# GuyTevet/motion-diffusion-model

Hardware: NVIDIA H100
Metric: motions/sec (higher is better)
Workload: dtype fp16 operands / fp32 accumulate (in/out projections hi-lo split)

## Files before the change

### motion-diffusion-model_b200/csrc/attention_tc.cuh

```cuda
#pragma once
#include <cuda_fp16.h>

#include "epilogues.cuh"
#include "ptx.cuh"

namespace b200 {

constexpr int ATC_THREADS = 128;
constexpr int ATC_QROWS = 64;
constexpr int ATC_TILES_PER_CTA = 4;
constexpr int ATC_DH = 128;
constexpr int ATC_MAX_KEYS = 256;

__host__ __device__ constexpr int atc_keys(int S) { return S <= 64 ? 64 : S <= 208 ? 208 : 256; }

struct AttnTcSmem {
  static __host__ __device__ int total(int keys) { return 1024 + 4 * keys * 128; }
};

template <int KEYS, bool WIDE>
__global__ void __launch_bounds__(ATC_THREADS, 2)
attention_tc_kernel(const __grid_constant__ CUtensorMap map_kv, const __half* __restrict__ qkv, __half* __restrict__ out,
                    const int* __restrict__ kvlen, int S, int d, float scale_log2) {
  constexpr int ATOM = KEYS * 128;
  constexpr int NS = KEYS / 2;
  constexpr int NB = KEYS / 16;
  extern __shared__ uint8_t smem_raw[];
  __shared__ uint64_t bar_k, bar_v;
  uint8_t* sK = reinterpret_cast<uint8_t*>((reinterpret_cast<uintptr_t>(smem_raw) + 1023) & ~uintptr_t(1023));
  uint8_t* sV = sK + 2 * ATOM;
  const int warp = threadIdx.x >> 5, lane = threadIdx.x & 31;
  const int h = blockIdx.x, smp = blockIdx.y;
  const int ld = 3 * d;
  const __half* base = qkv + static_cast<size_t>(smp) * S * ld;

  pdl_launch_dependents();
  if (threadIdx.x == 0) {
    tma_prefetch_desc(&map_kv);
    mbar_init(&bar_k, 1);
    mbar_init(&bar_v, 1);
    fence_barrier_init();
  }
  __syncthreads();
  pdl_wait();
  if (threadIdx.x == 0) {
    mbar_expect_tx(&bar_k, 2 * ATOM);
    for (int a = 0; a < 2; ++a) tma_load_3d(sK + a * ATOM, &map_kv, &bar_k, d + h * ATC_DH + 64 * a, 0, smp);
    mbar_expect_tx(&bar_v, 2 * ATOM);
    for (int a = 0; a < 2; ++a) tma_load_3d(sV + a * ATOM, &map_kv, &bar_v, 2 * d + h * ATC_DH + 64 * a, 0, smp);
  }

  const int kvl = min(kvlen[smp], S);
  const int nblk = max(1, (kvl + 15) >> 4);
  const int g = lane >> 2, t = lane & 3;
  const uint64_t desc_k = wgmma_desc_k_sw128(smem_u32(sK));
  const uint64_t desc_v = wgmma_desc_mn_sw128(smem_u32(sV), ATOM);
  const int ntiles = (S + ATC_QROWS - 1) / ATC_QROWS;
  const int ldo = (WIDE ? 2 : 1) * d;

  uint32_t qa[8][4];
  auto load_q = [&](int tile) {
    const int ra = tile * ATC_QROWS + warp * 16 + g, rb = ra + 8;
    const bool va = ra < S, vb = rb < S;
    const uint32_t* pa = reinterpret_cast<const uint32_t*>(base + static_cast<size_t>(va ? ra : 0) * ld + h * ATC_DH);
    const uint32_t* pb = reinterpret_cast<const uint32_t*>(base + static_cast<size_t>(vb ? rb : 0) * ld + h * ATC_DH);
#pragma unroll
    for (int ks = 0; ks < 8; ++ks) {
      qa[ks][0] = va ? pa[8 * ks + t] : 0u;
      qa[ks][1] = vb ? pb[8 * ks + t] : 0u;
      qa[ks][2] = va ? pa[8 * ks + 4 + t] : 0u;
      qa[ks][3] = vb ? pb[8 * ks + 4 + t] : 0u;
    }
  };
  if (static_cast<int>(blockIdx.z) < ntiles) load_q(blockIdx.z);
#pragma unroll 1
  for (int tile = blockIdx.z; tile < ntiles; tile += gridDim.z) {
    const int ra = tile * ATC_QROWS + warp * 16 + g, rb = ra + 8;
    const bool va = ra < S, vb = rb < S;
    float s[NS];
    mbar_wait(&bar_k, 0);
    wgmma_fence();
#pragma unroll
    for (int ks = 0; ks < 8; ++ks)
      WgmmaRA<KEYS, 0>::mma(s, qa[ks], desc_k + (((ks >> 2) * ATOM + (ks & 3) * 32) >> 4), ks != 0);
    wgmma_commit();
    wgmma_wait<0>();
    wgmma_fence_acc(s);
    float mxa = -INFINITY, mxb = -INFINITY;
#pragma unroll
    for (int j = 0; j < NS / 4; ++j)
#pragma unroll
      for (int i = 0; i < 2; ++i) {
        if (8 * j + 2 * t + i < kvl) {
          mxa = fmaxf(mxa, s[4 * j + i]);
          mxb = fmaxf(mxb, s[4 * j + 2 + i]);
        }
      }
#pragma unroll
    for (int o = 1; o < 4; o <<= 1) {
      mxa = fmaxf(mxa, __shfl_xor_sync(0xffffffffu, mxa, o));
      mxb = fmaxf(mxb, __shfl_xor_sync(0xffffffffu, mxb, o));
    }
    const float offa = (mxa == -INFINITY) ? 0.f : mxa * scale_log2;
    const float offb = (mxb == -INFINITY) ? 0.f : mxb * scale_log2;
    auto ex2 = [](float x) {
      float y;
      asm("ex2.approx.ftz.f32 %0, %1;" : "=f"(y) : "f"(x));
      return y;
    };
    uint32_t p[NB][4];
    float suma = 0.f, sumb = 0.f;
#pragma unroll
    for (int j = 0; j < NS / 4; ++j) {
      const int key = 8 * j + 2 * t;
      const float p0 = key < kvl ? ex2(fmaf(s[4 * j], scale_log2, -offa)) : 0.f;
      const float p1 = key + 1 < kvl ? ex2(fmaf(s[4 * j + 1], scale_log2, -offa)) : 0.f;
      const float p2 = key < kvl ? ex2(fmaf(s[4 * j + 2], scale_log2, -offb)) : 0.f;
      const float p3 = key + 1 < kvl ? ex2(fmaf(s[4 * j + 3], scale_log2, -offb)) : 0.f;
      suma += p0 + p1;
      sumb += p2 + p3;
      p[j >> 1][2 * (j & 1)] = pack_half2(p0, p1);
      p[j >> 1][2 * (j & 1) + 1] = pack_half2(p2, p3);
    }
#pragma unroll
    for (int off = 1; off < 4; off <<= 1) {
      suma += __shfl_xor_sync(0xffffffffu, suma, off);
      sumb += __shfl_xor_sync(0xffffffffu, sumb, off);
    }
    const float inva = suma > 0.f ? 1.f / suma : 0.f;
    const float invb = sumb > 0.f ? 1.f / sumb : 0.f;
    float o[64];
    mbar_wait(&bar_v, 0);
    wgmma_fence();
#pragma unroll
    for (int kk = 0; kk < NB; ++kk)
      if (kk < nblk) WgmmaRA<128, 1>::mma(o, p[kk], desc_v + ((kk * 16 * 128) >> 4), kk != 0);
    wgmma_commit();
    if (tile + static_cast<int>(gridDim.z) < ntiles) load_q(tile + gridDim.z);
    wgmma_wait<0>();
    wgmma_fence_acc(o);
    __half* oa = out + (static_cast<size_t>(smp) * S + (va ? ra : 0)) * ldo + h * ATC_DH + 2 * t;
    __half* ob = out + (static_cast<size_t>(smp) * S + (vb ? rb : 0)) * ldo + h * ATC_DH + 2 * t;
#pragma unroll
    for (int j = 0; j < 16; ++j) {
      const float x0 = o[4 * j] * inva, x1 = o[4 * j + 1] * inva, x2 = o[4 * j + 2] * invb, x3 = o[4 * j + 3] * invb;
      const __half2 ha = __floats2half2_rn(x0, x1), hb = __floats2half2_rn(x2, x3);
      if (va) *reinterpret_cast<__half2*>(oa + 8 * j) = ha;
      if (vb) *reinterpret_cast<__half2*>(ob + 8 * j) = hb;
      if (WIDE) {
        const float2 fa = __half22float2(ha), fb = __half22float2(hb);
        if (va) *reinterpret_cast<__half2*>(oa + d + 8 * j) = __floats2half2_rn(x0 - fa.x, x1 - fa.y);
        if (vb) *reinterpret_cast<__half2*>(ob + d + 8 * j) = __floats2half2_rn(x2 - fb.x, x3 - fb.y);
      }
    }
  }
}

}
```

### motion-diffusion-model_b200/csrc/engine.cu

```cuda
#include <cuda.h>
#include <cuda_fp16.h>
#include <cuda_runtime.h>

#include <cmath>
#include <cstdarg>
#include <cstdio>
#include <cstring>
#include <map>
#include <string>
#include <vector>

#include "../../include/b200mdm.h"
#include "attention_tc.cuh"
#include "epilogues.cuh"
#include "gemm.cuh"
#include "gemm_ln.cuh"
#include "gemm_pingpong.cuh"
#include "postprocess.cuh"
#include "kernels.cuh"

using namespace b200;

static thread_local char g_err[512] = "";
static int fail(int code, const char* fmt, ...) {
  va_list ap;
  va_start(ap, fmt);
  vsnprintf(g_err, sizeof(g_err), fmt, ap);
  va_end(ap);
  return code;
}
#define CUDA_TRY(expr)                                                                               \
  do {                                                                                               \
    cudaError_t _e = (expr);                                                                         \
    if (_e != cudaSuccess)                                                                           \
      return fail(B200MDM_ECUDA, "%s failed: %s (%s:%d)", #expr, cudaGetErrorString(_e), __FILE__, __LINE__); \
  } while (0)
#define TRY(expr)            \
  do {                       \
    int _r = (expr);         \
    if (_r != B200MDM_OK) return _r; \
  } while (0)

typedef CUresult (*EncodeTiledFn)(CUtensorMap*, CUtensorMapDataType, cuuint32_t, void*, const cuuint64_t*,
                                  const cuuint64_t*, const cuuint32_t*, const cuuint32_t*, CUtensorMapInterleave,
                                  CUtensorMapSwizzle, CUtensorMapL2promotion, CUtensorMapFloatOOBfill);
static EncodeTiledFn g_encode = nullptr;
static int resolve_driver() {
  if (g_encode) return B200MDM_OK;
  void* fn = nullptr;
  cudaDriverEntryPointQueryResult qres;
  CUDA_TRY(cudaGetDriverEntryPoint("cuTensorMapEncodeTiled", &fn, cudaEnableDefault, &qres));
  if (!fn || qres != cudaDriverEntryPointSuccess) return fail(B200MDM_ECUDA, "cuTensorMapEncodeTiled not available");
  g_encode = reinterpret_cast<EncodeTiledFn>(fn);
  return B200MDM_OK;
}
static int make_map_t(CUtensorMap* m, const void* ptr, int elem_bytes, uint64_t rows, uint64_t cols, uint64_t ld,
                      uint32_t box_rows) {
  TRY(resolve_driver());
  if ((reinterpret_cast<uintptr_t>(ptr) & 15) || (ld * elem_bytes) % 16) return fail(B200MDM_EINVAL, "TMA operand misaligned");
  cuuint64_t gdim[2] = {cols, rows};
  cuuint64_t gstr[1] = {ld * elem_bytes};
  cuuint32_t box[2] = {static_cast<cuuint32_t>(128 / elem_bytes), box_rows};
  cuuint32_t estr[2] = {1, 1};
  CUresult r = g_encode(m, elem_bytes == 2 ? CU_TENSOR_MAP_DATA_TYPE_FLOAT16 : CU_TENSOR_MAP_DATA_TYPE_FLOAT32, 2,
                        const_cast<void*>(ptr), gdim, gstr, box, estr, CU_TENSOR_MAP_INTERLEAVE_NONE,
                        CU_TENSOR_MAP_SWIZZLE_128B, CU_TENSOR_MAP_L2_PROMOTION_L2_256B, CU_TENSOR_MAP_FLOAT_OOB_FILL_NONE);
  if (r != CUDA_SUCCESS) return fail(B200MDM_ECUDA, "cuTensorMapEncodeTiled failed (%d)", static_cast<int>(r));
  return B200MDM_OK;
}
static int make_map(CUtensorMap* m, const void* ptr, uint64_t rows, uint64_t cols, uint64_t ld, uint32_t box_rows) {
  return make_map_t(m, ptr, 2, rows, cols, ld, box_rows);
}
static int make_map_3d(CUtensorMap* m, const void* ptr, uint64_t n, uint64_t rows, uint64_t cols, uint64_t ld,
                       uint32_t box_rows) {
  TRY(resolve_driver());
  if ((reinterpret_cast<uintptr_t>(ptr) & 15) || (ld * 2) % 16) return fail(B200MDM_EINVAL, "TMA operand misaligned");
  cuuint64_t gdim[3] = {cols, rows, n};
  cuuint64_t gstr[2] = {ld * 2, rows * ld * 2};
  cuuint32_t box[3] = {64, box_rows, 1};
  cuuint32_t estr[3] = {1, 1, 1};
  CUresult r = g_encode(m, CU_TENSOR_MAP_DATA_TYPE_FLOAT16, 3, const_cast<void*>(ptr), gdim, gstr, box, estr,
                        CU_TENSOR_MAP_INTERLEAVE_NONE, CU_TENSOR_MAP_SWIZZLE_128B, CU_TENSOR_MAP_L2_PROMOTION_L2_256B,
                        CU_TENSOR_MAP_FLOAT_OOB_FILL_NONE);
  if (r != CUDA_SUCCESS) return fail(B200MDM_ECUDA, "cuTensorMapEncodeTiled(3d) failed (%d)", static_cast<int>(r));
  return B200MDM_OK;
}

static int make_hres_map(CUtensorMap* m, const void* hres, uint64_t rows) {
  return make_map(m, hres, rows, 2 * GLN_D, 2 * GLN_D, GLN_RES_BOX_ROWS);
}

static int make_map_res(CUtensorMap* m, const void* ptr, uint64_t rows, uint64_t d) {
  TRY(resolve_driver());
  if (reinterpret_cast<uintptr_t>(ptr) & 15) return fail(B200MDM_EINVAL, "TMA operand misaligned");
  cuuint64_t gdim[2] = {2 * d, rows};
  cuuint64_t gstr[1] = {d * 4};
  cuuint32_t box[2] = {32, 32};
  cuuint32_t estr[2] = {1, 1};
  CUresult r = g_encode(m, CU_TENSOR_MAP_DATA_TYPE_FLOAT16, 2, const_cast<void*>(ptr), gdim, gstr, box, estr,
                        CU_TENSOR_MAP_INTERLEAVE_NONE, CU_TENSOR_MAP_SWIZZLE_64B, CU_TENSOR_MAP_L2_PROMOTION_L2_256B,
                        CU_TENSOR_MAP_FLOAT_OOB_FILL_NONE);
  if (r != CUDA_SUCCESS) return fail(B200MDM_ECUDA, "cuTensorMapEncodeTiled(residual) failed (%d)", static_cast<int>(r));
  return B200MDM_OK;
}

struct Tensor32 {
  float* dev = nullptr;
  std::vector<int64_t> shape;
  size_t numel = 0;
};

struct LayerW {
  __half *wqkv = nullptr, *wo = nullptr, *w1 = nullptr, *w2 = nullptr;
  const float *bqkv, *bo, *b1, *b2, *g1, *be1, *g2, *be2;
  CUtensorMap m_wqkv, m_w1;
  CUtensorMap m_wo_256, m_w2_256;
  __half *wq_c = nullptr, *wo_c = nullptr;
  const float *bq_c = nullptr, *bo_c = nullptr, *g3 = nullptr, *be3 = nullptr;
  CUtensorMap m_wq_c, m_wo_c_256;
  const float *wv_c32 = nullptr, *bv_c32 = nullptr, *wo_c32 = nullptr;
};

struct GraphKey {
  int mode = -1, B = 0, T = 0, flags = 0;
  int order = 0;
  const void *pred = nullptr, *imask = nullptr, *imotion = nullptr;
  const void* target_g = nullptr;
  bool operator==(const GraphKey& o) const {
    return mode == o.mode && B == o.B && T == o.T && flags == o.flags && order == o.order && pred == o.pred &&
           imask == o.imask && imotion == o.imotion && target_g == o.target_g;
  }
};

struct Workspace {
  int B = 0, T = 0, S = 0, halves = 1, Bp = 0, M = 0, MB = 0;
  __half *xin16 = nullptr, *hres = nullptr, *qkv16 = nullptr, *att16 = nullptr, *ffn16 = nullptr, *g16 = nullptr;
  float *tok0 = nullptr, *condproj = nullptr, *proj = nullptr, *scale = nullptr, *x_work = nullptr, *eps_buf = nullptr;
  int *kvlen = nullptr, *tvec = nullptr, *action = nullptr;
  CUtensorMap m_xin, m_h16, m_att, m_ffn, m_g16;
  CUtensorMap m_qkv_st, m_ffn_st;
  CUtensorMap m_qkv_kv;
  CUtensorMap m_res_c, m_res_u;
  CUtensorMap m_hres;
  float* pe_bias = nullptr;
  bool cond_set = false;
  int Mt = 0;
  float *encperm = nullptr, *memtok = nullptr, *memproj = nullptr;
  __half *mem16 = nullptr, *qc16 = nullptr, *kvc16 = nullptr;
  unsigned char* memmask = nullptr;
  CUtensorMap m_mem, m_qc_st, m_kvc_st;
  bool prefix_set = false;
  float *cross_mb = nullptr, *cross_u = nullptr, *cross_b = nullptr, *cross_c = nullptr;
  float *tgt_valid = nullptr, *tgt_g = nullptr;
  bool target_set = false;
  float *plms_ring = nullptr, *plms_mid = nullptr, *plms_pred = nullptr;
  int plms_done = -1, plms_order = 0;
  cudaGraphExec_t graph_exec = nullptr;
  GraphKey graph_key;
  int graph_kernels = 0;
  unsigned long long last_use = 0;
};

struct b200mdm_engine : Workspace {
  b200mdm_config cfg;
  int d, ff, L, H, JF, Kp_in, N_out_pad;
  int num_sms = 132;
  std::map<std::string, Tensor32> store;
  bool finalized = false;
  __half *w_in3 = nullptr, *w_out3 = nullptr;
  CUtensorMap m_win, m_wout;
  std::vector<LayerW> layers;
  const float *b_in = nullptr, *b_out = nullptr, *pe = nullptr, *w_txt = nullptr, *b_txt = nullptr, *act_emb = nullptr;
  float *temb_hidden = nullptr, *temb_table = nullptr;
  __half* wkv_all = nullptr;
  float* bkv_all = nullptr;
  CUtensorMap m_wkv_all;
  float *tw0 = nullptr, *tb0 = nullptr, *twk = nullptr, *tbk = nullptr, *twsum = nullptr;
  int tG = 0, tdj = 0, tin = 0, tlayers = 0;
  std::vector<float> h_valid;
  float* sched = nullptr;
  int* tmap = nullptr;
  int n_steps = 0, sched_cap = 0;
  float* sched_next = nullptr;
  bool sched_next_fresh = false;
  std::vector<Workspace> pool;
  unsigned long long use_clock = 0;
  std::vector<int> h_kv, h_action;
  std::vector<unsigned char> h_mask;
  bool dec = false;
  bool dec_clip = false;
  float* cross_t = nullptr;
  int ctx = 0, s_off = 1;
  int kw = 1;
  const unsigned char* inpaint_mask = nullptr;
  const float* inpaint_motion = nullptr;
  unsigned long long noise_seed = 0;
  long long noise_sample_base = 0;
  StepState* state = nullptr;
  cudaStream_t work = nullptr;
  cudaEvent_t ev_in = nullptr, ev_out = nullptr;
  long long launches = 0;
};

template <class T>
static int dalloc(T** p, size_t n, bool zero = false) {
  const cudaError_t err = cudaMalloc(reinterpret_cast<void**>(p), n * sizeof(T));
  if (err != cudaSuccess) {
    cudaGetLastError();
    return fail(B200MDM_ECUDA, "cudaMalloc of %zu bytes failed: %s", n * sizeof(T), cudaGetErrorString(err));
  }
  if (zero) CUDA_TRY(cudaMemset(*p, 0, n * sizeof(T)));
  return B200MDM_OK;
}
template <class T>
static void dfree(T*& p) {
  if (p) cudaFree(p);
  p = nullptr;
}

template <int BN, class Epi, bool RES = false>
static int set_gemm_attr() {
  CUDA_TRY(cudaFuncSetAttribute(gemm_f16_wgmma<BN, Epi, RES>, cudaFuncAttributeMaxDynamicSharedMemorySize,
                                GemmSmem<BN, Epi, RES>::TOTAL));
  return B200MDM_OK;
}
template <class Epi>
static int set_pingpong_attr() {
  CUDA_TRY(cudaFuncSetAttribute(gemm_f16_pingpong<Epi>, cudaFuncAttributeMaxDynamicSharedMemorySize, PP_SMEM_BYTES));
  return B200MDM_OK;
}
template <int KEYS>
static int set_attention_attr() {
  CUDA_TRY(cudaFuncSetAttribute(attention_tc_kernel<KEYS, false>, cudaFuncAttributeMaxDynamicSharedMemorySize,
                                AttnTcSmem::total(KEYS)));
  CUDA_TRY(cudaFuncSetAttribute(attention_tc_kernel<KEYS, true>, cudaFuncAttributeMaxDynamicSharedMemorySize,
                                AttnTcSmem::total(KEYS)));
  return B200MDM_OK;
}
static int init_kernel_attrs() {
  static unsigned long long done_mask = 0;
  int dev = 0;
  CUDA_TRY(cudaGetDevice(&dev));
  if (dev < 64 && ((done_mask >> dev) & 1ull)) return B200MDM_OK;
  TRY((set_pingpong_attr<EpiBiasF16<false>>()));
  TRY((set_pingpong_attr<EpiBiasF16<true>>()));
  TRY((set_pingpong_attr<EpiBiasF16Wide<true>>()));
  TRY((set_pingpong_attr<EpiBiasF16Global>()));
  TRY((set_gemm_attr<256, EpiBiasF16<false>>()));
  TRY((set_gemm_attr<256, EpiBiasF16<true>>()));
  TRY((set_gemm_attr<64, EpiBiasF16<false>, true>()));
  TRY((set_gemm_attr<64, EpiBiasF16<true>, true>()));
  CUDA_TRY(cudaFuncSetAttribute(gemm_resid_ln_cluster, cudaFuncAttributeMaxDynamicSharedMemorySize, GemmLnSmem::TOTAL));
  TRY((set_gemm_attr<128, EpiEmbed>()));
  TRY((set_gemm_attr<96, EpiOut<OutStep>>()));
  TRY((set_gemm_attr<96, EpiOut<OutPlms>>()));
  TRY((set_gemm_attr<96, EpiOut<OutReverse>>()));
  TRY((set_attention_attr<64>()));
  TRY((set_attention_attr<208>()));
  TRY((set_attention_attr<256>()));
  CUDA_TRY(cudaFuncSetAttribute(cross_attention_long_kernel, cudaFuncAttributeMaxDynamicSharedMemorySize, XAL_SMEM));
  if (dev < 64) done_mask |= 1ull << dev;
  return B200MDM_OK;
}

static bool g_pdl_now = false;
static bool pdl_enabled() {
  static int v = -1;
  if (v < 0) {
    const char* e = getenv("B200MDM_PDL");
    v = (e && e[0] == '0') ? 0 : 1;
  }
  return v == 1;
}
struct PdlScope {
  PdlScope() { g_pdl_now = pdl_enabled(); }
  ~PdlScope() { g_pdl_now = false; }
};
template <class... KArgs, class... Args>
static cudaError_t launch_k(void (*kern)(KArgs...), dim3 grid, dim3 block, size_t smem, cudaStream_t s, Args&&... args) {
  cudaLaunchConfig_t cfg;
  memset(&cfg, 0, sizeof(cfg));
  cfg.gridDim = grid;
  cfg.blockDim = block;
  cfg.dynamicSmemBytes = smem;
  cfg.stream = s;
  cudaLaunchAttribute at[1];
  at[0].id = cudaLaunchAttributeProgrammaticStreamSerialization;
  at[0].val.programmaticStreamSerializationAllowed = 1;
  cfg.attrs = at;
  cfg.numAttrs = g_pdl_now ? 1 : 0;
  return cudaLaunchKernelEx(&cfg, kern, static_cast<KArgs>(std::forward<Args>(args))...);
}

template <int BN, class Epi, class = void> struct epi_unstaged : std::false_type {};
template <int BN, class Epi> struct epi_unstaged<BN, Epi, std::enable_if_t<Epi::UNSTAGED>> : std::true_type {};

template <int BN, class Epi>
static int launch_gemm(const CUtensorMap& a, const CUtensorMap& b, const CUtensorMap& c, int M, int N, int K,
                       const typename Epi::Params& p, cudaStream_t s, int num_sms) {
  if (!epi_unstaged<BN, Epi>::value && N * 4 > GEMM_BIAS_BYTES)
    return fail(B200MDM_ENOTIMPL, "GEMM epilogue vectors are staged for N <= %d", GEMM_BIAS_BYTES / 4);
  const int tiles = ((M + GEMM_BLOCK_M - 1) / GEMM_BLOCK_M) * ((N + BN - 1) / BN);
  const int grid = tiles < num_sms ? tiles : num_sms;
  CUDA_TRY(launch_k(gemm_f16_wgmma<BN, Epi>, dim3(grid), dim3(GEMM_THREADS), GemmSmem<BN, Epi>::TOTAL, s, a, b, c, M, N, K, p));
  return B200MDM_OK;
}
template <int BN, class Epi>
static int launch_gemm_resident(const CUtensorMap& a, const CUtensorMap& b, const CUtensorMap& c, int M, int N, int K,
                                const typename Epi::Params& p, cudaStream_t s, int num_sms) {
  const int tiles_n = (N + BN - 1) / BN;
  const int tiles = ((M + GEMM_BLOCK_M - 1) / GEMM_BLOCK_M) * tiles_n;
  const int grid = tiles < num_sms ? tiles : num_sms;
  if (K > GEMM_RES_KB_MAX * GEMM_BLOCK_K || tiles_n > grid || N * 4 > GEMM_BIAS_BYTES)
    return fail(B200MDM_ENOTIMPL, "W-resident GEMM needs K <= %d and N <= %d", GEMM_RES_KB_MAX * GEMM_BLOCK_K, grid * BN);
  CUDA_TRY(launch_k(gemm_f16_wgmma<BN, Epi, true>, dim3(grid), dim3(GEMM_THREADS), GemmSmem<BN, Epi, true>::TOTAL, s, a, b, c, M, N, K, p));
  return B200MDM_OK;
}
template <class Epi>
static int launch_gemm_pp(const CUtensorMap& a, const CUtensorMap& b, const CUtensorMap& c, int M, int N, int K,
                          const typename Epi::Params& p, cudaStream_t s, int num_sms) {
  if (!epi_unstaged<PP_BLOCK_N, Epi>::value && N * 4 > GEMM_BIAS_BYTES)
    return fail(B200MDM_ENOTIMPL, "GEMM epilogue vectors are staged for N <= %d", GEMM_BIAS_BYTES / 4);
  const int tiles = ((M + GEMM_BLOCK_M - 1) / GEMM_BLOCK_M) * ((N + PP_BLOCK_N - 1) / PP_BLOCK_N);
  const int grid = tiles < num_sms ? tiles : num_sms;
  CUDA_TRY(launch_k(gemm_f16_pingpong<Epi>, dim3(grid), dim3(GEMM_THREADS), PP_SMEM_BYTES, s, a, b, c, M, N, K, p));
  return B200MDM_OK;
}
template <bool GELU>
static int launch_gemm_bias(const CUtensorMap& a, const CUtensorMap& b, const CUtensorMap& c, int M, int N, int K,
                            const float* bias, cudaStream_t s, int num_sms) {
  typename EpiBiasF16<GELU>::Params p{bias};
  return launch_gemm_pp<EpiBiasF16<GELU>>(a, b, c, M, N, K, p, s, num_sms);
}

static int launch_gemm_resid_ln(const CUtensorMap& a, const CUtensorMap& w256, const CUtensorMap& hres, int M, int K,
                                const float* bias, const float* gamma, const float* beta, cudaStream_t s, int num_sms) {
  const int tiles = (M + GEMM_BLOCK_M - 1) / GEMM_BLOCK_M;
  const int max_clusters = num_sms / 2;
  const int clusters = tiles < max_clusters ? tiles : max_clusters;
  GemmLnParams lp{bias, gamma, beta, 1e-5f};
  CUDA_TRY(launch_k(gemm_resid_ln_cluster, dim3(2 * clusters), dim3(GLN_THREADS), GemmLnSmem::TOTAL, s, a, w256, hres, M, K, lp));
  return B200MDM_OK;
}

static int make_attention_kv_map(CUtensorMap* m, const void* qkv, int n_samples, int S, int ld) {
  return make_map_3d(m, qkv, n_samples, S, ld, ld, atc_keys(S));
}
template <int KEYS>
static cudaError_t launch_attention_keys(const CUtensorMap& map_kv, const __half* qkv, __half* out, const int* kvlen,
                                         dim3 grid, int S, int d, float scale_log2, cudaStream_t s, bool wide) {
  return launch_k(wide ? attention_tc_kernel<KEYS, true> : attention_tc_kernel<KEYS, false>, grid, dim3(ATC_THREADS),
                  AttnTcSmem::total(KEYS), s, map_kv, qkv, out, kvlen, S, d, scale_log2);
}
static int launch_attention_tc(const CUtensorMap& map_kv, const __half* qkv, __half* out, const int* kvlen, int n_samples,
                               int S, int d, int H, cudaStream_t s, bool wide = false) {
  if (d != H * ATC_DH) return fail(B200MDM_ENOTIMPL, "attention: head_dim must be 128");
  if (S > ATC_MAX_KEYS) return fail(B200MDM_ENOTIMPL, "attention: at most %d tokens per sample", ATC_MAX_KEYS);
  const float scale_log2 = 1.4426950408889634f / sqrtf(static_cast<float>(ATC_DH));
  const int tiles = (S + ATC_QROWS - 1) / ATC_QROWS;
  const dim3 grid(H, n_samples, (tiles + ATC_TILES_PER_CTA - 1) / ATC_TILES_PER_CTA);
  const int keys = atc_keys(S);
  if (keys == 64) CUDA_TRY(launch_attention_keys<64>(map_kv, qkv, out, kvlen, grid, S, d, scale_log2, s, wide));
  else if (keys == 208) CUDA_TRY(launch_attention_keys<208>(map_kv, qkv, out, kvlen, grid, S, d, scale_log2, s, wide));
  else CUDA_TRY(launch_attention_keys<256>(map_kv, qkv, out, kvlen, grid, S, d, scale_log2, s, wide));
  return B200MDM_OK;
}
#ifdef B200_TRACE
static int debug_skip_mask() {
  static int v = -1;
  if (v < 0) {
    const char* e = getenv("B200MDM_DEBUG_SKIP");
    v = e ? atoi(e) : 0;
  }
  return v;
}
#define B200_SKIP(bit) (debug_skip_mask() & (bit))
#else
#define B200_SKIP(bit) (0)
#endif
extern "C" const char* b200mdm_last_error(void) { return g_err; }
extern "C" int b200mdm_version(void) { return 1; }

extern "C" int b200mdm_create(const b200mdm_config* cfg, b200mdm_engine** out) {
  if (!cfg || !out) return fail(B200MDM_EINVAL, "null argument");
  if (cfg->arch != B200MDM_ARCH_TRANS_ENC && cfg->arch != B200MDM_ARCH_TRANS_DEC)
    return fail(B200MDM_ENOTIMPL, "arch %d: trans_enc and trans_dec are implemented", cfg->arch);
  if (cfg->arch == B200MDM_ARCH_TRANS_DEC && (cfg->cond_mode != B200MDM_COND_TEXT || cfg->context_len < 0))
    return fail(B200MDM_ENOTIMPL, "trans_dec needs text-token conditioning (BERT) and context_len >= 0");
  if (cfg->emb_trans_dec < 0 || cfg->emb_trans_dec > 1 || cfg->dec_memory < B200MDM_DEC_MEMORY_TOKENS ||
      cfg->dec_memory > B200MDM_DEC_MEMORY_CLIP)
    return fail(B200MDM_EINVAL, "emb_trans_dec must be 0 or 1 and dec_memory 0 (tokens) or 1 (CLIP) (got %d / %d)",
                cfg->emb_trans_dec, cfg->dec_memory);
  if (cfg->arch == B200MDM_ARCH_TRANS_ENC && (cfg->emb_trans_dec || cfg->dec_memory))
    return fail(B200MDM_EINVAL, "emb_trans_dec and dec_memory are trans_dec fields");
  if (cfg->arch == B200MDM_ARCH_TRANS_DEC && (cfg->dec_memory == B200MDM_DEC_MEMORY_CLIP) != (cfg->emb_trans_dec == 1))
    return fail(B200MDM_ENOTIMPL, "trans_dec implements the BERT token memory without the timestep token (DiP) and the CLIP "
                "memory with it (emb_trans_dec); got dec_memory %d, emb_trans_dec %d", cfg->dec_memory, cfg->emb_trans_dec);
  if (cfg->dec_memory == B200MDM_DEC_MEMORY_CLIP && cfg->context_len != 0)
    return fail(B200MDM_ENOTIMPL, "trans_dec with a CLIP memory has no prefix completion (context_len %d)", cfg->context_len);
  if (cfg->latent_dim != 512 || cfg->num_heads != 4 || cfg->ff_size % 64 || cfg->ff_size <= 0)
    return fail(B200MDM_ENOTIMPL, "kernels are specialised for latent_dim 512 / 4 heads (got %d / %d)", cfg->latent_dim,
                cfg->num_heads);
  if (cfg->num_layers <= 0 || cfg->njoints <= 0 || cfg->nfeats <= 0 || cfg->pos_embed_max_len <= 0 || cfg->temb_rows <= 0)
    return fail(B200MDM_EINVAL, "bad config");
  if (cfg->target_encoder < B200MDM_TARGET_NONE || cfg->target_encoder > B200MDM_TARGET_SPLIT)
    return fail(B200MDM_EINVAL, "target_encoder %d: 0 none, 1 single, 2 multi, 3 split", cfg->target_encoder);
  if (cfg->target_encoder != B200MDM_TARGET_NONE) {
    if (cfg->target_joints <= 0 || cfg->target_joints > 64 || cfg->target_enc_layers < 0 || cfg->target_enc_layers > 16)
      return fail(B200MDM_EINVAL, "target encoder: 1..64 joints and 0..16 layers (got %d / %d)", cfg->target_joints,
                  cfg->target_enc_layers);
    if (cfg->target_encoder == B200MDM_TARGET_SPLIT && cfg->latent_dim % cfg->target_joints)
      return fail(B200MDM_EINVAL, "split target encoder: latent_dim %% target_joints != 0 (model/mdm.py:427)");
  }
  int dev = 0;
  CUDA_TRY(cudaGetDevice(&dev));
  cudaDeviceProp prop;
  CUDA_TRY(cudaGetDeviceProperties(&prop, dev));
  if (prop.major != 9 || prop.minor != 0) return fail(B200MDM_ECUDA, "sm_90a device required (found sm_%d%d)", prop.major, prop.minor);
  TRY(init_kernel_attrs());
  TRY(resolve_driver());
  b200mdm_engine* e = new b200mdm_engine();
  e->cfg = *cfg;
  e->d = cfg->latent_dim;
  e->ff = cfg->ff_size;
  e->L = cfg->num_layers;
  e->H = cfg->num_heads;
  e->JF = cfg->njoints * cfg->nfeats;
  e->Kp_in = (e->JF + 7) & ~7;
  e->N_out_pad = ((e->JF + 95) / 96) * 96;
  e->num_sms = prop.multiProcessorCount;
  e->layers.resize(e->L);
  e->dec = cfg->arch == B200MDM_ARCH_TRANS_DEC;
  e->dec_clip = e->dec && cfg->dec_memory == B200MDM_DEC_MEMORY_CLIP;
  e->ctx = e->dec ? cfg->context_len : 0;
  e->s_off = (e->dec && !e->dec_clip) ? e->ctx : 1;
  e->kw = (e->dec && !e->dec_clip) ? 2 : 1;
  CUDA_TRY(cudaStreamCreateWithFlags(&e->work, cudaStreamNonBlocking));
  CUDA_TRY(cudaEventCreateWithFlags(&e->ev_in, cudaEventDisableTiming));
  CUDA_TRY(cudaEventCreateWithFlags(&e->ev_out, cudaEventDisableTiming));
  TRY(dalloc(&e->state, 1, true));
  *out = e;
  return B200MDM_OK;
}

static void drop_graph(Workspace* w) {
  if (w->graph_exec) cudaGraphExecDestroy(w->graph_exec);
  w->graph_exec = nullptr;
  w->graph_key = GraphKey();
}
static void free_workspace(Workspace* w) {
  drop_graph(w);
  dfree(w->xin16); dfree(w->hres); dfree(w->qkv16); dfree(w->att16); dfree(w->ffn16); dfree(w->g16);
  dfree(w->tok0); dfree(w->condproj); dfree(w->proj); dfree(w->scale); dfree(w->x_work); dfree(w->pe_bias); dfree(w->eps_buf);
  dfree(w->kvlen); dfree(w->tvec); dfree(w->action);
  dfree(w->encperm); dfree(w->memtok); dfree(w->memproj); dfree(w->mem16); dfree(w->qc16); dfree(w->kvc16); dfree(w->memmask);
  dfree(w->cross_mb); dfree(w->cross_u); dfree(w->cross_b); dfree(w->cross_c);
  dfree(w->tgt_valid); dfree(w->tgt_g);
  dfree(w->plms_ring); dfree(w->plms_mid); dfree(w->plms_pred);
  *w = Workspace();
}
static void free_all_workspaces(b200mdm_engine* e) {
  free_workspace(static_cast<Workspace*>(e));
  for (auto& w : e->pool) free_workspace(&w);
  e->pool.clear();
}
static void drop_all_graphs(b200mdm_engine* e) {
  drop_graph(static_cast<Workspace*>(e));
  for (auto& w : e->pool) drop_graph(&w);
}

extern "C" int b200mdm_destroy(b200mdm_engine* e) {
  if (!e) return B200MDM_OK;
  cudaDeviceSynchronize();
  free_all_workspaces(e);
  for (auto& kv : e->store) cudaFree(kv.second.dev);
  for (auto& l : e->layers) { dfree(l.wqkv); dfree(l.wo); dfree(l.w1); dfree(l.w2); dfree(l.wq_c); dfree(l.wo_c); }
  dfree(e->w_in3); dfree(e->w_out3); dfree(e->temb_hidden); dfree(e->temb_table); dfree(e->sched); dfree(e->tmap);
  dfree(e->sched_next);
  dfree(e->wkv_all); dfree(e->bkv_all); dfree(e->cross_t);
  dfree(e->tw0); dfree(e->tb0); dfree(e->twk); dfree(e->tbk); dfree(e->twsum);
  dfree(e->state);
  if (e->work) cudaStreamDestroy(e->work);
  if (e->ev_in) cudaEventDestroy(e->ev_in);
  if (e->ev_out) cudaEventDestroy(e->ev_out);
  delete e;
  return B200MDM_OK;
}

static bool known_weight_name(const b200mdm_engine* e, const std::string& n) {
  static const char* fixed[] = {"input_process.poseEmbedding.weight", "input_process.poseEmbedding.bias",
                                "embed_timestep.time_embed.0.weight", "embed_timestep.time_embed.0.bias",
                                "embed_timestep.time_embed.2.weight", "embed_timestep.time_embed.2.bias",
                                "embed_text.weight", "embed_text.bias", "embed_action.action_embedding",
                                "output_process.poseFinal.weight", "output_process.poseFinal.bias",
                                "sequence_pos_encoder.pe", "embed_timestep.sequence_pos_encoder.pe"};
  for (const char* f : fixed)
    if (n == f) return true;
  static const char* per_layer[] = {"self_attn.in_proj_weight", "self_attn.in_proj_bias", "self_attn.out_proj.weight",
                                    "self_attn.out_proj.bias", "linear1.weight", "linear1.bias", "linear2.weight",
                                    "linear2.bias", "norm1.weight", "norm1.bias", "norm2.weight", "norm2.bias",
                                    "multihead_attn.in_proj_weight", "multihead_attn.in_proj_bias",
                                    "multihead_attn.out_proj.weight", "multihead_attn.out_proj.bias", "norm3.weight", "norm3.bias"};
  const std::string pre = e->dec ? "seqTransDecoder.layers." : "seqTransEncoder.layers.";
  if (n.compare(0, pre.size(), pre) == 0) {
    size_t dot = n.find('.', pre.size());
    if (dot == std::string::npos) return false;
    int l = atoi(n.substr(pre.size(), dot - pre.size()).c_str());
    if (l < 0 || l >= e->L) return false;
    std::string rest = n.substr(dot + 1);
    for (const char* f : per_layer)
      if (rest == f) return true;
  }
  if (e->cfg.target_encoder != B200MDM_TARGET_NONE) {
    const int tl = e->cfg.target_enc_layers, nj = e->cfg.target_joints;
    auto lin = [](const std::string& r, int max_layer) {
      for (int k = 0; k <= max_layer; ++k)
        if (r == std::to_string(2 * k) + ".weight" || r == std::to_string(2 * k) + ".bias") return true;
      return false;
    };
    auto joint = [nj](const std::string& r, std::string* tail) {
      size_t dot = r.find('.');
      if (dot == std::string::npos || dot == 0 || r.find_first_not_of("0123456789") != dot) return false;
      if (atoi(r.substr(0, dot).c_str()) >= nj) return false;
      *tail = r.substr(dot + 1);
      return true;
    };
    const std::string pre = "embed_target_cond.";
    if (n.compare(0, pre.size(), pre) != 0) return false;
    const std::string r = n.substr(pre.size());
    std::string tail;
    switch (e->cfg.target_encoder) {
      case B200MDM_TARGET_SINGLE:
        return r.compare(0, 4, "mlp.") == 0 && lin(r.substr(4), tl);
      case B200MDM_TARGET_SPLIT:
        return r.compare(0, 10, "mini_mlps.") == 0 && joint(r.substr(10), &tail) && lin(tail, tl);
      case B200MDM_TARGET_MULTI:
        if (r == "target_all_loc_emb.weights") return true;
        return r.compare(0, 15, "target_loc_emb.") == 0 && joint(r.substr(15), &tail) && lin(tail, 1);
    }
  }
  return false;
}

extern "C" int b200mdm_load_weight(b200mdm_engine* e, const char* name, const float* data, const int64_t* shape,
                                   int32_t ndim) {
  if (!e || !name || !data || !shape || ndim < 1 || ndim > 4) return fail(B200MDM_EINVAL, "bad argument");
  std::string n(name);
  if (!known_weight_name(e, n)) return fail(B200MDM_EINVAL, "unexpected state_dict key '%s'", name);
  size_t numel = 1;
  std::vector<int64_t> shp(shape, shape + ndim);
  for (int64_t s : shp) {
    if (s <= 0) return fail(B200MDM_EINVAL, "bad shape for '%s'", name);
    numel *= static_cast<size_t>(s);
  }
  Tensor32& t = e->store[n];
  if (t.dev && t.numel != numel) { cudaFree(t.dev); t.dev = nullptr; }
  if (!t.dev) TRY(dalloc(&t.dev, numel));
  t.shape = shp;
  t.numel = numel;
  CUDA_TRY(cudaMemcpy(t.dev, data, numel * sizeof(float), cudaMemcpyDefault));
  e->finalized = false;
  return B200MDM_OK;
}

static int need(b200mdm_engine* e, const std::string& name, std::initializer_list<int64_t> shape, const float** out) {
  auto it = e->store.find(name);
  if (it == e->store.end()) return fail(B200MDM_ESTATE, "missing weight '%s'", name.c_str());
  std::vector<int64_t> want(shape);
  size_t numel = 1;
  for (int64_t s : want) numel *= static_cast<size_t>(s);
  if (it->second.numel != numel) return fail(B200MDM_EINVAL, "weight '%s' has %zu elements, expected %zu", name.c_str(), it->second.numel, numel);
  *out = it->second.dev;
  return B200MDM_OK;
}

static int to_f16(const float* src, __half** dst, size_t n, cudaStream_t s) {
  TRY(dalloc(dst, n));
  f32_to_f16_kernel<<<512, 256, 0, s>>>(src, *dst, n);
  CUDA_TRY(cudaGetLastError());
  return B200MDM_OK;
}
static int to_f16_k(const float* src, __half** dst, int N, int K, int kw, cudaStream_t s) {
  if (kw == 1) return to_f16(src, dst, static_cast<size_t>(N) * K, s);
  TRY(dalloc(dst, static_cast<size_t>(N) * K * 2));
  f32_to_f16_dup_kernel<<<512, 256, 0, s>>>(src, *dst, N, K);
  CUDA_TRY(cudaGetLastError());
  return B200MDM_OK;
}

static int pack_target_weights(b200mdm_engine* e, cudaStream_t s) {
  dfree(e->tw0); dfree(e->tb0); dfree(e->twk); dfree(e->tbk); dfree(e->twsum);
  const int enc = e->cfg.target_encoder, n = e->cfg.target_joints, d = e->d;
  if (enc == B200MDM_TARGET_NONE) return B200MDM_OK;
  const bool multi = enc == B200MDM_TARGET_MULTI;
  e->tG = enc == B200MDM_TARGET_SINGLE ? 1 : n;
  e->tdj = enc == B200MDM_TARGET_SPLIT ? d / n : d;
  e->tin = enc == B200MDM_TARGET_SINGLE ? 4 * n : multi ? 3 : 4;
  e->tlayers = multi ? 1 : e->cfg.target_enc_layers;
  const int G = e->tG, dj = e->tdj, in = e->tin, L = e->tlayers;
  TRY(dalloc(&e->tw0, static_cast<size_t>(G) * dj * in));
  TRY(dalloc(&e->tb0, static_cast<size_t>(G) * dj));
  TRY(dalloc(&e->twk, static_cast<size_t>(L > 0 ? L : 1) * G * dj * dj));
  TRY(dalloc(&e->tbk, static_cast<size_t>(L > 0 ? L : 1) * G * dj));
  for (int i = 0; i < G; ++i) {
    const std::string p = enc == B200MDM_TARGET_SINGLE ? std::string("embed_target_cond.mlp.")
                          : multi ? "embed_target_cond.target_loc_emb." + std::to_string(i) + "."
                                  : "embed_target_cond.mini_mlps." + std::to_string(i) + ".";
    const float *w, *b;
    TRY(need(e, p + "0.weight", {dj, in}, &w));
    TRY(need(e, p + "0.bias", {dj}, &b));
    CUDA_TRY(cudaMemcpyAsync(e->tw0 + static_cast<size_t>(i) * dj * in, w, sizeof(float) * dj * in, cudaMemcpyDeviceToDevice, s));
    CUDA_TRY(cudaMemcpyAsync(e->tb0 + static_cast<size_t>(i) * dj, b, sizeof(float) * dj, cudaMemcpyDeviceToDevice, s));
    for (int l = 0; l < L; ++l) {
      const std::string k = std::to_string(2 * (l + 1));
      TRY(need(e, p + k + ".weight", {dj, dj}, &w));
      TRY(need(e, p + k + ".bias", {dj}, &b));
      CUDA_TRY(cudaMemcpyAsync(e->twk + (static_cast<size_t>(l) * G + i) * dj * dj, w, sizeof(float) * dj * dj,
                               cudaMemcpyDeviceToDevice, s));
      CUDA_TRY(cudaMemcpyAsync(e->tbk + (static_cast<size_t>(l) * G + i) * dj, b, sizeof(float) * dj, cudaMemcpyDeviceToDevice, s));
    }
  }
  if (multi) {
    const float* ws;
    TRY(need(e, "embed_target_cond.target_all_loc_emb.weights", {n}, &ws));
    TRY(dalloc(&e->twsum, n));
    CUDA_TRY(cudaMemcpyAsync(e->twsum, ws, sizeof(float) * n, cudaMemcpyDeviceToDevice, s));
  }
  return B200MDM_OK;
}

static int encode_target(b200mdm_engine* e, const float* target_dev, const uint8_t* valid_host, int B, float* valid_dev,
                         float* g_dev, std::vector<float>& staging, cudaStream_t s) {
  const int n = e->cfg.target_joints, d = e->d;
  staging.assign(static_cast<size_t>(B) * n, 0.f);
  for (size_t i = 0; i < staging.size(); ++i) staging[i] = valid_host[i] ? 1.f : 0.f;
  CUDA_TRY(cudaMemcpyAsync(valid_dev, staging.data(), staging.size() * sizeof(float), cudaMemcpyHostToDevice, s));
  const size_t smem = sizeof(float) * (4 * n + 2 * d);
  target_embed_kernel<<<B, d, smem, s>>>(target_dev, valid_dev, e->tw0, e->tb0, e->twk, e->tbk, e->twsum, g_dev, n, e->tG,
                                         e->tdj, e->tin, e->tlayers, e->cfg.target_encoder == B200MDM_TARGET_MULTI ? 1 : 0);
  CUDA_TRY(cudaGetLastError());
  return B200MDM_OK;
}

extern "C" int b200mdm_finalize_weights(b200mdm_engine* e, void* stream) {
  if (!e) return fail(B200MDM_EINVAL, "null engine");
  cudaStream_t s = static_cast<cudaStream_t>(stream);
  const int d = e->d, ff = e->ff, JF = e->JF;
  const float *w_in, *w_out, *t0w, *t0b, *t2w, *t2b;
  TRY(need(e, "input_process.poseEmbedding.weight", {d, JF}, &w_in));
  TRY(need(e, "input_process.poseEmbedding.bias", {d}, &e->b_in));
  TRY(need(e, "output_process.poseFinal.weight", {JF, d}, &w_out));
  TRY(need(e, "output_process.poseFinal.bias", {JF}, &e->b_out));
  TRY(need(e, "embed_timestep.time_embed.0.weight", {d, d}, &t0w));
  TRY(need(e, "embed_timestep.time_embed.0.bias", {d}, &t0b));
  TRY(need(e, "embed_timestep.time_embed.2.weight", {d, d}, &t2w));
  TRY(need(e, "embed_timestep.time_embed.2.bias", {d}, &t2b));
  TRY(need(e, "sequence_pos_encoder.pe", {e->cfg.pos_embed_max_len, d}, &e->pe));
  if (e->cfg.cond_mode == B200MDM_COND_TEXT) {
    TRY(need(e, "embed_text.weight", {d, e->cfg.cond_dim}, &e->w_txt));
    TRY(need(e, "embed_text.bias", {d}, &e->b_txt));
  } else if (e->cfg.cond_mode == B200MDM_COND_ACTION) {
    TRY(need(e, "embed_action.action_embedding", {e->cfg.num_actions, d}, &e->act_emb));
  }
  if (e->cfg.temb_rows > e->cfg.pos_embed_max_len) return fail(B200MDM_EINVAL, "temb_rows exceeds the positional table");

  CUDA_TRY(cudaDeviceSynchronize());
  free_all_workspaces(e);
  for (auto& l : e->layers) { dfree(l.wqkv); dfree(l.wo); dfree(l.w1); dfree(l.w2); dfree(l.wq_c); dfree(l.wo_c); }
  dfree(e->w_in3); dfree(e->w_out3); dfree(e->temb_hidden); dfree(e->temb_table); dfree(e->wkv_all); dfree(e->bkv_all);
  dfree(e->cross_t);

  const int Kp = e->Kp_in;
  TRY(dalloc(&e->w_in3, static_cast<size_t>(d) * 3 * Kp, true));
  split_weight_kernel<<<d, 128, 0, s>>>(w_in, e->w_in3, d, JF, Kp);
  CUDA_TRY(cudaGetLastError());
  TRY(dalloc(&e->w_out3, static_cast<size_t>(e->N_out_pad) * 3 * d, true));
  split_weight_kernel<<<JF, 128, 0, s>>>(w_out, e->w_out3, JF, d, d);
  CUDA_TRY(cudaGetLastError());
  TRY(make_map(&e->m_win, e->w_in3, d, 3 * Kp, 3 * Kp, 128));
  TRY(make_map(&e->m_wout, e->w_out3, e->N_out_pad, 3 * d, 3 * d, 96));

  for (int l = 0; l < e->L; ++l) {
    LayerW& w = e->layers[l];
    const std::string p = std::string(e->dec ? "seqTransDecoder.layers." : "seqTransEncoder.layers.") + std::to_string(l) + ".";
    const float *wqkv, *wo, *w1, *w2;
    TRY(need(e, p + "self_attn.in_proj_weight", {3 * d, d}, &wqkv));
    TRY(need(e, p + "self_attn.in_proj_bias", {3 * d}, &w.bqkv));
    TRY(need(e, p + "self_attn.out_proj.weight", {d, d}, &wo));
    TRY(need(e, p + "self_attn.out_proj.bias", {d}, &w.bo));
    TRY(need(e, p + "linear1.weight", {ff, d}, &w1));
    TRY(need(e, p + "linear1.bias", {ff}, &w.b1));
    TRY(need(e, p + "linear2.weight", {d, ff}, &w2));
    TRY(need(e, p + "linear2.bias", {d}, &w.b2));
    TRY(need(e, p + "norm1.weight", {d}, &w.g1));
    TRY(need(e, p + "norm1.bias", {d}, &w.be1));
    TRY(need(e, p + "norm2.weight", {d}, &w.g2));
    TRY(need(e, p + "norm2.bias", {d}, &w.be2));
    const int kw = e->kw;
    TRY(to_f16_k(wqkv, &w.wqkv, 3 * d, d, kw, s));
    TRY(to_f16_k(wo, &w.wo, d, d, kw, s));
    TRY(to_f16_k(w1, &w.w1, ff, d, kw, s));
    TRY(to_f16_k(w2, &w.w2, d, ff, kw, s));
    TRY(make_map(&w.m_wqkv, w.wqkv, 3 * d, kw * d, kw * d, 128));
    TRY(make_map(&w.m_w1, w.w1, ff, kw * d, kw * d, 128));
    TRY(make_map(&w.m_wo_256, w.wo, d, kw * d, kw * d, 256));
    TRY(make_map(&w.m_w2_256, w.w2, d, kw * ff, kw * ff, 256));
    if (e->dec) {
      const float *wc, *bc, *woc;
      TRY(need(e, p + "multihead_attn.in_proj_weight", {3 * d, d}, &wc));
      TRY(need(e, p + "multihead_attn.in_proj_bias", {3 * d}, &bc));
      TRY(need(e, p + "multihead_attn.out_proj.weight", {d, d}, &woc));
      TRY(need(e, p + "multihead_attn.out_proj.bias", {d}, &w.bo_c));
      TRY(need(e, p + "norm3.weight", {d}, &w.g3));
      TRY(need(e, p + "norm3.bias", {d}, &w.be3));
      if (e->dec_clip) {
        w.wv_c32 = wc + static_cast<size_t>(2) * d * d;
        w.bv_c32 = bc + 2 * d;
        w.wo_c32 = woc;
        continue;
      }
      w.bq_c = bc;
      TRY(to_f16_k(wc, &w.wq_c, d, d, kw, s));
      if (l == 0) {
        TRY(dalloc(&e->wkv_all, static_cast<size_t>(e->L) * 2 * d * d));
        TRY(dalloc(&e->bkv_all, static_cast<size_t>(e->L) * 2 * d));
        TRY(make_map(&e->m_wkv_all, e->wkv_all, static_cast<uint64_t>(e->L) * 2 * d, d, d, 128));
      }
      f32_to_f16_kernel<<<512, 256, 0, s>>>(wc + static_cast<size_t>(d) * d, e->wkv_all + static_cast<size_t>(l) * 2 * d * d,
                                            static_cast<size_t>(2) * d * d);
      CUDA_TRY(cudaGetLastError());
      CUDA_TRY(cudaMemcpyAsync(e->bkv_all + static_cast<size_t>(l) * 2 * d, bc + d, sizeof(float) * 2 * d, cudaMemcpyDeviceToDevice, s));
      TRY(to_f16_k(woc, &w.wo_c, d, d, kw, s));
      TRY(make_map(&w.m_wq_c, w.wq_c, d, kw * d, kw * d, 128));
      TRY(make_map(&w.m_wo_c_256, w.wo_c, d, kw * d, kw * d, 256));
    }
  }
  TRY(pack_target_weights(e, s));
  const int R = e->cfg.temb_rows;
  TRY(dalloc(&e->temb_hidden, static_cast<size_t>(R) * d));
  TRY(dalloc(&e->temb_table, static_cast<size_t>(R) * d));
  const size_t warps = static_cast<size_t>(R) * d;
  const int blocks = static_cast<int>((warps * 32 + 255) / 256);
  small_linear_kernel<1><<<blocks, 256, 0, s>>>(e->pe, t0w, t0b, e->temb_hidden, R, d, d, d);
  CUDA_TRY(cudaGetLastError());
  small_linear_kernel<0><<<blocks, 256, 0, s>>>(e->temb_hidden, t2w, t2b, e->temb_table, R, d, d, d);
  CUDA_TRY(cudaGetLastError());
  if (e->dec_clip) {
    TRY(dalloc(&e->cross_t, static_cast<size_t>(e->L) * R * d));
    for (int l = 0; l < e->L; ++l) {
      const LayerW& w = e->layers[l];
      small_linear_kernel<0><<<blocks, 256, 0, s>>>(e->temb_table, w.wv_c32, nullptr, e->temb_hidden, R, d, d, d);
      CUDA_TRY(cudaGetLastError());
      small_linear_kernel<0><<<blocks, 256, 0, s>>>(e->temb_hidden, w.wo_c32, nullptr, e->cross_t + static_cast<size_t>(l) * R * d,
                                                    R, d, d, d);
      CUDA_TRY(cudaGetLastError());
    }
  }
  CUDA_TRY(cudaStreamSynchronize(s));
  e->finalized = true;
  return B200MDM_OK;
}

extern "C" int b200mdm_set_schedule(b200mdm_engine* e, int32_t n_steps, const float* rows_host,
                                    const int32_t* timestep_map_host) {
  if (!e || n_steps <= 0 || !rows_host || !timestep_map_host) return fail(B200MDM_EINVAL, "bad argument");
  for (int i = 0; i < n_steps; ++i)
    if (timestep_map_host[i] < 0 || timestep_map_host[i] >= e->cfg.temb_rows)
      return fail(B200MDM_EINVAL, "timestep_map[%d] = %d outside the pre-embedded range [0, %d)", i, timestep_map_host[i],
                  e->cfg.temb_rows);
  CUDA_TRY(cudaDeviceSynchronize());
  if (n_steps > e->sched_cap) {
    drop_all_graphs(e);
    dfree(e->sched);
    dfree(e->tmap);
    dfree(e->sched_next);
    e->sched_cap = 0;
    const int cap = n_steps > 1000 ? n_steps : 1000;
    TRY(dalloc(&e->sched, static_cast<size_t>(cap) * SCHED_STRIDE));
    TRY(dalloc(&e->tmap, cap));
    TRY(dalloc(&e->sched_next, static_cast<size_t>(cap) * SCHED_NEXT_STRIDE));
    e->sched_cap = cap;
  }
  e->n_steps = n_steps;
  e->sched_next_fresh = false;
  CUDA_TRY(cudaMemcpy(e->sched, rows_host, static_cast<size_t>(n_steps) * SCHED_STRIDE * sizeof(float), cudaMemcpyHostToDevice));
  CUDA_TRY(cudaMemcpy(e->tmap, timestep_map_host, static_cast<size_t>(n_steps) * sizeof(int), cudaMemcpyHostToDevice));
  return B200MDM_OK;
}

static_assert(SCHED_NEXT_STRIDE == B200MDM_SCHED_NEXT_STRIDE, "the reverse table's row layout is part of the ABI");
static_assert(MODE_X0 == B200MDM_MODE_X0 && MODE_DDPM == B200MDM_MODE_DDPM && MODE_DDIM == B200MDM_MODE_DDIM &&
                  MODE_DDIM_REVERSE == B200MDM_MODE_DDIM_REVERSE,
              "the output epilogue's modes are the public ones");
extern "C" int b200mdm_set_schedule_next(b200mdm_engine* e, int32_t n_steps, const float* rows_host) {
  if (!e || !rows_host) return fail(B200MDM_EINVAL, "bad argument");
  if (e->n_steps <= 0) return fail(B200MDM_ESTATE, "b200mdm_set_schedule has not been called");
  if (n_steps != e->n_steps)
    return fail(B200MDM_EINVAL, "n_steps %d differs from the schedule's %d", n_steps, e->n_steps);
  CUDA_TRY(cudaDeviceSynchronize());
  CUDA_TRY(cudaMemcpy(e->sched_next, rows_host, static_cast<size_t>(n_steps) * SCHED_NEXT_STRIDE * sizeof(float),
                      cudaMemcpyHostToDevice));
  e->sched_next_fresh = true;
  return B200MDM_OK;
}

static void attach_l2_window(b200mdm_engine* e, cudaStream_t stream = nullptr);

static int build_workspace(b200mdm_engine* e, int B, int T, int halves, cudaStream_t s) {
  const int d = e->d, S = T + e->s_off, Bp = halves * B;
  const size_t M = static_cast<size_t>(Bp) * S, MB = static_cast<size_t>(B) * S;
  TRY(dalloc(&e->xin16, MB * 3 * e->Kp_in, true));
  const int kw = e->kw;
  TRY(dalloc(&e->hres, M * d * 2, true));
  TRY(dalloc(&e->qkv16, M * 3 * d));
  TRY(dalloc(&e->att16, M * d * kw));
  TRY(dalloc(&e->ffn16, M * e->ff * kw));
  TRY(dalloc(&e->g16, static_cast<size_t>(B) * T * 3 * d));
  TRY(dalloc(&e->tok0, static_cast<size_t>(Bp) * d));
  TRY(dalloc(&e->condproj, static_cast<size_t>(Bp) * d, true));
  TRY(dalloc(&e->proj, static_cast<size_t>(B) * d, true));
  TRY(dalloc(&e->scale, B, true));
  TRY(dalloc(&e->x_work, static_cast<size_t>(B) * e->JF * T));
  TRY(dalloc(&e->kvlen, Bp));
  TRY(dalloc(&e->tvec, B, true));
  TRY(dalloc(&e->action, B, true));
  if (e->dec_clip) {
    const size_t rows = static_cast<size_t>(Bp) * d, all = static_cast<size_t>(e->L) * Bp * d;
    TRY(dalloc(&e->cross_mb, rows));
    TRY(dalloc(&e->cross_u, rows));
    TRY(dalloc(&e->cross_b, all));
    TRY(dalloc(&e->cross_c, all));
  } else if (e->dec) {
    TRY(dalloc(&e->qc16, M * d));
    TRY(make_map_t(&e->m_qc_st, e->qc16, 2, M, d, d, 32));
    e->Mt = 0;
    e->prefix_set = false;
  }
  e->B = B; e->T = T; e->S = S; e->halves = halves; e->Bp = Bp;
  e->M = static_cast<int>(M); e->MB = static_cast<int>(MB);
  attach_l2_window(e);
  TRY(make_map(&e->m_xin, e->xin16, MB, 3 * e->Kp_in, 3 * e->Kp_in, GEMM_BLOCK_M));
  TRY(make_map(&e->m_h16, e->hres, M, kw * d, 2 * d, GEMM_BLOCK_M));
  TRY(make_map(&e->m_att, e->att16, M, kw * d, kw * d, GEMM_BLOCK_M));
  TRY(make_map(&e->m_ffn, e->ffn16, M, kw * e->ff, kw * e->ff, GEMM_BLOCK_M));
  TRY(make_map(&e->m_g16, e->g16, static_cast<size_t>(B) * T, 3 * d, 3 * d, GEMM_BLOCK_M));
  TRY(make_map_t(&e->m_qkv_st, e->qkv16, 2, M, 3 * d, 3 * d, 32));
  TRY(make_attention_kv_map(&e->m_qkv_kv, e->qkv16, Bp, S, 3 * d));
  TRY(make_map_t(&e->m_ffn_st, e->ffn16, 2, M, kw * e->ff, kw * e->ff, 32));
  TRY(make_map_res(&e->m_res_c, e->hres, MB, d));
  TRY(make_map_res(&e->m_res_u, e->hres + (halves == 2 ? MB * d * 2 : 0), MB, d));
  TRY(make_hres_map(&e->m_hres, e->hres, M));
  TRY(dalloc(&e->pe_bias, static_cast<size_t>(S) * d));
  pe_bias_kernel<<<S, 128, 0, s>>>(e->pe_bias, e->pe, e->b_in, S, d);
  CUDA_TRY(cudaGetLastError());
  TRY(dalloc(&e->eps_buf, static_cast<size_t>(B) * e->JF * T));
  if (e->cfg.target_encoder != B200MDM_TARGET_NONE) {
    TRY(dalloc(&e->tgt_valid, static_cast<size_t>(B) * e->cfg.target_joints));
    TRY(dalloc(&e->tgt_g, static_cast<size_t>(B) * d));
  }
  return B200MDM_OK;
}

static void attach_l2_window(b200mdm_engine* e, cudaStream_t stream) {
  cudaDeviceProp prop;
  int dev = 0;
  if (cudaGetDevice(&dev) == cudaSuccess && cudaGetDeviceProperties(&prop, dev) == cudaSuccess && prop.persistingL2CacheMaxSize > 0) {
    const size_t want = static_cast<size_t>(e->M) * e->d * 2 * sizeof(__half);
    cudaStreamAttrValue attr;
    memset(&attr, 0, sizeof(attr));
    if (2 * want <= static_cast<size_t>(prop.l2CacheSize)) {
      const size_t carve = want < static_cast<size_t>(prop.persistingL2CacheMaxSize) ? want : static_cast<size_t>(prop.persistingL2CacheMaxSize);
      cudaDeviceSetLimit(cudaLimitPersistingL2CacheSize, carve);
      attr.accessPolicyWindow.base_ptr = e->hres;
      attr.accessPolicyWindow.num_bytes = want < static_cast<size_t>(prop.accessPolicyMaxWindowSize) ? want : static_cast<size_t>(prop.accessPolicyMaxWindowSize);
      attr.accessPolicyWindow.hitRatio = want <= carve ? 1.0f : static_cast<float>(carve) / static_cast<float>(want);
      attr.accessPolicyWindow.hitProp = cudaAccessPropertyPersisting;
      attr.accessPolicyWindow.missProp = cudaAccessPropertyStreaming;
    }
    cudaStreamSetAttribute(stream ? stream : e->work, cudaStreamAttributeAccessPolicyWindow, &attr);
    cudaGetLastError();
  }
}

static int select_workspace(b200mdm_engine* e, int B, int T, int halves, cudaStream_t s) {
  constexpr size_t MAX_PARKED = 3;
  Workspace* cur = static_cast<Workspace*>(e);
  e->last_use = ++e->use_clock;
  if (cur->B == B && cur->T == T && cur->halves == halves) return B200MDM_OK;
  if (cur->B > 0) {
    e->pool.push_back(*cur);
    *cur = Workspace();
  }
  for (size_t i = 0; i < e->pool.size(); ++i) {
    if (e->pool[i].B == B && e->pool[i].T == T && e->pool[i].halves == halves) {
      *cur = e->pool[i];
      e->pool.erase(e->pool.begin() + i);
      cur->last_use = e->use_clock;
      cur->cond_set = false;
      cur->prefix_set = false;
      cur->target_set = false;
      attach_l2_window(e);
      return B200MDM_OK;
    }
  }
  while (e->pool.size() > MAX_PARKED) {
    size_t lru = 0;
    for (size_t i = 1; i < e->pool.size(); ++i)
      if (e->pool[i].last_use < e->pool[lru].last_use) lru = i;
    CUDA_TRY(cudaDeviceSynchronize());
    free_workspace(&e->pool[lru]);
    e->pool.erase(e->pool.begin() + lru);
  }
  int r = build_workspace(e, B, T, halves, s);
  if (r != B200MDM_OK) free_workspace(cur);
  cur->last_use = e->use_clock;
  return r;
}


extern "C" int b200mdm_set_cond(b200mdm_engine* e, int32_t batch, int32_t nframes, const float* cond_embed_dev,
                                const int64_t* lengths_host, const float* scale_dev, int32_t force_uncond,
                                const int64_t* action_host, void* stream) {
  if (!e) return fail(B200MDM_EINVAL, "null engine");
  if (e->dec) return fail(B200MDM_EINVAL, "trans_dec engines take their conditioning through b200mdm_set_cond_dec");
  if (!e->finalized) return fail(B200MDM_ESTATE, "weights not finalised");
  if (batch <= 0 || nframes <= 0) return fail(B200MDM_EINVAL, "bad batch / nframes");
  if (nframes + 1 > e->cfg.pos_embed_max_len) return fail(B200MDM_EINVAL, "sequence longer than the positional table");
  if (nframes + 1 > ATC_MAX_KEYS)
    return fail(B200MDM_ENOTIMPL, "sequences of more than %d tokens (the attention kernels keep all keys of a sample on chip; "
                "every dataset of the reference stops at 196 frames)", ATC_MAX_KEYS);
  cudaStream_t s = static_cast<cudaStream_t>(stream);
  const int halves = scale_dev ? 2 : 1;
  if (e->cfg.cond_mode == B200MDM_COND_TEXT && !cond_embed_dev && !(halves == 1 && force_uncond))
    return fail(B200MDM_EINVAL, "text-conditioned model needs y['text_embed']");
  if (e->cfg.cond_mode == B200MDM_COND_ACTION && !action_host && !(halves == 1 && force_uncond))
    return fail(B200MDM_EINVAL, "action-conditioned model needs y['action']");
  if (halves == 2 && e->cfg.cond_mode == B200MDM_COND_NONE)
    return fail(B200MDM_EINVAL, "classifier-free guidance needs a conditioned model (sampler_util.py:29)");
  TRY(select_workspace(e, batch, nframes, halves, s));
  const int d = e->d, B = batch, S = nframes + 1;
  std::vector<int>& kv = e->h_kv;
  kv.assign(e->Bp, S);
  if (e->cfg.mask_frames && lengths_host && nframes > 1) {
    for (int b = 0; b < e->Bp; ++b) {
      long long len = lengths_host[b % B];
      if (len < 0) len = 0;
      if (len > nframes) len = nframes;
      kv[b] = static_cast<int>(len) + 1;
    }
  }
  CUDA_TRY(cudaMemcpyAsync(e->kvlen, kv.data(), kv.size() * sizeof(int), cudaMemcpyHostToDevice, s));
  if (scale_dev) CUDA_TRY(cudaMemcpyAsync(e->scale, scale_dev, B * sizeof(float), cudaMemcpyDeviceToDevice, s));
  if (e->cfg.cond_mode == B200MDM_COND_ACTION && action_host) {
    std::vector<int>& a = e->h_action;
    a.assign(B, 0);
    for (int b = 0; b < B; ++b) {
      if (action_host[b] < 0 || action_host[b] >= e->cfg.num_actions) return fail(B200MDM_EINVAL, "action index out of range");
      a[b] = static_cast<int>(action_host[b]);
    }
    CUDA_TRY(cudaMemcpyAsync(e->action, a.data(), B * sizeof(int), cudaMemcpyHostToDevice, s));
  }
  if (e->cfg.cond_mode == B200MDM_COND_TEXT && cond_embed_dev) {
    const size_t warps = static_cast<size_t>(B) * d;
    small_linear_kernel<0><<<static_cast<int>((warps * 32 + 255) / 256), 256, 0, s>>>(cond_embed_dev, e->w_txt, e->b_txt, e->proj, B,
                                                                                       d, e->cfg.cond_dim, e->cfg.cond_dim);
    CUDA_TRY(cudaGetLastError());
    e->launches++;
  }
  condproj_fill_kernel<<<e->Bp, 128, 0, s>>>(e->condproj, e->proj, e->b_txt, e->act_emb, e->action, B, d, e->Bp,
                                             (halves == 1 && force_uncond) ? 1 : 0, e->cfg.cond_mode);
  CUDA_TRY(cudaGetLastError());
  e->launches++;
  e->cond_set = true;
  e->target_set = false;
  return B200MDM_OK;
}

static int cross_rows_per_sample(b200mdm_engine* e, const float* g, cudaStream_t s) {
  const int d = e->d, Bp = e->Bp;
  cross_mem_kernel<<<Bp, 128, 0, s>>>(e->cross_mb, e->condproj, g, e->B, d);
  CUDA_TRY(cudaGetLastError());
  const int blocks = static_cast<int>((static_cast<size_t>(Bp) * d * 32 + 255) / 256);
  for (int l = 0; l < e->L; ++l) {
    const LayerW& w = e->layers[l];
    small_linear_kernel<0><<<blocks, 256, 0, s>>>(e->cross_mb, w.wv_c32, w.bv_c32, e->cross_u, Bp, d, d, d);
    CUDA_TRY(cudaGetLastError());
    small_linear_kernel<0><<<blocks, 256, 0, s>>>(e->cross_u, w.wo_c32, w.bo_c, e->cross_b + static_cast<size_t>(l) * Bp * d,
                                                  Bp, d, d, d);
    CUDA_TRY(cudaGetLastError());
  }
  e->launches += 1 + 2 * e->L;
  return B200MDM_OK;
}

static int set_cond_dec_clip(b200mdm_engine* e, int32_t batch, int32_t nframes, const float* clip_dev,
                             const uint8_t* text_mask_host, int32_t n_tokens, const int64_t* lengths_host,
                             const float* scale_dev, int32_t force_uncond, cudaStream_t s) {
  if (n_tokens != 1) return fail(B200MDM_EINVAL, "a CLIP-memory decoder takes one memory token per sample (n_tokens %d)", n_tokens);
  if (batch <= 0 || nframes <= 0) return fail(B200MDM_EINVAL, "bad batch / nframes");
  if (!clip_dev || !text_mask_host) return fail(B200MDM_EINVAL, "the CLIP decoder needs y['text_embed'] and an all-zero mask");
  for (int b = 0; b < batch; ++b)
    if (text_mask_host[b]) return fail(B200MDM_EINVAL, "the CLIP memory has no padding mask (model/mdm.py:262-263)");
  if (nframes + 1 > e->cfg.pos_embed_max_len) return fail(B200MDM_EINVAL, "sequence longer than the positional table");
  if (nframes + 1 > ATC_MAX_KEYS) return fail(B200MDM_ENOTIMPL, "sequences of more than %d tokens", ATC_MAX_KEYS);
  const int halves = scale_dev ? 2 : 1;
  TRY(select_workspace(e, batch, nframes, halves, s));
  const int d = e->d, B = batch, S = e->S;
  std::vector<int>& kv = e->h_kv;
  kv.assign(e->Bp, S);
  if (e->cfg.mask_frames && lengths_host && nframes > 1) {
    for (int b = 0; b < e->Bp; ++b) {
      long long len = lengths_host[b % B];
      if (len < 0) len = 0;
      if (len > nframes) len = nframes;
      kv[b] = static_cast<int>(len) + 1;
    }
  }
  CUDA_TRY(cudaMemcpyAsync(e->kvlen, kv.data(), kv.size() * sizeof(int), cudaMemcpyHostToDevice, s));
  if (scale_dev) CUDA_TRY(cudaMemcpyAsync(e->scale, scale_dev, B * sizeof(float), cudaMemcpyDeviceToDevice, s));
  const size_t warps = static_cast<size_t>(B) * d;
  small_linear_kernel<0><<<static_cast<int>((warps * 32 + 255) / 256), 256, 0, s>>>(clip_dev, e->w_txt, e->b_txt, e->proj, B, d,
                                                                                     e->cfg.cond_dim, e->cfg.cond_dim);
  CUDA_TRY(cudaGetLastError());
  condproj_fill_kernel<<<e->Bp, 128, 0, s>>>(e->condproj, e->proj, e->b_txt, nullptr, nullptr, B, d, e->Bp,
                                             (halves == 1 && force_uncond) ? 1 : 0, B200MDM_COND_TEXT);
  CUDA_TRY(cudaGetLastError());
  e->launches += 2;
  TRY(cross_rows_per_sample(e, nullptr, s));
  e->cond_set = true;
  e->target_set = false;
  return B200MDM_OK;
}

extern "C" int b200mdm_set_cond_dec(b200mdm_engine* e, int32_t batch, int32_t nframes, const float* enc_text_dev,
                                    const uint8_t* text_mask_host, int32_t n_tokens, const int64_t* lengths_host,
                                    const float* scale_dev, int32_t force_uncond, void* stream) {
  if (!e) return fail(B200MDM_EINVAL, "null engine");
  if (!e->dec) return fail(B200MDM_EINVAL, "b200mdm_set_cond_dec is for trans_dec engines");
  if (!e->finalized) return fail(B200MDM_ESTATE, "weights not finalised");
  if (e->dec_clip)
    return set_cond_dec_clip(e, batch, nframes, enc_text_dev, text_mask_host, n_tokens, lengths_host, scale_dev, force_uncond,
                             static_cast<cudaStream_t>(stream));
  if (batch <= 0 || nframes <= 0) return fail(B200MDM_EINVAL, "bad batch / nframes");
  if (n_tokens <= 0 || n_tokens > XAL_MAX_MT)
    return fail(B200MDM_EINVAL, "n_tokens %d: a text memory holds 1..%d tokens (DistilBERT's position limit)", n_tokens, XAL_MAX_MT);
  if (nframes + e->ctx > e->cfg.pos_embed_max_len) return fail(B200MDM_EINVAL, "sequence longer than the positional table");
  if (nframes + e->ctx > ATC_MAX_KEYS) return fail(B200MDM_ENOTIMPL, "sequences of more than %d tokens", ATC_MAX_KEYS);
  if (!enc_text_dev || !text_mask_host) return fail(B200MDM_EINVAL, "DiP needs y['text_embed'] = (tokens, mask)");
  cudaStream_t s = static_cast<cudaStream_t>(stream);
  const int halves = scale_dev ? 2 : 1;
  TRY(select_workspace(e, batch, nframes, halves, s));
  const int d = e->d, B = batch, S = e->S, Bp = e->Bp, Mt = n_tokens, C = e->cfg.cond_dim;
  if (Mt != e->Mt) {
    CUDA_TRY(cudaDeviceSynchronize());
    drop_graph(e);
    dfree(e->encperm); dfree(e->memtok); dfree(e->memproj); dfree(e->mem16); dfree(e->kvc16); dfree(e->memmask);
    e->Mt = 0;
    TRY(dalloc(&e->encperm, static_cast<size_t>(B) * Mt * C));
    TRY(dalloc(&e->memtok, static_cast<size_t>(B) * Mt * d));
    TRY(dalloc(&e->memproj, static_cast<size_t>(Bp) * Mt * d));
    TRY(dalloc(&e->mem16, static_cast<size_t>(Bp) * Mt * 2 * d));
    TRY(dalloc(&e->kvc16, static_cast<size_t>(Bp) * Mt * 2 * d * e->L));
    TRY(dalloc(&e->memmask, static_cast<size_t>(Bp) * Mt));
    TRY(make_map(&e->m_mem, e->mem16, static_cast<uint64_t>(Bp) * Mt, 2 * d, 2 * d, GEMM_BLOCK_M));
    TRY(make_map_t(&e->m_kvc_st, e->kvc16, 2, static_cast<uint64_t>(Bp) * Mt, 2 * d * e->L, 2 * d * e->L, 32));
    e->Mt = Mt;
  }
  std::vector<int>& kv = e->h_kv;
  kv.assign(Bp, S);
  if (e->cfg.mask_frames && lengths_host && S > 1) {
    for (int b = 0; b < Bp; ++b) {
      long long len = lengths_host[b % B];
      if (len < 0) len = 0;
      if (len > nframes) len = nframes;
      kv[b] = static_cast<int>(len) + e->ctx;
    }
  }
  std::vector<unsigned char>& mk = e->h_mask;
  mk.assign(static_cast<size_t>(Bp) * Mt, 0);
  for (int b = 0; b < Bp; ++b)
    for (int m = 0; m < Mt; ++m) mk[static_cast<size_t>(b) * Mt + m] = text_mask_host[static_cast<size_t>(b % B) * Mt + m] ? 1 : 0;
  CUDA_TRY(cudaMemcpyAsync(e->kvlen, kv.data(), kv.size() * sizeof(int), cudaMemcpyHostToDevice, s));
  CUDA_TRY(cudaMemcpyAsync(e->memmask, mk.data(), mk.size(), cudaMemcpyHostToDevice, s));
  if (scale_dev) CUDA_TRY(cudaMemcpyAsync(e->scale, scale_dev, B * sizeof(float), cudaMemcpyDeviceToDevice, s));
  permute_mbc_kernel<<<dim3(Mt, B), 128, 0, s>>>(enc_text_dev, e->encperm, Mt, B, C);
  CUDA_TRY(cudaGetLastError());
  const size_t warps = static_cast<size_t>(B) * Mt * d;
  small_linear_kernel<0><<<static_cast<int>((warps * 32 + 255) / 256), 256, 0, s>>>(e->encperm, e->w_txt, e->b_txt, e->memtok, B * Mt, d, C, C);
  CUDA_TRY(cudaGetLastError());
  memproj_fill_kernel<<<dim3(Mt, Bp), 128, 0, s>>>(e->memproj, e->memtok, e->b_txt, B, Mt, d, Bp, (halves == 1 && force_uncond) ? 1 : 0);
  CUDA_TRY(cudaGetLastError());
  e->launches += 3;
  e->cond_set = true;
  e->target_set = false;
  return B200MDM_OK;
}

extern "C" int b200mdm_set_target(b200mdm_engine* e, const float* target_dev, const uint8_t* valid_host, void* stream) {
  if (!e || !target_dev || !valid_host) return fail(B200MDM_EINVAL, "null argument");
  if (e->cfg.target_encoder == B200MDM_TARGET_NONE) return fail(B200MDM_EINVAL, "this engine has no target encoder");
  if (!e->cond_set) return fail(B200MDM_ESTATE, "call b200mdm_set_cond / b200mdm_set_cond_dec first (they size the workspace)");
  TRY(encode_target(e, target_dev, valid_host, e->B, e->tgt_valid, e->tgt_g, e->h_valid, static_cast<cudaStream_t>(stream)));
  e->launches++;
  if (e->dec_clip) TRY(cross_rows_per_sample(e, e->tgt_g, static_cast<cudaStream_t>(stream)));
  e->target_set = true;
  return B200MDM_OK;
}

extern "C" int b200mdm_set_prefix(b200mdm_engine* e, const float* prefix_dev, void* stream) {
  if (!e || !prefix_dev) return fail(B200MDM_EINVAL, "null argument");
  if (!e->dec || e->ctx <= 0) return fail(B200MDM_EINVAL, "this engine has no prefix (context_len == 0)");
  if (!e->cond_set) return fail(B200MDM_ESTATE, "call b200mdm_set_cond_dec first (it sizes the workspace)");
  dim3 grid((e->ctx + 31) / 32, (e->JF + 31) / 32, e->B), block(32, 8);
  pack_input_kernel<<<grid, block, 0, static_cast<cudaStream_t>(stream)>>>(prefix_dev, e->xin16, e->B, e->JF, e->ctx, e->S, e->Kp_in,
                                                                          3 * e->Kp_in, 0);
  CUDA_TRY(cudaGetLastError());
  e->launches++;
  e->prefix_set = true;
  return B200MDM_OK;
}

extern "C" int b200mdm_set_inpaint(b200mdm_engine* e, const uint8_t* mask_dev, const float* motion_dev) {
  if (!e) return fail(B200MDM_EINVAL, "null engine");
  if ((mask_dev == nullptr) != (motion_dev == nullptr)) return fail(B200MDM_EINVAL, "inpainting needs both mask and motion");
  e->inpaint_mask = mask_dev;
  e->inpaint_motion = motion_dev;
  return B200MDM_OK;
}

struct StepArgs {
  int mode = B200MDM_MODE_X0;
  const float* x_in = nullptr;
  const float* noise = nullptr;
  int const_noise = 0;
  int clip = 0;
  float* x_out = nullptr;
  float* pred = nullptr;
  bool explicit_t = false;
  bool philox = false;
  int back = 0;
  const float* x_step = nullptr;
  int order = 0;
};

static int launch_out_gemm(const CUtensorMap& m_g16, const CUtensorMap& m_wout, int B, int T, int JF, int d,
                           const StepArgs& a, EpiOutParams p, cudaStream_t s, int sms) {
  p.x_t = a.x_in;
  p.noise = a.noise;
  p.x_out = a.x_out;
  p.pred_xstart = a.pred;
  p.x_step = a.x_step;
  p.noise_batch_stride = a.const_noise ? 0 : static_cast<long long>(JF) * T;
  p.B = B; p.T = T; p.J = JF; p.mode = a.mode;
  p.clip_denoised = a.clip;
  p.order = a.order;
  p.back = a.back;
  const int M = B * T, N = ((JF + 95) / 96) * 96, K = 3 * d;
  if (a.mode <= MODE_DDIM) return launch_gemm<96, EpiOut<OutStep>>(m_g16, m_wout, m_g16, M, N, K, p, s, sms);
  if (a.mode == MODE_DDIM_REVERSE) return launch_gemm<96, EpiOut<OutReverse>>(m_g16, m_wout, m_g16, M, N, K, p, s, sms);
  return launch_gemm<96, EpiOut<OutPlms>>(m_g16, m_wout, m_g16, M, N, K, p, s, sms);
}

static int enqueue_forward(b200mdm_engine* e, const StepArgs& a, cudaStream_t s, int* n_kernels) {
  const int d = e->d, ff = e->ff, B = e->B, T = e->T, S = e->S, JF = e->JF, Kp = e->Kp_in;
  int nk = 0;
  PdlScope pdl_scope;
  if (a.philox) {
    const long long quads = (static_cast<long long>(JF) * T + 3) / 4 * B;
    const int blocks = static_cast<int>(quads / 256 + 1 < 1184 ? quads / 256 + 1 : 1184);
    CUDA_TRY(launch_k(philox_normal_kernel, dim3(blocks), dim3(256), 0, s, e->eps_buf, B, static_cast<long long>(JF) * T,
                      0ull, 0ll, 0u, e->state));
    ++nk;
  }
  {
    dim3 grid((T + 31) / 32, (JF + 31) / 32, B), block(32, 8);
    CUDA_TRY(launch_k(pack_input_kernel, grid, block, 0, s, a.x_in, e->xin16, B, JF, T, S, Kp, 3 * Kp, e->s_off));
    ++nk;
  }
  {
    EpiEmbed::Params p;
    p.res_c = e->m_res_c; p.res_u = e->m_res_u;
    p.pe_bias = e->pe_bias;
    p.S = S; p.d = d; p.halves = e->halves;
    TRY((launch_gemm<128, EpiEmbed>(e->m_xin, e->m_win, e->m_xin, e->MB, d, 3 * Kp, p, s, e->num_sms)));
    ++nk;
  }
  const float* target_g = e->target_set ? e->tgt_g : nullptr;
  if (!e->dec || e->dec_clip) {
    CUDA_TRY(launch_k(tok0_rows_kernel, dim3(e->Bp), dim3(128), 0, s, e->hres, e->dec_clip ? nullptr : e->condproj,
                      e->temb_table, e->pe, a.explicit_t ? e->tvec : nullptr, e->tmap, e->state, target_g, B, S, d,
                      e->cfg.temb_rows, a.back));
    if (e->dec_clip) {
      CUDA_TRY(launch_k(cross_rows_kernel, dim3(e->Bp, e->L), dim3(128), 0, s, e->cross_c, e->cross_b, e->cross_t,
                        a.explicit_t ? e->tvec : nullptr, e->tmap, e->state, B, e->Bp, d, e->cfg.temb_rows, a.back));
      ++nk;
    }
  } else {
    CUDA_TRY(launch_k(mem_build_kernel, dim3(e->Mt, e->Bp), dim3(128), 0, s, e->mem16, e->memproj, e->temb_table,
                      a.explicit_t ? e->tvec : nullptr, e->tmap, e->state, target_g, B, e->Mt, d, e->cfg.temb_rows, a.back));
    EpiBiasF16Global::Params p{e->bkv_all};
    TRY((launch_gemm_pp<EpiBiasF16Global>(e->m_mem, e->m_wkv_all, e->m_kvc_st, e->Bp * e->Mt, e->L * 2 * d, d, p, s, e->num_sms)));
    ++nk;
  }
  ++nk;
  const int kw = e->kw;
  const bool wide = kw == 2;
  for (int l = 0; l < e->L; ++l) {
    const LayerW& w = e->layers[l];
    if (B200_SKIP(1)) {
      ++nk;
    } else {
      {
        TRY((launch_gemm_bias<false>(e->m_h16, w.m_wqkv, e->m_qkv_st, e->M, 3 * d, d, w.bqkv, s, e->num_sms)));
      }
      TRY(launch_attention_tc(e->m_qkv_kv, e->qkv16, e->att16, e->kvlen, e->Bp, S, d, e->H, s, wide));
    }
    if (!B200_SKIP(2)) TRY(launch_gemm_resid_ln(e->m_att, w.m_wo_256, e->m_hres, e->M, kw * d, w.bo, w.g1, w.be1, s, e->num_sms));
    if (e->dec_clip) {
      CUDA_TRY(launch_k(row_bias_ln_kernel, dim3((e->M + RBLN_ROWS_PER_CTA - 1) / RBLN_ROWS_PER_CTA), dim3(32 * RBLN_ROWS_PER_CTA),
                        0, s, e->hres, e->cross_c + static_cast<size_t>(l) * e->Bp * d, w.g2, w.be2, e->M, S, 1e-5f));
      ++nk;
    } else if (e->dec) {
      TRY((launch_gemm_bias<false>(e->m_h16, w.m_wq_c, e->m_qc_st, e->M, d, d, w.bq_c, s, e->num_sms)));
      {
        const float sl2 = 1.4426950408889634f / sqrtf(128.0f);
        const dim3 cg(e->H, e->Bp), cb(128);
        const __half* kvl = e->kvc16 + static_cast<size_t>(l) * 2 * d;
        const int ldkv = e->L * 2 * d;
        if (e->Mt <= 16)
          CUDA_TRY(launch_k(cross_attention_kernel<2>, cg, cb, 0, s, e->qc16, kvl, e->memmask, e->att16, S, e->Mt, d, ldkv, sl2));
        else if (e->Mt <= 32)
          CUDA_TRY(launch_k(cross_attention_kernel<4>, cg, cb, 0, s, e->qc16, kvl, e->memmask, e->att16, S, e->Mt, d, ldkv, sl2));
        else if (e->Mt <= 64)
          CUDA_TRY(launch_k(cross_attention_kernel<8>, cg, cb, 0, s, e->qc16, kvl, e->memmask, e->att16, S, e->Mt, d, ldkv, sl2));
        else
          CUDA_TRY(launch_k(cross_attention_long_kernel, dim3(e->H, e->Bp, (S + XAL_ROWS - 1) / XAL_ROWS), cb, XAL_SMEM, s,
                            e->qc16, kvl, e->memmask, e->att16, S, e->Mt, d, ldkv, sl2));
      }
      TRY(launch_gemm_resid_ln(e->m_att, w.m_wo_c_256, e->m_hres, e->M, d, w.bo_c, w.g2, w.be2, s, e->num_sms));
      nk += 3;
    }
    if (wide) {
      EpiBiasF16Wide<true>::Params p{w.b1, ff};
      TRY((launch_gemm_pp<EpiBiasF16Wide<true>>(e->m_h16, w.m_w1, e->m_ffn_st, e->M, ff, kw * d, p, s, e->num_sms)));
    } else if (!B200_SKIP(4)) {
      TRY((launch_gemm_bias<true>(e->m_h16, w.m_w1, e->m_ffn_st, e->M, ff, d, w.b1, s, e->num_sms)));
    }
    if (!B200_SKIP(8)) TRY(launch_gemm_resid_ln(e->m_ffn, w.m_w2_256, e->m_hres, e->M, kw * ff, w.b2, e->dec ? w.g3 : w.g2,
                             e->dec ? w.be3 : w.be2, s, e->num_sms));
    nk += 5;
  }
  CUDA_TRY(launch_k(blend_split_kernel, dim3((B * T + 7) / 8), dim3(256), 0, s, e->hres, e->g16, e->scale, B, S, T, e->s_off, d,
                    e->halves));
  ++nk;
  {
    EpiOutParams p{};
    p.bias = e->b_out;
    p.inpaint_mask = e->inpaint_mask;
    p.inpaint_motion = e->inpaint_motion;
    p.sched = e->sched;
    p.sched_next = e->sched_next;
    p.eps_ring = e->plms_ring;
    p.state = e->state;
    TRY(launch_out_gemm(e->m_g16, e->m_wout, B, T, JF, d, a, p, s, e->num_sms));
    ++nk;
  }
  *n_kernels = nk;
  return B200MDM_OK;
}

static int check_ready(b200mdm_engine* e, bool need_sched) {
  if (!e) return fail(B200MDM_EINVAL, "null engine");
  if (!e->finalized) return fail(B200MDM_ESTATE, "weights not finalised");
  if (!e->cond_set) return fail(B200MDM_ESTATE, "b200mdm_set_cond has not been called");
  if (e->dec && e->ctx > 0 && !e->prefix_set) return fail(B200MDM_ESTATE, "b200mdm_set_prefix has not been called (y['prefix'])");
  if (need_sched && e->n_steps <= 0) return fail(B200MDM_ESTATE, "b200mdm_set_schedule has not been called");
  return B200MDM_OK;
}

extern "C" int b200mdm_denoise(b200mdm_engine* e, const float* x_dev, const int32_t* timesteps_host, float* out_dev,
                               void* stream) {
  TRY(check_ready(e, false));
  if (!x_dev || !timesteps_host || !out_dev) return fail(B200MDM_EINVAL, "null tensor");
  for (int b = 0; b < e->B; ++b)
    if (timesteps_host[b] < 0 || timesteps_host[b] >= e->cfg.temb_rows)
      return fail(B200MDM_EINVAL, "timestep %d outside the pre-embedded range [0, %d)", timesteps_host[b], e->cfg.temb_rows);
  cudaStream_t s = static_cast<cudaStream_t>(stream);
  CUDA_TRY(cudaMemcpyAsync(e->tvec, timesteps_host, e->B * sizeof(int), cudaMemcpyHostToDevice, s));
  CUDA_TRY(cudaStreamSynchronize(s));
  StepArgs a;
  a.mode = B200MDM_MODE_X0;
  a.x_in = x_dev;
  a.x_out = out_dev;
  a.explicit_t = true;
  int nk = 0;
  TRY(enqueue_forward(e, a, s, &nk));
  e->launches += nk;
  return B200MDM_OK;
}

extern "C" int b200mdm_sample_step(b200mdm_engine* e, int32_t mode, int32_t index, const float* x_t_dev,
                                   const float* noise_dev, int32_t flags, float* x_out_dev,
                                   float* pred_xstart_dev, void* stream) {
  TRY(check_ready(e, true));
  const bool reverse = mode == B200MDM_MODE_DDIM_REVERSE;
  if (mode != B200MDM_MODE_DDPM && mode != B200MDM_MODE_DDIM && !reverse) return fail(B200MDM_EINVAL, "bad mode");
  if (index < 0 || index >= e->n_steps) return fail(B200MDM_EINVAL, "schedule index out of range");
  if (!x_t_dev || (!noise_dev && !reverse) || !x_out_dev) return fail(B200MDM_EINVAL, "null tensor");
  if (reverse && (flags & ~B200MDM_FLAG_CLIP_DENOISED))
    return fail(B200MDM_EINVAL, "DDIM inversion takes no flag but B200MDM_FLAG_CLIP_DENOISED");
  if (reverse && !e->sched_next_fresh)
    return fail(B200MDM_ESTATE, "b200mdm_set_schedule_next has not been called for the current schedule");
  cudaStream_t s = static_cast<cudaStream_t>(stream);
  step_set_kernel<<<1, 1, 0, s>>>(e->state, 0, index, nullptr, 0, e->noise_seed, e->noise_sample_base, e->n_steps);
  CUDA_TRY(cudaGetLastError());
  StepArgs a;
  a.mode = mode;
  a.x_in = x_t_dev;
  a.noise = noise_dev;
  a.const_noise = flags & B200MDM_FLAG_CONST_NOISE;
  a.clip = (flags & B200MDM_FLAG_CLIP_DENOISED) ? 1 : 0;
  a.x_out = x_out_dev;
  a.pred = pred_xstart_dev;
  int nk = 0;
  TRY(enqueue_forward(e, a, s, &nk));
  e->launches += nk + 1;
  return B200MDM_OK;
}

static cudaError_t launch_advance(b200mdm_engine* e, const StepArgs& a, cudaStream_t s) {
  PdlScope pdl_scope;
  return launch_k(step_advance_kernel, dim3(1), dim3(1), 0, s, e->state, a.mode == MODE_DDIM_REVERSE ? 1 : -1);
}

static int ensure_step_graph(b200mdm_engine* e, const GraphKey& key, const StepArgs& a) {
  if (e->graph_exec && key == e->graph_key) return B200MDM_OK;
  drop_graph(e);
  cudaGraph_t graph = nullptr;
  CUDA_TRY(cudaStreamBeginCapture(e->work, cudaStreamCaptureModeThreadLocal));
  int nk = 0;
  int r = enqueue_forward(e, a, e->work, &nk);
  if (r == B200MDM_OK && launch_advance(e, a, e->work) != cudaSuccess)
    r = fail(B200MDM_ECUDA, "step_advance launch failed during capture");
  cudaError_t ce = cudaStreamEndCapture(e->work, &graph);
  if (r != B200MDM_OK) {
    if (graph) cudaGraphDestroy(graph);
    return r;
  }
  if (ce != cudaSuccess) return fail(B200MDM_ECUDA, "graph capture failed: %s", cudaGetErrorString(ce));
  ce = cudaGraphInstantiate(&e->graph_exec, graph, 0);
  cudaGraphDestroy(graph);
  if (ce != cudaSuccess) {
    e->graph_exec = nullptr;
    return fail(B200MDM_ECUDA, "graph instantiate failed: %s", cudaGetErrorString(ce));
  }
  e->graph_key = key;
  e->graph_kernels = nk + 1;
  return B200MDM_OK;
}

static int enqueue_step(b200mdm_engine* e, const StepArgs& a, cudaStream_t s, bool use_graph) {
  if (use_graph) {
    CUDA_TRY(cudaGraphLaunch(e->graph_exec, s));
    e->launches += e->graph_kernels;
    return B200MDM_OK;
  }
  int nk = 0;
  TRY(enqueue_forward(e, a, s, &nk));
  CUDA_TRY(launch_advance(e, a, s));
  e->launches += nk + 1;
  return B200MDM_OK;
}

static int enqueue_plms_euler(b200mdm_engine* e, const StepArgs& base, const float* x_t, float* x_out, cudaStream_t s) {
  StepArgs a = base;
  a.mode = MODE_PLMS_EULER1;
  a.x_in = x_t;
  a.x_out = e->plms_mid;
  a.pred = e->plms_pred;
  int nk1 = 0, nk2 = 0;
  TRY(enqueue_forward(e, a, s, &nk1));
  a.mode = MODE_PLMS_EULER2;
  a.x_in = e->plms_mid;
  a.x_step = x_t;
  a.x_out = x_out;
  a.back = 1;
  TRY(enqueue_forward(e, a, s, &nk2));
  CUDA_TRY(launch_advance(e, a, s));
  e->launches += nk1 + nk2 + 1;
  return B200MDM_OK;
}

static int run_loop(b200mdm_engine* e, const StepArgs& a, int32_t flags, int32_t first_index, int32_t n_run,
                    const float* x_in_dev, float* x_out_dev, const float* noise_tape_dev, int64_t noise_step_stride,
                    int32_t use_graph, void* stream, int done = 0, bool plms_euler = false) {
  cudaStream_t user = static_cast<cudaStream_t>(stream);
  const size_t x_bytes = static_cast<size_t>(e->B) * e->JF * e->T * sizeof(float);
  cudaStream_t s = use_graph ? e->work : user;
  if (!use_graph) attach_l2_window(e, user);
  if (use_graph) {
    GraphKey key;
    key.mode = a.mode; key.B = e->B; key.T = e->T; key.flags = flags; key.order = a.order;
    key.imask = e->inpaint_mask; key.imotion = e->inpaint_motion;
    key.target_g = e->target_set ? e->tgt_g : nullptr;
    TRY(ensure_step_graph(e, key, a));
    CUDA_TRY(cudaEventRecord(e->ev_in, user));
    CUDA_TRY(cudaStreamWaitEvent(e->work, e->ev_in, 0));
  }
  e->plms_done = -1;
  if (x_in_dev) CUDA_TRY(cudaMemcpyAsync(e->x_work, x_in_dev, x_bytes, cudaMemcpyDeviceToDevice, s));
  step_set_kernel<<<1, 1, 0, s>>>(e->state, done, first_index, noise_tape_dev, noise_step_stride, e->noise_seed,
                                  e->noise_sample_base, e->n_steps);
  CUDA_TRY(cudaGetLastError());
  e->launches += 1;
  int k = 0;
  if (plms_euler) {
    TRY(enqueue_plms_euler(e, a, e->x_work, e->x_work, s));
    k = 1;
  }
  for (; k < n_run; ++k) TRY(enqueue_step(e, a, s, use_graph));
  if (a.mode == MODE_PLMS_AB) {
    e->plms_done = done + n_run;
    e->plms_order = a.order;
  }
  if (x_out_dev) CUDA_TRY(cudaMemcpyAsync(x_out_dev, e->x_work, x_bytes, cudaMemcpyDeviceToDevice, s));
  if (use_graph) {
    CUDA_TRY(cudaEventRecord(e->ev_out, e->work));
    CUDA_TRY(cudaStreamWaitEvent(user, e->ev_out, 0));
  }
  return B200MDM_OK;
}

extern "C" int b200mdm_sample_loop_range(b200mdm_engine* e, int32_t mode, int32_t first_index, int32_t n_run,
                                         const float* x_in_dev, float* x_out_dev, const float* noise_tape_dev,
                                         int64_t noise_step_stride, int32_t flags, int32_t use_graph, void* stream) {
  TRY(check_ready(e, true));
  if (mode != B200MDM_MODE_DDPM && mode != B200MDM_MODE_DDIM) return fail(B200MDM_EINVAL, "bad mode");
  if (n_run <= 0 || first_index >= e->n_steps || first_index - n_run + 1 < 0) return fail(B200MDM_EINVAL, "bad step range");
  const bool philox = (flags & B200MDM_FLAG_PHILOX_NOISE) != 0;
  if (!philox && !noise_tape_dev) return fail(B200MDM_EINVAL, "null noise tape (or pass B200MDM_FLAG_PHILOX_NOISE)");
  StepArgs a;
  a.mode = mode;
  a.x_in = e->x_work;
  a.x_out = e->x_work;
  a.noise = philox ? e->eps_buf : nullptr;
  a.philox = philox;
  a.const_noise = flags & B200MDM_FLAG_CONST_NOISE;
  a.clip = (flags & B200MDM_FLAG_CLIP_DENOISED) ? 1 : 0;
  return run_loop(e, a, flags, first_index, n_run, x_in_dev, x_out_dev, noise_tape_dev, noise_step_stride, use_graph, stream);
}

extern "C" int b200mdm_sample_loop(b200mdm_engine* e, int32_t mode, int32_t skip_timesteps, const float* x_T_dev,
                                   float* x_0_dev, const float* noise_tape_dev, int64_t noise_step_stride,
                                   int32_t flags, int32_t use_graph, void* stream) {
  TRY(check_ready(e, true));
  if (skip_timesteps < 0 || skip_timesteps >= e->n_steps) return fail(B200MDM_EINVAL, "bad skip_timesteps");
  if (!x_T_dev || !x_0_dev) return fail(B200MDM_EINVAL, "null tensor");
  return b200mdm_sample_loop_range(e, mode, e->n_steps - 1 - skip_timesteps, e->n_steps - skip_timesteps, x_T_dev, x_0_dev,
                                   noise_tape_dev, noise_step_stride, flags, use_graph, stream);
}

extern "C" int b200mdm_ddim_reverse_loop_range(b200mdm_engine* e, int32_t first_index, int32_t n_run, const float* x_in_dev,
                                               float* x_out_dev, int32_t flags, int32_t use_graph, void* stream) {
  if (flags & ~B200MDM_FLAG_CLIP_DENOISED)
    return fail(B200MDM_EINVAL, "DDIM inversion takes no flag but B200MDM_FLAG_CLIP_DENOISED");
  if (n_run <= 0 || first_index < 0) return fail(B200MDM_EINVAL, "bad step range");
  TRY(check_ready(e, true));
  if (n_run > e->n_steps - first_index) return fail(B200MDM_EINVAL, "bad step range");
  if (!e->sched_next_fresh)
    return fail(B200MDM_ESTATE, "b200mdm_set_schedule_next has not been called for the current schedule");
  StepArgs a;
  a.mode = B200MDM_MODE_DDIM_REVERSE;
  a.x_in = e->x_work;
  a.x_out = e->x_work;
  a.clip = (flags & B200MDM_FLAG_CLIP_DENOISED) ? 1 : 0;
  return run_loop(e, a, flags, first_index, n_run, x_in_dev, x_out_dev, nullptr, 0, use_graph, stream);
}

static int ensure_plms(b200mdm_engine* e) {
  if (e->plms_ring && e->plms_mid && e->plms_pred) return B200MDM_OK;
  const size_t n = static_cast<size_t>(e->B) * e->JF * e->T;
  int r = B200MDM_OK;
  if (!e->plms_ring) r = dalloc(&e->plms_ring, PLMS_RING * n);
  if (r == B200MDM_OK && !e->plms_mid) r = dalloc(&e->plms_mid, n);
  if (r == B200MDM_OK && !e->plms_pred) r = dalloc(&e->plms_pred, n);
  if (r != B200MDM_OK) {
    dfree(e->plms_ring); dfree(e->plms_mid); dfree(e->plms_pred);
  }
  return r;
}

extern "C" int b200mdm_plms_loop_range(b200mdm_engine* e, int32_t order, int32_t first_index, int32_t n_run,
                                       const float* x_in_dev, float* x_out_dev, int32_t flags, int32_t use_graph,
                                       void* stream) {
  if (order < 1 || order > 4) return fail(B200MDM_EINVAL, "PLMS order %d is not an integer from 1 to 4", order);
  if (flags & ~B200MDM_FLAG_CLIP_DENOISED) return fail(B200MDM_EINVAL, "PLMS takes no flag but B200MDM_FLAG_CLIP_DENOISED");
  if (x_in_dev && order == 1)
    return fail(B200MDM_EINVAL, "a PLMS loop of order 1 has no first step (the reference needs old_out there)");
  if (n_run <= 0) return fail(B200MDM_EINVAL, "bad step range");
  TRY(check_ready(e, true));
  if (first_index >= e->n_steps || first_index - n_run + 1 < 0) return fail(B200MDM_EINVAL, "bad step range");
  if (!x_in_dev && (e->plms_done < 0 || e->plms_order != order))
    return fail(B200MDM_ESTATE, "no PLMS loop of order %d to continue (pass x_in_dev)", order);
  TRY(ensure_plms(e));
  StepArgs a;
  a.mode = MODE_PLMS_AB;
  a.order = order;
  a.x_in = e->x_work;
  a.x_out = e->x_work;
  a.clip = (flags & B200MDM_FLAG_CLIP_DENOISED) ? 1 : 0;
  const int done = x_in_dev ? 0 : e->plms_done;
  return run_loop(e, a, flags, first_index, n_run, x_in_dev, x_out_dev, nullptr, 0, use_graph, stream, done, done == 0);
}

extern "C" int b200mdm_plms_step(b200mdm_engine* e, int32_t index, int32_t order, const float* x_t_dev,
                                 const float* const* old_eps_dev, int32_t n_old, int32_t flags, float* x_out_dev,
                                 float* pred_xstart_dev, float* eps_out_dev, void* stream) {
  if (order < 1 || order > 4) return fail(B200MDM_EINVAL, "PLMS order %d is not an integer from 1 to 4", order);
  if (flags & ~B200MDM_FLAG_CLIP_DENOISED) return fail(B200MDM_EINVAL, "PLMS takes no flag but B200MDM_FLAG_CLIP_DENOISED");
  const bool euler = old_eps_dev == nullptr;
  if (n_old < 0 || (euler && n_old != 0))
    return fail(B200MDM_EINVAL, "bad eps history (n_old %d with %s array)", n_old, euler ? "a null" : "an");
  if (euler && order == 1)
    return fail(B200MDM_EINVAL, "PLMS of order 1 needs an eps history (the reference needs old_out there)");
  if (!x_t_dev || !x_out_dev) return fail(B200MDM_EINVAL, "null tensor");
  const int h = n_old < PLMS_RING ? n_old : PLMS_RING;
  for (int j = 0; j < h; ++j)
    if (!old_eps_dev[n_old - h + j]) return fail(B200MDM_EINVAL, "null eps history entry %d", n_old - h + j);
  TRY(check_ready(e, true));
  if (index < 0 || index >= e->n_steps) return fail(B200MDM_EINVAL, "schedule index out of range");
  TRY(ensure_plms(e));
  cudaStream_t s = static_cast<cudaStream_t>(stream);
  const size_t n = static_cast<size_t>(e->B) * e->JF * e->T, x_bytes = n * sizeof(float);
  for (int j = 0; j < h; ++j)
    CUDA_TRY(cudaMemcpyAsync(e->plms_ring + j * n, old_eps_dev[n_old - h + j], x_bytes, cudaMemcpyDeviceToDevice, s));
  step_set_kernel<<<1, 1, 0, s>>>(e->state, h, index, nullptr, 0, e->noise_seed, e->noise_sample_base, e->n_steps);
  CUDA_TRY(cudaGetLastError());
  e->launches += 1;
  e->plms_done = -1;
  StepArgs a;
  a.order = order;
  a.clip = (flags & B200MDM_FLAG_CLIP_DENOISED) ? 1 : 0;
  if (euler) {
    TRY(enqueue_plms_euler(e, a, x_t_dev, x_out_dev, s));
    if (pred_xstart_dev) CUDA_TRY(cudaMemcpyAsync(pred_xstart_dev, e->plms_pred, x_bytes, cudaMemcpyDeviceToDevice, s));
  } else {
    a.mode = MODE_PLMS_AB;
    a.x_in = x_t_dev;
    a.x_out = x_out_dev;
    a.pred = pred_xstart_dev;
    int nk = 0;
    TRY(enqueue_forward(e, a, s, &nk));
    e->launches += nk;
  }
  if (eps_out_dev)
    CUDA_TRY(cudaMemcpyAsync(eps_out_dev, e->plms_ring + (h % PLMS_RING) * n, x_bytes, cudaMemcpyDeviceToDevice, s));
  return B200MDM_OK;
}

extern "C" int b200mdm_set_noise_stream(b200mdm_engine* e, uint64_t seed, int64_t sample_index_base) {
  if (!e) return fail(B200MDM_EINVAL, "null engine");
  e->noise_seed = seed;
  e->noise_sample_base = sample_index_base;
  return B200MDM_OK;
}
extern "C" int b200mdm_philox_normal(float* out_dev, int32_t batch, int64_t n_per_sample, uint64_t seed,
                                     int64_t sample_index_base, int32_t step_id, void* stream) {
  if (!out_dev || batch <= 0 || n_per_sample <= 0) return fail(B200MDM_EINVAL, "bad argument");
  const long long quads = (n_per_sample + 3) / 4 * batch;
  const int blocks = static_cast<int>(quads / 256 + 1 < 1184 ? quads / 256 + 1 : 1184);
  philox_normal_kernel<<<blocks, 256, 0, static_cast<cudaStream_t>(stream)>>>(out_dev, batch, n_per_sample, seed, sample_index_base,
                                                                             static_cast<uint32_t>(step_id), nullptr);
  CUDA_TRY(cudaGetLastError());
  return B200MDM_OK;
}

extern "C" int b200mdm_q_sample(b200mdm_engine* e, float sqrt_ac, float sqrt_1mac, const float* x_start_dev,
                                const float* noise_dev, float* out_dev, int64_t n, void* stream) {
  if (!e || !noise_dev || !out_dev || n <= 0) return fail(B200MDM_EINVAL, "bad argument");
  q_sample_kernel<<<592, 256, 0, static_cast<cudaStream_t>(stream)>>>(out_dev, x_start_dev, noise_dev, sqrt_ac, sqrt_1mac,
                                                                     static_cast<size_t>(n));
  CUDA_TRY(cudaGetLastError());
  e->launches++;
  return B200MDM_OK;
}

extern "C" int64_t b200mdm_launch_count(b200mdm_engine* e, int32_t reset) {
  if (!e) return 0;
  long long v = e->launches;
  if (reset) e->launches = 0;
  return v;
}

template <int BN, bool RES = false>
static int test_gemm_bn(const void* a16, const void* w16, const float* bias, void* out16, int M, int N, int K, int act,
                        cudaStream_t s, int sms) {
  CUtensorMap ma, mb, mc;
  TRY(make_map(&ma, a16, M, K, K, GEMM_BLOCK_M));
  TRY(make_map(&mb, w16, N, K, K, BN));
  TRY(make_map_t(&mc, out16, 2, M, N, N, 32));
  EpiBiasF16<true>::Params pg{bias};
  EpiBiasF16<false>::Params pn{bias};
  if constexpr (RES)
    return act ? launch_gemm_resident<BN, EpiBiasF16<true>>(ma, mb, mc, M, N, K, pg, s, sms)
               : launch_gemm_resident<BN, EpiBiasF16<false>>(ma, mb, mc, M, N, K, pn, s, sms);
  else if constexpr (BN == PP_BLOCK_N)
    return act ? launch_gemm_pp<EpiBiasF16<true>>(ma, mb, mc, M, N, K, pg, s, sms)
               : launch_gemm_pp<EpiBiasF16<false>>(ma, mb, mc, M, N, K, pn, s, sms);
  else
    return act ? launch_gemm<BN, EpiBiasF16<true>>(ma, mb, mc, M, N, K, pg, s, sms)
               : launch_gemm<BN, EpiBiasF16<false>>(ma, mb, mc, M, N, K, pn, s, sms);
}

extern "C" int b200mdm_test_gemm_f16(const void* a16_dev, const void* w16_dev, const float* bias_dev, void* out16_dev,
                                     int32_t M, int32_t N, int32_t K, int32_t act, int32_t block_n, void* stream) {
  if (!a16_dev || !w16_dev || !bias_dev || !out16_dev || M <= 0 || N <= 0 || K <= 0 || K % 8 || N % 8)
    return fail(B200MDM_EINVAL, "bad argument (K %% 8 == 0, N %% 8 == 0 required)");
  TRY(init_kernel_attrs());
  int dev = 0, sms = 132;
  CUDA_TRY(cudaGetDevice(&dev));
  CUDA_TRY(cudaDeviceGetAttribute(&sms, cudaDevAttrMultiProcessorCount, dev));
  cudaStream_t s = static_cast<cudaStream_t>(stream);
  if (block_n == 128) return test_gemm_bn<128>(a16_dev, w16_dev, bias_dev, out16_dev, M, N, K, act, s, sms);
  if (block_n == 512) return test_gemm_bn<256>(a16_dev, w16_dev, bias_dev, out16_dev, M, N, K, act, s, sms);
  if (block_n == 513) return test_gemm_bn<64, true>(a16_dev, w16_dev, bias_dev, out16_dev, M, N, K, act, s, sms);
  return fail(B200MDM_EINVAL, "block_n must be 128 (128 x 128 tiles), 512 (128 x 256 tiles) or 513 (W-resident, 128 x 64 tiles)");
}

struct StreamScratch {
  cudaStream_t s;
  std::vector<void*> ptrs;
  explicit StreamScratch(cudaStream_t st) : s(st) {}
  ~StreamScratch() {
    for (void* p : ptrs) cudaFreeAsync(p, s);
  }
  template <class T>
  int alloc(T** p, size_t n, bool zero = false) {
    CUDA_TRY(cudaMallocAsync(reinterpret_cast<void**>(p), n * sizeof(T), s));
    ptrs.push_back(*p);
    if (zero) CUDA_TRY(cudaMemsetAsync(*p, 0, n * sizeof(T), s));
    return B200MDM_OK;
  }
};

static int device_sms(int* sms) {
  int dev = 0;
  CUDA_TRY(cudaGetDevice(&dev));
  CUDA_TRY(cudaDeviceGetAttribute(sms, cudaDevAttrMultiProcessorCount, dev));
  return B200MDM_OK;
}

extern "C" int b200mdm_test_gemm_epi(const void* a16_dev, const void* w16_dev, const float* bias_dev, void* out16_dev,
                                     int32_t M, int32_t N, int32_t K, int32_t epi, void* stream) {
  if (!a16_dev || !w16_dev || !bias_dev || !out16_dev || M <= 0 || N <= 0 || K <= 0 || K % 8)
    return fail(B200MDM_EINVAL, "bad argument (K %% 8 == 0 required)");
  TRY(init_kernel_attrs());
  int sms = 132;
  TRY(device_sms(&sms));
  cudaStream_t s = static_cast<cudaStream_t>(stream);
  CUtensorMap ma, mb, mc;
  TRY(make_map(&ma, a16_dev, M, K, K, GEMM_BLOCK_M));
  TRY(make_map(&mb, w16_dev, N, K, K, 128));
  if (epi == 0) {
    if (N % 64) return fail(B200MDM_EINVAL, "EpiBiasF16Wide needs N %% 64 == 0");
    TRY(make_map_t(&mc, out16_dev, 2, M, 2 * static_cast<uint64_t>(N), 2 * static_cast<uint64_t>(N), 32));
    EpiBiasF16Wide<true>::Params p{bias_dev, N};
    return launch_gemm_pp<EpiBiasF16Wide<true>>(ma, mb, mc, M, N, K, p, s, sms);
  }
  if (epi == 1) {
    if (N % 32) return fail(B200MDM_EINVAL, "EpiBiasF16Global needs N %% 32 == 0");
    TRY(make_map_t(&mc, out16_dev, 2, M, N, N, 32));
    EpiBiasF16Global::Params p{bias_dev};
    return launch_gemm_pp<EpiBiasF16Global>(ma, mb, mc, M, N, K, p, s, sms);
  }
  return fail(B200MDM_EINVAL, "epi must be 0 (EpiBiasF16Wide<GELU>) or 1 (EpiBiasF16Global)");
}

extern "C" int b200mdm_test_embed(const float* x_dev, const float* w_in_dev, const float* b_in_dev, const float* pe_dev,
                                  void* hres16_dev, int32_t B, int32_t JF, int32_t T, int32_t d, int32_t s_off,
                                  int32_t halves, void* stream) {
  if (!x_dev || !w_in_dev || !b_in_dev || !pe_dev || !hres16_dev || B <= 0 || JF <= 0 || T <= 0 || s_off < 0 ||
      d <= 0 || d % 64 || d * 4 > GEMM_BIAS_BYTES || (halves != 1 && halves != 2))
    return fail(B200MDM_EINVAL, "bad argument (d %% 64 == 0, d <= %d, halves 1 or 2)", GEMM_BIAS_BYTES / 4);
  TRY(init_kernel_attrs());
  int sms = 132;
  TRY(device_sms(&sms));
  cudaStream_t s = static_cast<cudaStream_t>(stream);
  const int S = T + s_off, Kp = (JF + 7) & ~7, MB = B * S;
  StreamScratch scr(s);
  __half *xin16 = nullptr, *w_in3 = nullptr;
  float* pe_bias = nullptr;
  TRY(scr.alloc(&xin16, static_cast<size_t>(MB) * 3 * Kp, true));
  TRY(scr.alloc(&w_in3, static_cast<size_t>(d) * 3 * Kp, true));
  TRY(scr.alloc(&pe_bias, static_cast<size_t>(S) * d));
  {
    dim3 grid((T + 31) / 32, (JF + 31) / 32, B), block(32, 8);
    pack_input_kernel<<<grid, block, 0, s>>>(x_dev, xin16, B, JF, T, S, Kp, 3 * Kp, s_off);
    CUDA_TRY(cudaGetLastError());
  }
  split_weight_kernel<<<d, 128, 0, s>>>(w_in_dev, w_in3, d, JF, Kp);
  CUDA_TRY(cudaGetLastError());
  pe_bias_kernel<<<S, 128, 0, s>>>(pe_bias, pe_dev, b_in_dev, S, d);
  CUDA_TRY(cudaGetLastError());
  CUtensorMap m_xin, m_win;
  TRY(make_map(&m_xin, xin16, MB, 3 * Kp, 3 * Kp, GEMM_BLOCK_M));
  TRY(make_map(&m_win, w_in3, d, 3 * Kp, 3 * Kp, 128));
  EpiEmbed::Params p;
  TRY(make_map_res(&p.res_c, hres16_dev, MB, d));
  TRY(make_map_res(&p.res_u, static_cast<__half*>(hres16_dev) + (halves == 2 ? static_cast<size_t>(MB) * d * 2 : 0), MB, d));
  p.pe_bias = pe_bias;
  p.S = S; p.d = d; p.halves = halves;
  return launch_gemm<128, EpiEmbed>(m_xin, m_win, m_xin, MB, d, 3 * Kp, p, s, sms);
}

extern "C" int b200mdm_test_out_step(const void* hres16_dev, const float* scale_dev, const float* w_out_dev,
                                     const float* b_out_dev, const float* x_t_dev, const float* noise_dev,
                                     const float* sched_row_dev, int32_t mode, int32_t flags, const uint8_t* inpaint_mask_dev,
                                     const float* inpaint_motion_dev, float* x_out_dev, float* pred_xstart_dev, int32_t B,
                                     int32_t JF, int32_t T, int32_t d, int32_t s_off, int32_t halves, void* stream) {
  if (!hres16_dev || !w_out_dev || !b_out_dev || !x_t_dev || !x_out_dev || !pred_xstart_dev || B <= 0 || JF <= 0 ||
      T <= 0 || s_off < 0 || d <= 0 || d % 64 || (halves != 1 && halves != 2) || (halves == 2 && !scale_dev) ||
      mode < B200MDM_MODE_X0 || mode > B200MDM_MODE_DDIM || (mode != B200MDM_MODE_X0 && (!noise_dev || !sched_row_dev)) ||
      (inpaint_mask_dev == nullptr) != (inpaint_motion_dev == nullptr))
    return fail(B200MDM_EINVAL, "bad argument");
  TRY(init_kernel_attrs());
  int sms = 132;
  TRY(device_sms(&sms));
  cudaStream_t s = static_cast<cudaStream_t>(stream);
  const int S = T + s_off, N_out_pad = ((JF + 95) / 96) * 96;
  StreamScratch scr(s);
  __half *g16 = nullptr, *w_out3 = nullptr;
  StepState* st = nullptr;
  TRY(scr.alloc(&g16, static_cast<size_t>(B) * T * 3 * d));
  TRY(scr.alloc(&w_out3, static_cast<size_t>(N_out_pad) * 3 * d, true));
  TRY(scr.alloc(&st, 1, true));
  split_weight_kernel<<<JF, 128, 0, s>>>(w_out_dev, w_out3, JF, d, d);
  CUDA_TRY(cudaGetLastError());
  blend_split_kernel<<<(B * T + 7) / 8, 256, 0, s>>>(static_cast<const __half*>(hres16_dev), g16, scale_dev, B, S, T, s_off, d,
                                                     halves);
  CUDA_TRY(cudaGetLastError());
  CUtensorMap m_g16, m_wout;
  TRY(make_map(&m_g16, g16, static_cast<uint64_t>(B) * T, 3 * d, 3 * d, GEMM_BLOCK_M));
  TRY(make_map(&m_wout, w_out3, N_out_pad, 3 * d, 3 * d, 96));
  EpiOutParams p{};
  p.bias = b_out_dev;
  p.inpaint_mask = inpaint_mask_dev;
  p.inpaint_motion = inpaint_motion_dev;
  p.sched = sched_row_dev;
  p.state = st;
  StepArgs a;
  a.mode = mode;
  a.x_in = x_t_dev;
  a.noise = noise_dev;
  a.const_noise = flags & B200MDM_FLAG_CONST_NOISE;
  a.clip = (flags & B200MDM_FLAG_CLIP_DENOISED) ? 1 : 0;
  a.x_out = x_out_dev;
  a.pred = pred_xstart_dev;
  return launch_out_gemm(m_g16, m_wout, B, T, JF, d, a, p, s, sms);
}

extern "C" int b200mdm_test_attention(const void* qkv16_dev, void* out16_dev, const int32_t* kvlen_dev,
                                      int32_t n_samples, int32_t S, int32_t d, int32_t impl, void* stream) {
  if (!qkv16_dev || !out16_dev || !kvlen_dev || n_samples <= 0 || S <= 0) return fail(B200MDM_EINVAL, "bad argument");
  TRY(init_kernel_attrs());
  cudaStream_t s = static_cast<cudaStream_t>(stream);
  if (impl != 0 && impl != 1) return fail(B200MDM_EINVAL, "impl must be 0 (fp16 output) or 1 ([hi | lo] output)");
  if (S > ATC_MAX_KEYS) return fail(B200MDM_EINVAL, "attention handles at most %d tokens", ATC_MAX_KEYS);
  CUtensorMap mkv;
  TRY(make_attention_kv_map(&mkv, qkv16_dev, n_samples, S, 3 * d));
  return launch_attention_tc(mkv, static_cast<const __half*>(qkv16_dev), static_cast<__half*>(out16_dev), kvlen_dev, n_samples,
                             S, d, d / ATC_DH, s, impl == 1);
}

extern "C" int b200mdm_test_cross_attention(const void* q16_dev, const void* kv16_dev, const unsigned char* mask_dev,
                                            void* out16_dev, int32_t n_samples, int32_t S, int32_t n_tokens, int32_t ld_kv,
                                            void* stream) {
  const int d = 512;
  if (!q16_dev || !kv16_dev || !mask_dev || !out16_dev || n_samples <= 0 || S <= 0 || n_tokens <= 0 || n_tokens > XAL_MAX_MT ||
      ld_kv < 2 * d || ld_kv % 8)
    return fail(B200MDM_EINVAL, "bad argument");
  cudaStream_t s = static_cast<cudaStream_t>(stream);
  const float sl2 = 1.4426950408889634f / sqrtf(128.0f);
  const dim3 cg(d / 128, n_samples), cb(128);
  const __half* q = static_cast<const __half*>(q16_dev);
  const __half* kv = static_cast<const __half*>(kv16_dev);
  __half* o = static_cast<__half*>(out16_dev);
  if (n_tokens <= 16) CUDA_TRY(launch_k(cross_attention_kernel<2>, cg, cb, 0, s, q, kv, mask_dev, o, S, n_tokens, d, ld_kv, sl2));
  else if (n_tokens <= 32) CUDA_TRY(launch_k(cross_attention_kernel<4>, cg, cb, 0, s, q, kv, mask_dev, o, S, n_tokens, d, ld_kv, sl2));
  else if (n_tokens <= 64) CUDA_TRY(launch_k(cross_attention_kernel<8>, cg, cb, 0, s, q, kv, mask_dev, o, S, n_tokens, d, ld_kv, sl2));
  else {
    TRY(init_kernel_attrs());
    CUDA_TRY(launch_k(cross_attention_long_kernel, dim3(d / 128, n_samples, (S + XAL_ROWS - 1) / XAL_ROWS), cb, XAL_SMEM, s, q, kv,
                      mask_dev, o, S, n_tokens, d, ld_kv, sl2));
  }
  return B200MDM_OK;
}

extern "C" int b200mdm_test_qkv_attention(const void* h16_dev, int32_t ld, const void* wqkv16_dev, const float* bqkv_dev,
                                          void* out16_dev, const int32_t* kvlen_dev, int32_t n_samples, int32_t S,
                                          void* stream) {
  if (!h16_dev || !wqkv16_dev || !bqkv_dev || !out16_dev || !kvlen_dev || n_samples <= 0 || S <= 0 || S > ATC_MAX_KEYS ||
      ld < 512 || ld % 8)
    return fail(B200MDM_EINVAL, "bad argument");
  TRY(init_kernel_attrs());
  int dev = 0, sms = 132;
  CUDA_TRY(cudaGetDevice(&dev));
  CUDA_TRY(cudaDeviceGetAttribute(&sms, cudaDevAttrMultiProcessorCount, dev));
  cudaStream_t s = static_cast<cudaStream_t>(stream);
  const int M = n_samples * S;
  __half* qkv = nullptr;
  CUDA_TRY(cudaMallocAsync(reinterpret_cast<void**>(&qkv), static_cast<size_t>(M) * 1536 * sizeof(__half), s));
  CUtensorMap ma, mb, mc, mkv;
  int r = make_map(&ma, h16_dev, M, 512, ld, GEMM_BLOCK_M);
  if (r == B200MDM_OK) r = make_map(&mb, wqkv16_dev, 1536, 512, 512, 128);
  if (r == B200MDM_OK) r = make_map_t(&mc, qkv, 2, M, 1536, 1536, 32);
  if (r == B200MDM_OK) r = launch_gemm_bias<false>(ma, mb, mc, M, 1536, 512, bqkv_dev, s, sms);
  if (r == B200MDM_OK) r = make_attention_kv_map(&mkv, qkv, n_samples, S, 1536);
  if (r == B200MDM_OK)
    r = launch_attention_tc(mkv, qkv, static_cast<__half*>(out16_dev), kvlen_dev, n_samples, S, 512, 4, s);
  CUDA_TRY(cudaFreeAsync(qkv, s));
  return r;
}

extern "C" int b200mdm_test_gemm_resid_ln(const void* a16_dev, const void* w16_dev, const float* bias_dev,
                                          const float* gamma_dev, const float* beta_dev, void* hres16_dev, int32_t M,
                                          int32_t K, void* stream) {
  if (!a16_dev || !w16_dev || !bias_dev || !gamma_dev || !beta_dev || !hres16_dev || M <= 0 || K <= 0 || K % 8)
    return fail(B200MDM_EINVAL, "bad argument");
  TRY(init_kernel_attrs());
  int dev = 0, sms = 132;
  CUDA_TRY(cudaGetDevice(&dev));
  CUDA_TRY(cudaDeviceGetAttribute(&sms, cudaDevAttrMultiProcessorCount, dev));
  CUtensorMap ma, mb, mh;
  TRY(make_map(&ma, a16_dev, M, K, K, GEMM_BLOCK_M));
  TRY(make_map(&mb, w16_dev, GLN_D, K, K, 256));
  TRY(make_hres_map(&mh, hres16_dev, M));
  return launch_gemm_resid_ln(ma, mb, mh, M, K, bias_dev, gamma_dev, beta_dev, static_cast<cudaStream_t>(stream), sms);
}

extern "C" int b200mdm_test_cross_rows(b200mdm_engine* e, int32_t timestep, float* out_dev, void* stream) {
  if (!e || !out_dev) return fail(B200MDM_EINVAL, "bad argument");
  if (!e->dec_clip) return fail(B200MDM_EINVAL, "cross-attention rows belong to trans_dec engines with a CLIP memory");
  if (!e->finalized || !e->cond_set) return fail(B200MDM_ESTATE, "weights and b200mdm_set_cond_dec first");
  if (timestep < 0 || timestep >= e->cfg.temb_rows) return fail(B200MDM_EINVAL, "timestep outside [0, %d)", e->cfg.temb_rows);
  cudaStream_t s = static_cast<cudaStream_t>(stream);
  std::vector<int> t(e->B, timestep);
  CUDA_TRY(cudaMemcpyAsync(e->tvec, t.data(), e->B * sizeof(int), cudaMemcpyHostToDevice, s));
  cross_rows_kernel<<<dim3(e->Bp, e->L), 128, 0, s>>>(out_dev, e->cross_b, e->cross_t, e->tvec, e->tmap, e->state, e->B, e->Bp,
                                                      e->d, e->cfg.temb_rows, 0);
  CUDA_TRY(cudaGetLastError());
  CUDA_TRY(cudaStreamSynchronize(s));
  return B200MDM_OK;
}

extern "C" int b200mdm_test_row_bias_ln(void* hres16_dev, const float* c_dev, const float* gamma_dev, const float* beta_dev,
                                        int32_t M, int32_t S, void* stream) {
  if (!hres16_dev || !c_dev || !gamma_dev || !beta_dev || M <= 0 || S <= 0) return fail(B200MDM_EINVAL, "bad argument");
  if ((reinterpret_cast<uintptr_t>(hres16_dev) | reinterpret_cast<uintptr_t>(c_dev) | reinterpret_cast<uintptr_t>(gamma_dev) |
       reinterpret_cast<uintptr_t>(beta_dev)) & 15)
    return fail(B200MDM_EINVAL, "operands must be 16-byte aligned");
  row_bias_ln_kernel<<<(M + RBLN_ROWS_PER_CTA - 1) / RBLN_ROWS_PER_CTA, 32 * RBLN_ROWS_PER_CTA, 0, static_cast<cudaStream_t>(stream)>>>(
      static_cast<__half*>(hres16_dev), c_dev, gamma_dev, beta_dev, M, S, 1e-5f);
  CUDA_TRY(cudaGetLastError());
  return B200MDM_OK;
}

#ifdef B200_TRACE
extern "C" int b200mdm_debug_ln_trace(uint64_t* host_out, int32_t* dims) {
  if (!dims) return fail(B200MDM_EINVAL, "bad argument");
  dims[0] = GLN_TRACE_CTAS; dims[1] = GLN_TRACE_ITERS; dims[2] = GLN_TRACE_ROLES; dims[3] = GLN_TRACE_EVENTS;
  if (host_out) {
    CUDA_TRY(cudaDeviceSynchronize());
    CUDA_TRY(cudaMemcpyFromSymbol(host_out, g_gln_trace, sizeof(g_gln_trace)));
    void* dev = nullptr;
    CUDA_TRY(cudaGetSymbolAddress(&dev, g_gln_trace));
    CUDA_TRY(cudaMemset(dev, 0, sizeof(g_gln_trace)));
    CUDA_TRY(cudaDeviceSynchronize());
  }
  return B200MDM_OK;
}
#endif

extern "C" int b200mdm_recover_from_ric(const float* data_dev, int64_t stride_b, int64_t stride_f, int64_t stride_t,
                                        const float* mean_dev, const float* std_dev, float* out_dev, int64_t ostride_b,
                                        int64_t ostride_t, int64_t ostride_c, int32_t batch, int32_t nframes,
                                        int32_t njoints, void* stream) {
  if (!data_dev || !out_dev || batch <= 0 || nframes <= 0 || njoints < 2) return fail(B200MDM_EINVAL, "bad argument");
  if ((mean_dev == nullptr) != (std_dev == nullptr)) return fail(B200MDM_EINVAL, "mean and std come together");
  const size_t smem = static_cast<size_t>(nframes) * 7 * sizeof(float);
  if (smem > 48 * 1024) return fail(B200MDM_ENOTIMPL, "recover_from_ric: %d frames exceed the single-CTA scan", nframes);
  RicArgs a;
  a.x = data_dev; a.xb = stride_b; a.xf = stride_f; a.xt = stride_t;
  a.mean = mean_dev; a.std = std_dev;
  a.out = out_dev; a.ob = ostride_b; a.ot = ostride_t; a.oc = ostride_c;
  a.T = nframes; a.joints = njoints;
  recover_from_ric_kernel<<<batch, 256, smem, static_cast<cudaStream_t>(stream)>>>(a);
  CUDA_TRY(cudaGetLastError());
  return B200MDM_OK;
}

extern "C" int b200mdm_test_target(b200mdm_engine* e, const float* target_dev, const uint8_t* valid_host, int32_t batch,
                                   float* out_dev, void* stream) {
  if (!e || !target_dev || !valid_host || !out_dev || batch <= 0) return fail(B200MDM_EINVAL, "bad argument");
  if (e->cfg.target_encoder == B200MDM_TARGET_NONE) return fail(B200MDM_EINVAL, "this engine has no target encoder");
  if (!e->finalized) return fail(B200MDM_ESTATE, "weights not finalised");
  cudaStream_t s = static_cast<cudaStream_t>(stream);
  float* valid = nullptr;
  CUDA_TRY(cudaMallocAsync(reinterpret_cast<void**>(&valid), static_cast<size_t>(batch) * e->cfg.target_joints * sizeof(float), s));
  std::vector<float> staging;
  const int r = encode_target(e, target_dev, valid_host, batch, valid, out_dev, staging, s);
  cudaFreeAsync(valid, s);
  CUDA_TRY(cudaStreamSynchronize(s));
  return r;
}
```

### motion-diffusion-model_b200/csrc/wgmma_ops.inc

```
template <> struct Wgmma<64> {
  static constexpr int NREG = 32;
  static __device__ __forceinline__ void mma(float (&d)[32], uint64_t da, uint64_t db, uint32_t accumulate) {
    asm volatile(
        "{\n\t.reg .pred p;\n\tsetp.ne.b32 p, %34, 0;\n\t"
        "wgmma.mma_async.sync.aligned.m64n64k16.f32.f16.f16 {%0, %1, %2, %3, %4, %5, %6, %7, %8, %9, %10, %11, %12, %13, %14, %15, %16, %17, %18, %19, %20, %21, %22, %23, %24, %25, %26, %27, %28, %29, %30, %31}, %32, %33, p, 1, 1, 0, 0;\n\t}\n"
        : "+f"(d[0]), "+f"(d[1]), "+f"(d[2]), "+f"(d[3]), "+f"(d[4]), "+f"(d[5]), "+f"(d[6]), "+f"(d[7]), "+f"(d[8]), "+f"(d[9]), "+f"(d[10]), "+f"(d[11]), "+f"(d[12]), "+f"(d[13]), "+f"(d[14]), "+f"(d[15]), "+f"(d[16]), "+f"(d[17]), "+f"(d[18]), "+f"(d[19]), "+f"(d[20]), "+f"(d[21]), "+f"(d[22]), "+f"(d[23]), "+f"(d[24]), "+f"(d[25]), "+f"(d[26]), "+f"(d[27]), "+f"(d[28]), "+f"(d[29]), "+f"(d[30]), "+f"(d[31])
        : "l"(da), "l"(db), "r"(accumulate));
  }
};
template <> struct Wgmma<96> {
  static constexpr int NREG = 48;
  static __device__ __forceinline__ void mma(float (&d)[48], uint64_t da, uint64_t db, uint32_t accumulate) {
    asm volatile(
        "{\n\t.reg .pred p;\n\tsetp.ne.b32 p, %50, 0;\n\t"
        "wgmma.mma_async.sync.aligned.m64n96k16.f32.f16.f16 {%0, %1, %2, %3, %4, %5, %6, %7, %8, %9, %10, %11, %12, %13, %14, %15, %16, %17, %18, %19, %20, %21, %22, %23, %24, %25, %26, %27, %28, %29, %30, %31, %32, %33, %34, %35, %36, %37, %38, %39, %40, %41, %42, %43, %44, %45, %46, %47}, %48, %49, p, 1, 1, 0, 0;\n\t}\n"
        : "+f"(d[0]), "+f"(d[1]), "+f"(d[2]), "+f"(d[3]), "+f"(d[4]), "+f"(d[5]), "+f"(d[6]), "+f"(d[7]), "+f"(d[8]), "+f"(d[9]), "+f"(d[10]), "+f"(d[11]), "+f"(d[12]), "+f"(d[13]), "+f"(d[14]), "+f"(d[15]), "+f"(d[16]), "+f"(d[17]), "+f"(d[18]), "+f"(d[19]), "+f"(d[20]), "+f"(d[21]), "+f"(d[22]), "+f"(d[23]), "+f"(d[24]), "+f"(d[25]), "+f"(d[26]), "+f"(d[27]), "+f"(d[28]), "+f"(d[29]), "+f"(d[30]), "+f"(d[31]), "+f"(d[32]), "+f"(d[33]), "+f"(d[34]), "+f"(d[35]), "+f"(d[36]), "+f"(d[37]), "+f"(d[38]), "+f"(d[39]), "+f"(d[40]), "+f"(d[41]), "+f"(d[42]), "+f"(d[43]), "+f"(d[44]), "+f"(d[45]), "+f"(d[46]), "+f"(d[47])
        : "l"(da), "l"(db), "r"(accumulate));
  }
};
template <> struct Wgmma<128> {
  static constexpr int NREG = 64;
  static __device__ __forceinline__ void mma(float (&d)[64], uint64_t da, uint64_t db, uint32_t accumulate) {
    asm volatile(
        "{\n\t.reg .pred p;\n\tsetp.ne.b32 p, %66, 0;\n\t"
        "wgmma.mma_async.sync.aligned.m64n128k16.f32.f16.f16 {%0, %1, %2, %3, %4, %5, %6, %7, %8, %9, %10, %11, %12, %13, %14, %15, %16, %17, %18, %19, %20, %21, %22, %23, %24, %25, %26, %27, %28, %29, %30, %31, %32, %33, %34, %35, %36, %37, %38, %39, %40, %41, %42, %43, %44, %45, %46, %47, %48, %49, %50, %51, %52, %53, %54, %55, %56, %57, %58, %59, %60, %61, %62, %63}, %64, %65, p, 1, 1, 0, 0;\n\t}\n"
        : "+f"(d[0]), "+f"(d[1]), "+f"(d[2]), "+f"(d[3]), "+f"(d[4]), "+f"(d[5]), "+f"(d[6]), "+f"(d[7]), "+f"(d[8]), "+f"(d[9]), "+f"(d[10]), "+f"(d[11]), "+f"(d[12]), "+f"(d[13]), "+f"(d[14]), "+f"(d[15]), "+f"(d[16]), "+f"(d[17]), "+f"(d[18]), "+f"(d[19]), "+f"(d[20]), "+f"(d[21]), "+f"(d[22]), "+f"(d[23]), "+f"(d[24]), "+f"(d[25]), "+f"(d[26]), "+f"(d[27]), "+f"(d[28]), "+f"(d[29]), "+f"(d[30]), "+f"(d[31]), "+f"(d[32]), "+f"(d[33]), "+f"(d[34]), "+f"(d[35]), "+f"(d[36]), "+f"(d[37]), "+f"(d[38]), "+f"(d[39]), "+f"(d[40]), "+f"(d[41]), "+f"(d[42]), "+f"(d[43]), "+f"(d[44]), "+f"(d[45]), "+f"(d[46]), "+f"(d[47]), "+f"(d[48]), "+f"(d[49]), "+f"(d[50]), "+f"(d[51]), "+f"(d[52]), "+f"(d[53]), "+f"(d[54]), "+f"(d[55]), "+f"(d[56]), "+f"(d[57]), "+f"(d[58]), "+f"(d[59]), "+f"(d[60]), "+f"(d[61]), "+f"(d[62]), "+f"(d[63])
        : "l"(da), "l"(db), "r"(accumulate));
  }
};
template <> struct Wgmma<256> {
  static constexpr int NREG = 128;
  static __device__ __forceinline__ void mma(float (&d)[128], uint64_t da, uint64_t db, uint32_t accumulate) {
    asm volatile(
        "{\n\t.reg .pred p;\n\tsetp.ne.b32 p, %130, 0;\n\t"
        "wgmma.mma_async.sync.aligned.m64n256k16.f32.f16.f16 {%0, %1, %2, %3, %4, %5, %6, %7, %8, %9, %10, %11, %12, %13, %14, %15, %16, %17, %18, %19, %20, %21, %22, %23, %24, %25, %26, %27, %28, %29, %30, %31, %32, %33, %34, %35, %36, %37, %38, %39, %40, %41, %42, %43, %44, %45, %46, %47, %48, %49, %50, %51, %52, %53, %54, %55, %56, %57, %58, %59, %60, %61, %62, %63, %64, %65, %66, %67, %68, %69, %70, %71, %72, %73, %74, %75, %76, %77, %78, %79, %80, %81, %82, %83, %84, %85, %86, %87, %88, %89, %90, %91, %92, %93, %94, %95, %96, %97, %98, %99, %100, %101, %102, %103, %104, %105, %106, %107, %108, %109, %110, %111, %112, %113, %114, %115, %116, %117, %118, %119, %120, %121, %122, %123, %124, %125, %126, %127}, %128, %129, p, 1, 1, 0, 0;\n\t}\n"
        : "+f"(d[0]), "+f"(d[1]), "+f"(d[2]), "+f"(d[3]), "+f"(d[4]), "+f"(d[5]), "+f"(d[6]), "+f"(d[7]), "+f"(d[8]), "+f"(d[9]), "+f"(d[10]), "+f"(d[11]), "+f"(d[12]), "+f"(d[13]), "+f"(d[14]), "+f"(d[15]), "+f"(d[16]), "+f"(d[17]), "+f"(d[18]), "+f"(d[19]), "+f"(d[20]), "+f"(d[21]), "+f"(d[22]), "+f"(d[23]), "+f"(d[24]), "+f"(d[25]), "+f"(d[26]), "+f"(d[27]), "+f"(d[28]), "+f"(d[29]), "+f"(d[30]), "+f"(d[31]), "+f"(d[32]), "+f"(d[33]), "+f"(d[34]), "+f"(d[35]), "+f"(d[36]), "+f"(d[37]), "+f"(d[38]), "+f"(d[39]), "+f"(d[40]), "+f"(d[41]), "+f"(d[42]), "+f"(d[43]), "+f"(d[44]), "+f"(d[45]), "+f"(d[46]), "+f"(d[47]), "+f"(d[48]), "+f"(d[49]), "+f"(d[50]), "+f"(d[51]), "+f"(d[52]), "+f"(d[53]), "+f"(d[54]), "+f"(d[55]), "+f"(d[56]), "+f"(d[57]), "+f"(d[58]), "+f"(d[59]), "+f"(d[60]), "+f"(d[61]), "+f"(d[62]), "+f"(d[63]), "+f"(d[64]), "+f"(d[65]), "+f"(d[66]), "+f"(d[67]), "+f"(d[68]), "+f"(d[69]), "+f"(d[70]), "+f"(d[71]), "+f"(d[72]), "+f"(d[73]), "+f"(d[74]), "+f"(d[75]), "+f"(d[76]), "+f"(d[77]), "+f"(d[78]), "+f"(d[79]), "+f"(d[80]), "+f"(d[81]), "+f"(d[82]), "+f"(d[83]), "+f"(d[84]), "+f"(d[85]), "+f"(d[86]), "+f"(d[87]), "+f"(d[88]), "+f"(d[89]), "+f"(d[90]), "+f"(d[91]), "+f"(d[92]), "+f"(d[93]), "+f"(d[94]), "+f"(d[95]), "+f"(d[96]), "+f"(d[97]), "+f"(d[98]), "+f"(d[99]), "+f"(d[100]), "+f"(d[101]), "+f"(d[102]), "+f"(d[103]), "+f"(d[104]), "+f"(d[105]), "+f"(d[106]), "+f"(d[107]), "+f"(d[108]), "+f"(d[109]), "+f"(d[110]), "+f"(d[111]), "+f"(d[112]), "+f"(d[113]), "+f"(d[114]), "+f"(d[115]), "+f"(d[116]), "+f"(d[117]), "+f"(d[118]), "+f"(d[119]), "+f"(d[120]), "+f"(d[121]), "+f"(d[122]), "+f"(d[123]), "+f"(d[124]), "+f"(d[125]), "+f"(d[126]), "+f"(d[127])
        : "l"(da), "l"(db), "r"(accumulate));
  }
};
template <> struct WgmmaRA<64, 0> {
  static constexpr int NREG = 32;
  static __device__ __forceinline__ void mma(float (&d)[32], const uint32_t (&a)[4], uint64_t db, uint32_t accumulate) {
    asm volatile(
        "{\n\t.reg .pred p;\n\tsetp.ne.b32 p, %37, 0;\n\t"
        "wgmma.mma_async.sync.aligned.m64n64k16.f32.f16.f16 {%0, %1, %2, %3, %4, %5, %6, %7, %8, %9, %10, %11, %12, %13, %14, %15, %16, %17, %18, %19, %20, %21, %22, %23, %24, %25, %26, %27, %28, %29, %30, %31}, {%32, %33, %34, %35}, %36, p, 1, 1, 0;\n\t}\n"
        : "+f"(d[0]), "+f"(d[1]), "+f"(d[2]), "+f"(d[3]), "+f"(d[4]), "+f"(d[5]), "+f"(d[6]), "+f"(d[7]), "+f"(d[8]), "+f"(d[9]), "+f"(d[10]), "+f"(d[11]), "+f"(d[12]), "+f"(d[13]), "+f"(d[14]), "+f"(d[15]), "+f"(d[16]), "+f"(d[17]), "+f"(d[18]), "+f"(d[19]), "+f"(d[20]), "+f"(d[21]), "+f"(d[22]), "+f"(d[23]), "+f"(d[24]), "+f"(d[25]), "+f"(d[26]), "+f"(d[27]), "+f"(d[28]), "+f"(d[29]), "+f"(d[30]), "+f"(d[31])
        : "r"(a[0]), "r"(a[1]), "r"(a[2]), "r"(a[3]), "l"(db), "r"(accumulate));
  }
};
template <> struct WgmmaRA<208, 0> {
  static constexpr int NREG = 104;
  static __device__ __forceinline__ void mma(float (&d)[104], const uint32_t (&a)[4], uint64_t db, uint32_t accumulate) {
    asm volatile(
        "{\n\t.reg .pred p;\n\tsetp.ne.b32 p, %109, 0;\n\t"
        "wgmma.mma_async.sync.aligned.m64n208k16.f32.f16.f16 {%0, %1, %2, %3, %4, %5, %6, %7, %8, %9, %10, %11, %12, %13, %14, %15, %16, %17, %18, %19, %20, %21, %22, %23, %24, %25, %26, %27, %28, %29, %30, %31, %32, %33, %34, %35, %36, %37, %38, %39, %40, %41, %42, %43, %44, %45, %46, %47, %48, %49, %50, %51, %52, %53, %54, %55, %56, %57, %58, %59, %60, %61, %62, %63, %64, %65, %66, %67, %68, %69, %70, %71, %72, %73, %74, %75, %76, %77, %78, %79, %80, %81, %82, %83, %84, %85, %86, %87, %88, %89, %90, %91, %92, %93, %94, %95, %96, %97, %98, %99, %100, %101, %102, %103}, {%104, %105, %106, %107}, %108, p, 1, 1, 0;\n\t}\n"
        : "+f"(d[0]), "+f"(d[1]), "+f"(d[2]), "+f"(d[3]), "+f"(d[4]), "+f"(d[5]), "+f"(d[6]), "+f"(d[7]), "+f"(d[8]), "+f"(d[9]), "+f"(d[10]), "+f"(d[11]), "+f"(d[12]), "+f"(d[13]), "+f"(d[14]), "+f"(d[15]), "+f"(d[16]), "+f"(d[17]), "+f"(d[18]), "+f"(d[19]), "+f"(d[20]), "+f"(d[21]), "+f"(d[22]), "+f"(d[23]), "+f"(d[24]), "+f"(d[25]), "+f"(d[26]), "+f"(d[27]), "+f"(d[28]), "+f"(d[29]), "+f"(d[30]), "+f"(d[31]), "+f"(d[32]), "+f"(d[33]), "+f"(d[34]), "+f"(d[35]), "+f"(d[36]), "+f"(d[37]), "+f"(d[38]), "+f"(d[39]), "+f"(d[40]), "+f"(d[41]), "+f"(d[42]), "+f"(d[43]), "+f"(d[44]), "+f"(d[45]), "+f"(d[46]), "+f"(d[47]), "+f"(d[48]), "+f"(d[49]), "+f"(d[50]), "+f"(d[51]), "+f"(d[52]), "+f"(d[53]), "+f"(d[54]), "+f"(d[55]), "+f"(d[56]), "+f"(d[57]), "+f"(d[58]), "+f"(d[59]), "+f"(d[60]), "+f"(d[61]), "+f"(d[62]), "+f"(d[63]), "+f"(d[64]), "+f"(d[65]), "+f"(d[66]), "+f"(d[67]), "+f"(d[68]), "+f"(d[69]), "+f"(d[70]), "+f"(d[71]), "+f"(d[72]), "+f"(d[73]), "+f"(d[74]), "+f"(d[75]), "+f"(d[76]), "+f"(d[77]), "+f"(d[78]), "+f"(d[79]), "+f"(d[80]), "+f"(d[81]), "+f"(d[82]), "+f"(d[83]), "+f"(d[84]), "+f"(d[85]), "+f"(d[86]), "+f"(d[87]), "+f"(d[88]), "+f"(d[89]), "+f"(d[90]), "+f"(d[91]), "+f"(d[92]), "+f"(d[93]), "+f"(d[94]), "+f"(d[95]), "+f"(d[96]), "+f"(d[97]), "+f"(d[98]), "+f"(d[99]), "+f"(d[100]), "+f"(d[101]), "+f"(d[102]), "+f"(d[103])
        : "r"(a[0]), "r"(a[1]), "r"(a[2]), "r"(a[3]), "l"(db), "r"(accumulate));
  }
};
template <> struct WgmmaRA<256, 0> {
  static constexpr int NREG = 128;
  static __device__ __forceinline__ void mma(float (&d)[128], const uint32_t (&a)[4], uint64_t db, uint32_t accumulate) {
    asm volatile(
        "{\n\t.reg .pred p;\n\tsetp.ne.b32 p, %133, 0;\n\t"
        "wgmma.mma_async.sync.aligned.m64n256k16.f32.f16.f16 {%0, %1, %2, %3, %4, %5, %6, %7, %8, %9, %10, %11, %12, %13, %14, %15, %16, %17, %18, %19, %20, %21, %22, %23, %24, %25, %26, %27, %28, %29, %30, %31, %32, %33, %34, %35, %36, %37, %38, %39, %40, %41, %42, %43, %44, %45, %46, %47, %48, %49, %50, %51, %52, %53, %54, %55, %56, %57, %58, %59, %60, %61, %62, %63, %64, %65, %66, %67, %68, %69, %70, %71, %72, %73, %74, %75, %76, %77, %78, %79, %80, %81, %82, %83, %84, %85, %86, %87, %88, %89, %90, %91, %92, %93, %94, %95, %96, %97, %98, %99, %100, %101, %102, %103, %104, %105, %106, %107, %108, %109, %110, %111, %112, %113, %114, %115, %116, %117, %118, %119, %120, %121, %122, %123, %124, %125, %126, %127}, {%128, %129, %130, %131}, %132, p, 1, 1, 0;\n\t}\n"
        : "+f"(d[0]), "+f"(d[1]), "+f"(d[2]), "+f"(d[3]), "+f"(d[4]), "+f"(d[5]), "+f"(d[6]), "+f"(d[7]), "+f"(d[8]), "+f"(d[9]), "+f"(d[10]), "+f"(d[11]), "+f"(d[12]), "+f"(d[13]), "+f"(d[14]), "+f"(d[15]), "+f"(d[16]), "+f"(d[17]), "+f"(d[18]), "+f"(d[19]), "+f"(d[20]), "+f"(d[21]), "+f"(d[22]), "+f"(d[23]), "+f"(d[24]), "+f"(d[25]), "+f"(d[26]), "+f"(d[27]), "+f"(d[28]), "+f"(d[29]), "+f"(d[30]), "+f"(d[31]), "+f"(d[32]), "+f"(d[33]), "+f"(d[34]), "+f"(d[35]), "+f"(d[36]), "+f"(d[37]), "+f"(d[38]), "+f"(d[39]), "+f"(d[40]), "+f"(d[41]), "+f"(d[42]), "+f"(d[43]), "+f"(d[44]), "+f"(d[45]), "+f"(d[46]), "+f"(d[47]), "+f"(d[48]), "+f"(d[49]), "+f"(d[50]), "+f"(d[51]), "+f"(d[52]), "+f"(d[53]), "+f"(d[54]), "+f"(d[55]), "+f"(d[56]), "+f"(d[57]), "+f"(d[58]), "+f"(d[59]), "+f"(d[60]), "+f"(d[61]), "+f"(d[62]), "+f"(d[63]), "+f"(d[64]), "+f"(d[65]), "+f"(d[66]), "+f"(d[67]), "+f"(d[68]), "+f"(d[69]), "+f"(d[70]), "+f"(d[71]), "+f"(d[72]), "+f"(d[73]), "+f"(d[74]), "+f"(d[75]), "+f"(d[76]), "+f"(d[77]), "+f"(d[78]), "+f"(d[79]), "+f"(d[80]), "+f"(d[81]), "+f"(d[82]), "+f"(d[83]), "+f"(d[84]), "+f"(d[85]), "+f"(d[86]), "+f"(d[87]), "+f"(d[88]), "+f"(d[89]), "+f"(d[90]), "+f"(d[91]), "+f"(d[92]), "+f"(d[93]), "+f"(d[94]), "+f"(d[95]), "+f"(d[96]), "+f"(d[97]), "+f"(d[98]), "+f"(d[99]), "+f"(d[100]), "+f"(d[101]), "+f"(d[102]), "+f"(d[103]), "+f"(d[104]), "+f"(d[105]), "+f"(d[106]), "+f"(d[107]), "+f"(d[108]), "+f"(d[109]), "+f"(d[110]), "+f"(d[111]), "+f"(d[112]), "+f"(d[113]), "+f"(d[114]), "+f"(d[115]), "+f"(d[116]), "+f"(d[117]), "+f"(d[118]), "+f"(d[119]), "+f"(d[120]), "+f"(d[121]), "+f"(d[122]), "+f"(d[123]), "+f"(d[124]), "+f"(d[125]), "+f"(d[126]), "+f"(d[127])
        : "r"(a[0]), "r"(a[1]), "r"(a[2]), "r"(a[3]), "l"(db), "r"(accumulate));
  }
};
template <> struct WgmmaRA<128, 1> {
  static constexpr int NREG = 64;
  static __device__ __forceinline__ void mma(float (&d)[64], const uint32_t (&a)[4], uint64_t db, uint32_t accumulate) {
    asm volatile(
        "{\n\t.reg .pred p;\n\tsetp.ne.b32 p, %69, 0;\n\t"
        "wgmma.mma_async.sync.aligned.m64n128k16.f32.f16.f16 {%0, %1, %2, %3, %4, %5, %6, %7, %8, %9, %10, %11, %12, %13, %14, %15, %16, %17, %18, %19, %20, %21, %22, %23, %24, %25, %26, %27, %28, %29, %30, %31, %32, %33, %34, %35, %36, %37, %38, %39, %40, %41, %42, %43, %44, %45, %46, %47, %48, %49, %50, %51, %52, %53, %54, %55, %56, %57, %58, %59, %60, %61, %62, %63}, {%64, %65, %66, %67}, %68, p, 1, 1, 1;\n\t}\n"
        : "+f"(d[0]), "+f"(d[1]), "+f"(d[2]), "+f"(d[3]), "+f"(d[4]), "+f"(d[5]), "+f"(d[6]), "+f"(d[7]), "+f"(d[8]), "+f"(d[9]), "+f"(d[10]), "+f"(d[11]), "+f"(d[12]), "+f"(d[13]), "+f"(d[14]), "+f"(d[15]), "+f"(d[16]), "+f"(d[17]), "+f"(d[18]), "+f"(d[19]), "+f"(d[20]), "+f"(d[21]), "+f"(d[22]), "+f"(d[23]), "+f"(d[24]), "+f"(d[25]), "+f"(d[26]), "+f"(d[27]), "+f"(d[28]), "+f"(d[29]), "+f"(d[30]), "+f"(d[31]), "+f"(d[32]), "+f"(d[33]), "+f"(d[34]), "+f"(d[35]), "+f"(d[36]), "+f"(d[37]), "+f"(d[38]), "+f"(d[39]), "+f"(d[40]), "+f"(d[41]), "+f"(d[42]), "+f"(d[43]), "+f"(d[44]), "+f"(d[45]), "+f"(d[46]), "+f"(d[47]), "+f"(d[48]), "+f"(d[49]), "+f"(d[50]), "+f"(d[51]), "+f"(d[52]), "+f"(d[53]), "+f"(d[54]), "+f"(d[55]), "+f"(d[56]), "+f"(d[57]), "+f"(d[58]), "+f"(d[59]), "+f"(d[60]), "+f"(d[61]), "+f"(d[62]), "+f"(d[63])
        : "r"(a[0]), "r"(a[1]), "r"(a[2]), "r"(a[3]), "l"(db), "r"(accumulate));
  }
};
```

Baseline: 426.7.

## Make attention a persistent warp-specialized kernel with TMA Q loads and KV ring

Replaces the per-(head,sample) attention kernel with a persistent kernel. One producer warpgroup issues TMA loads of K, V and Q tiles into a multi-slot shared-memory ring guarded by full/empty mbarriers. Two consumer warpgroups, given more registers via setmaxnreg, run the QK^T and PV wgmma using Q taken straight from shared memory instead of register fragments. The aim is to overlap the loads of the next unit with compute and to cut launch and tail overhead. The cost is one CTA per SM, larger shared-memory use and more complex barrier phase logic.

After: 434.3 (median of 6 runs). 1.8% higher.

```diff
diff --git a/motion-diffusion-model_b200/csrc/attention_tc.cuh b/motion-diffusion-model_b200/csrc/attention_tc.cuh
--- a/motion-diffusion-model_b200/csrc/attention_tc.cuh
+++ b/motion-diffusion-model_b200/csrc/attention_tc.cuh
@@ -6,151 +6,205 @@
 
 namespace b200 {
 
-constexpr int ATC_THREADS = 128;
+constexpr int ATC_THREADS = 384;
 constexpr int ATC_QROWS = 64;
-constexpr int ATC_TILES_PER_CTA = 4;
 constexpr int ATC_DH = 128;
 constexpr int ATC_MAX_KEYS = 256;
+constexpr int ATC_REGS_PRODUCER = 40, ATC_REGS_CONSUMER = 232;
 
 __host__ __device__ constexpr int atc_keys(int S) { return S <= 64 ? 64 : S <= 208 ? 208 : 256; }
 
+template <int KEYS>
 struct AttnTcSmem {
-  static __host__ __device__ int total(int keys) { return 1024 + 4 * keys * 128; }
+  static constexpr int ATOM = KEYS * 128;
+  static constexpr int SLOT = 2 * ATOM;
+  static constexpr int NSLOT = KEYS == 64 ? 8 : 3;
+  static constexpr int QATOM = ATC_QROWS * 128;
+  static constexpr int QSTAGE = 2 * QATOM;
+  static constexpr int NQ = KEYS == 256 ? 2 : 4;
+  static constexpr int BAR_OFF = NSLOT * SLOT + NQ * QSTAGE;
+  static constexpr int TOTAL = 1024 + BAR_OFF + 2 * (NSLOT + NQ) * 8;
+  static_assert(TOTAL <= 232448, "shared-memory budget of one CTA");
 };
 
 template <int KEYS, bool WIDE>
-__global__ void __launch_bounds__(ATC_THREADS, 2)
-attention_tc_kernel(const __grid_constant__ CUtensorMap map_kv, const __half* __restrict__ qkv, __half* __restrict__ out,
-                    const int* __restrict__ kvlen, int S, int d, float scale_log2) {
-  constexpr int ATOM = KEYS * 128;
+__global__ void __launch_bounds__(ATC_THREADS, 1)
+attention_tc_persistent(const __grid_constant__ CUtensorMap map_kv, const __grid_constant__ CUtensorMap map_q,
+                        __half* __restrict__ out, const int* __restrict__ kvlen, int n_units, int H, int S,
+                        float scale_log2) {
+  using SM = AttnTcSmem<KEYS>;
+  constexpr int ATOM = SM::ATOM, SLOT = SM::SLOT, NSLOT = SM::NSLOT, QATOM = SM::QATOM, QSTAGE = SM::QSTAGE, NQ = SM::NQ;
+  constexpr int QPER = NQ / 2;
+  constexpr bool SPLIT = KEYS != 64;
   constexpr int NS = KEYS / 2;
   constexpr int NB = KEYS / 16;
   extern __shared__ uint8_t smem_raw[];
-  __shared__ uint64_t bar_k, bar_v;
-  uint8_t* sK = reinterpret_cast<uint8_t*>((reinterpret_cast<uintptr_t>(smem_raw) + 1023) & ~uintptr_t(1023));
-  uint8_t* sV = sK + 2 * ATOM;
+  uint8_t* smem = smem_raw + ((1024u - (smem_u32(smem_raw) & 1023u)) & 1023u);
+  uint8_t* ring = smem;
+  uint8_t* qst = smem + NSLOT * SLOT;
+  uint64_t* kv_full = reinterpret_cast<uint64_t*>(smem + SM::BAR_OFF);
+  uint64_t* kv_empty = kv_full + NSLOT;
+  uint64_t* q_full = kv_empty + NSLOT;
+  uint64_t* q_empty = q_full + NQ;
   const int warp = threadIdx.x >> 5, lane = threadIdx.x & 31;
-  const int h = blockIdx.x, smp = blockIdx.y;
-  const int ld = 3 * d;
-  const __half* base = qkv + static_cast<size_t>(smp) * S * ld;
+  const int d = H * ATC_DH;
+  const int ntiles = (S + ATC_QROWS - 1) / ATC_QROWS;
+  const int my_units = static_cast<int>(blockIdx.x) < n_units ? (n_units - 1 - blockIdx.x) / gridDim.x + 1 : 0;
 
   pdl_launch_dependents();
   if (threadIdx.x == 0) {
     tma_prefetch_desc(&map_kv);
-    mbar_init(&bar_k, 1);
-    mbar_init(&bar_v, 1);
+    tma_prefetch_desc(&map_q);
+    for (int s = 0; s < NSLOT; ++s) {
+      mbar_init(&kv_full[s], 1);
+      mbar_init(&kv_empty[s], SPLIT ? 8 : 4);
+    }
+    for (int s = 0; s < NQ; ++s) {
+      mbar_init(&q_full[s], 1);
+      mbar_init(&q_empty[s], 4);
+    }
     fence_barrier_init();
   }
   __syncthreads();
   pdl_wait();
-  if (threadIdx.x == 0) {
-    mbar_expect_tx(&bar_k, 2 * ATOM);
-    for (int a = 0; a < 2; ++a) tma_load_3d(sK + a * ATOM, &map_kv, &bar_k, d + h * ATC_DH + 64 * a, 0, smp);
-    mbar_expect_tx(&bar_v, 2 * ATOM);
-    for (int a = 0; a < 2; ++a) tma_load_3d(sV + a * ATOM, &map_kv, &bar_v, 2 * d + h * ATC_DH + 64 * a, 0, smp);
-  }
-
-  const int kvl = min(kvlen[smp], S);
-  const int nblk = max(1, (kvl + 15) >> 4);
-  const int g = lane >> 2, t = lane & 3;
-  const uint64_t desc_k = wgmma_desc_k_sw128(smem_u32(sK));
-  const uint64_t desc_v = wgmma_desc_mn_sw128(smem_u32(sV), ATOM);
-  const int ntiles = (S + ATC_QROWS - 1) / ATC_QROWS;
-  const int ldo = (WIDE ? 2 : 1) * d;
-
-  uint32_t qa[8][4];
-  auto load_q = [&](int tile) {
-    const int ra = tile * ATC_QROWS + warp * 16 + g, rb = ra + 8;
-    const bool va = ra < S, vb = rb < S;
-    const uint32_t* pa = reinterpret_cast<const uint32_t*>(base + static_cast<size_t>(va ? ra : 0) * ld + h * ATC_DH);
-    const uint32_t* pb = reinterpret_cast<const uint32_t*>(base + static_cast<size_t>(vb ? rb : 0) * ld + h * ATC_DH);
-#pragma unroll
-    for (int ks = 0; ks < 8; ++ks) {
-      qa[ks][0] = va ? pa[8 * ks + t] : 0u;
-      qa[ks][1] = vb ? pb[8 * ks + t] : 0u;
-      qa[ks][2] = va ? pa[8 * ks + 4 + t] : 0u;
-      qa[ks][3] = vb ? pb[8 * ks + 4 + t] : 0u;
-    }
-  };
-  if (static_cast<int>(blockIdx.z) < ntiles) load_q(blockIdx.z);
+
+  if (warp < 4) {
+    asm volatile("setmaxnreg.dec.sync.aligned.u32 %0;" ::"n"(ATC_REGS_PRODUCER));
+    if (warp == 0 && elect_one()) {
+      int qn0 = 0, qn1 = 0;
+      for (int i = 0; i < my_units; ++i) {
+        const int u = blockIdx.x + i * gridDim.x;
+        const int smp = u / H, h = u - smp * H;
+        auto load_kv = [&](int item, int col) {
+          const int slot = item % NSLOT;
+          mbar_wait(&kv_empty[slot], ((item / NSLOT) & 1) ^ 1);
+          mbar_expect_tx(&kv_full[slot], SLOT);
+          for (int a = 0; a < 2; ++a)
+            tma_load_3d(ring + slot * SLOT + a * ATOM, &map_kv, &kv_full[slot], col + 64 * a, 0, smp);
+        };
+        auto load_q = [&](int tile) {
+          const int c = SPLIT ? (tile & 1) : (i & 1);
+          const int k = c ? qn1++ : qn0++;
+          const int st = c * QPER + k % QPER;
+          mbar_wait(&q_empty[st], ((k / QPER) & 1) ^ 1);
+          mbar_expect_tx(&q_full[st], QSTAGE);
+          for (int a = 0; a < 2; ++a)
+            tma_load_3d(qst + st * QSTAGE + a * QATOM, &map_q, &q_full[st], h * ATC_DH + 64 * a, tile * ATC_QROWS, smp);
+        };
+        load_kv(2 * i, d + h * ATC_DH);
+        for (int tile = 0; tile < min(2, ntiles); ++tile) load_q(tile);
+        load_kv(2 * i + 1, 2 * d + h * ATC_DH);
+        for (int tile = 2; tile < ntiles; ++tile) load_q(tile);
+      }
+    }
+  } else {
+    asm volatile("setmaxnreg.inc.sync.aligned.u32 %0;" ::"n"(ATC_REGS_CONSUMER));
+    const int wg = (warp >> 2) - 1;
+    const int wq = warp & 3;
+    const int g = lane >> 2, t = lane & 3;
+    const int ldo = (WIDE ? 2 : 1) * d;
+    const int tile0 = SPLIT ? wg : 0, tstep = SPLIT ? 2 : 1;
+    int qn = 0;
 #pragma unroll 1
-  for (int tile = blockIdx.z; tile < ntiles; tile += gridDim.z) {
-    const int ra = tile * ATC_QROWS + warp * 16 + g, rb = ra + 8;
-    const bool va = ra < S, vb = rb < S;
-    float s[NS];
-    mbar_wait(&bar_k, 0);
-    wgmma_fence();
-#pragma unroll
-    for (int ks = 0; ks < 8; ++ks)
-      WgmmaRA<KEYS, 0>::mma(s, qa[ks], desc_k + (((ks >> 2) * ATOM + (ks & 3) * 32) >> 4), ks != 0);
-    wgmma_commit();
-    wgmma_wait<0>();
-    wgmma_fence_acc(s);
-    float mxa = -INFINITY, mxb = -INFINITY;
-#pragma unroll
-    for (int j = 0; j < NS / 4; ++j)
-#pragma unroll
-      for (int i = 0; i < 2; ++i) {
-        if (8 * j + 2 * t + i < kvl) {
-          mxa = fmaxf(mxa, s[4 * j + i]);
-          mxb = fmaxf(mxb, s[4 * j + 2 + i]);
-        }
-      }
-#pragma unroll
-    for (int o = 1; o < 4; o <<= 1) {
-      mxa = fmaxf(mxa, __shfl_xor_sync(0xffffffffu, mxa, o));
-      mxb = fmaxf(mxb, __shfl_xor_sync(0xffffffffu, mxb, o));
-    }
-    const float offa = (mxa == -INFINITY) ? 0.f : mxa * scale_log2;
-    const float offb = (mxb == -INFINITY) ? 0.f : mxb * scale_log2;
-    auto ex2 = [](float x) {
-      float y;
-      asm("ex2.approx.ftz.f32 %0, %1;" : "=f"(y) : "f"(x));
-      return y;
-    };
-    uint32_t p[NB][4];
-    float suma = 0.f, sumb = 0.f;
-#pragma unroll
-    for (int j = 0; j < NS / 4; ++j) {
-      const int key = 8 * j + 2 * t;
-      const float p0 = key < kvl ? ex2(fmaf(s[4 * j], scale_log2, -offa)) : 0.f;
-      const float p1 = key + 1 < kvl ? ex2(fmaf(s[4 * j + 1], scale_log2, -offa)) : 0.f;
-      const float p2 = key < kvl ? ex2(fmaf(s[4 * j + 2], scale_log2, -offb)) : 0.f;
-      const float p3 = key + 1 < kvl ? ex2(fmaf(s[4 * j + 3], scale_log2, -offb)) : 0.f;
-      suma += p0 + p1;
-      sumb += p2 + p3;
-      p[j >> 1][2 * (j & 1)] = pack_half2(p0, p1);
-      p[j >> 1][2 * (j & 1) + 1] = pack_half2(p2, p3);
-    }
-#pragma unroll
-    for (int off = 1; off < 4; off <<= 1) {
-      suma += __shfl_xor_sync(0xffffffffu, suma, off);
-      sumb += __shfl_xor_sync(0xffffffffu, sumb, off);
-    }
-    const float inva = suma > 0.f ? 1.f / suma : 0.f;
-    const float invb = sumb > 0.f ? 1.f / sumb : 0.f;
-    float o[64];
-    mbar_wait(&bar_v, 0);
-    wgmma_fence();
-#pragma unroll
-    for (int kk = 0; kk < NB; ++kk)
-      if (kk < nblk) WgmmaRA<128, 1>::mma(o, p[kk], desc_v + ((kk * 16 * 128) >> 4), kk != 0);
-    wgmma_commit();
-    if (tile + static_cast<int>(gridDim.z) < ntiles) load_q(tile + gridDim.z);
-    wgmma_wait<0>();
-    wgmma_fence_acc(o);
-    __half* oa = out + (static_cast<size_t>(smp) * S + (va ? ra : 0)) * ldo + h * ATC_DH + 2 * t;
-    __half* ob = out + (static_cast<size_t>(smp) * S + (vb ? rb : 0)) * ldo + h * ATC_DH + 2 * t;
-#pragma unroll
-    for (int j = 0; j < 16; ++j) {
-      const float x0 = o[4 * j] * inva, x1 = o[4 * j + 1] * inva, x2 = o[4 * j + 2] * invb, x3 = o[4 * j + 3] * invb;
-      const __half2 ha = __floats2half2_rn(x0, x1), hb = __floats2half2_rn(x2, x3);
-      if (va) *reinterpret_cast<__half2*>(oa + 8 * j) = ha;
-      if (vb) *reinterpret_cast<__half2*>(ob + 8 * j) = hb;
-      if (WIDE) {
-        const float2 fa = __half22float2(ha), fb = __half22float2(hb);
-        if (va) *reinterpret_cast<__half2*>(oa + d + 8 * j) = __floats2half2_rn(x0 - fa.x, x1 - fa.y);
-        if (vb) *reinterpret_cast<__half2*>(ob + d + 8 * j) = __floats2half2_rn(x2 - fb.x, x3 - fb.y);
+    for (int i = SPLIT ? 0 : wg; i < my_units; i += SPLIT ? 1 : 2) {
+      const int u = blockIdx.x + i * gridDim.x;
+      const int smp = u / H, h = u - smp * H;
+      const int kvl = min(kvlen[smp], S);
+      const int slot_k = (2 * i) % NSLOT, slot_v = (2 * i + 1) % NSLOT;
+      const uint32_t ph_k = ((2 * i) / NSLOT) & 1, ph_v = ((2 * i + 1) / NSLOT) & 1;
+      const uint64_t desc_k = wgmma_desc_k_sw128(smem_u32(ring + slot_k * SLOT));
+      const uint64_t desc_v = wgmma_desc_mn_sw128(smem_u32(ring + slot_v * SLOT), ATOM);
+#pragma unroll 1
+      for (int tile = tile0; tile < ntiles; tile += tstep) {
+        const bool last = tile + tstep >= ntiles;
+        const int st = wg * QPER + qn % QPER;
+        const uint32_t ph_q = (qn / QPER) & 1;
+        ++qn;
+        const int ra = tile * ATC_QROWS + wq * 16 + g, rb = ra + 8;
+        const bool va = ra < S, vb = rb < S;
+        float s[NS];
+        const uint64_t desc_q = wgmma_desc_k_sw128(smem_u32(qst + st * QSTAGE));
+        mbar_wait(&kv_full[slot_k], ph_k);
+        mbar_wait(&q_full[st], ph_q);
+        wgmma_fence();
+#pragma unroll
+        for (int ks = 0; ks < 8; ++ks)
+          Wgmma<KEYS>::mma(s, desc_q + (((ks >> 2) * QATOM + (ks & 3) * 32) >> 4),
+                           desc_k + (((ks >> 2) * ATOM + (ks & 3) * 32) >> 4), ks != 0);
+        wgmma_commit();
+        wgmma_wait<0>();
+        wgmma_fence_acc(s);
+        if (lane == 0) {
+          mbar_arrive(&q_empty[st]);
+          if (last) mbar_arrive(&kv_empty[slot_k]);
+        }
+        float mxa = -INFINITY, mxb = -INFINITY;
+#pragma unroll
+        for (int j = 0; j < NS / 4; ++j)
+#pragma unroll
+          for (int e = 0; e < 2; ++e) {
+            if (8 * j + 2 * t + e < kvl) {
+              mxa = fmaxf(mxa, s[4 * j + e]);
+              mxb = fmaxf(mxb, s[4 * j + 2 + e]);
+            }
+          }
+#pragma unroll
+        for (int o = 1; o < 4; o <<= 1) {
+          mxa = fmaxf(mxa, __shfl_xor_sync(0xffffffffu, mxa, o));
+          mxb = fmaxf(mxb, __shfl_xor_sync(0xffffffffu, mxb, o));
+        }
+        const float offa = (mxa == -INFINITY) ? 0.f : mxa * scale_log2;
+        const float offb = (mxb == -INFINITY) ? 0.f : mxb * scale_log2;
+        auto ex2 = [](float x) {
+          float y;
+          asm("ex2.approx.ftz.f32 %0, %1;" : "=f"(y) : "f"(x));
+          return y;
+        };
+        uint32_t p[NB][4];
+        float suma = 0.f, sumb = 0.f;
+#pragma unroll
+        for (int j = 0; j < NS / 4; ++j) {
+          const int key = 8 * j + 2 * t;
+          const float p0 = key < kvl ? ex2(fmaf(s[4 * j], scale_log2, -offa)) : 0.f;
+          const float p1 = key + 1 < kvl ? ex2(fmaf(s[4 * j + 1], scale_log2, -offa)) : 0.f;
+          const float p2 = key < kvl ? ex2(fmaf(s[4 * j + 2], scale_log2, -offb)) : 0.f;
+          const float p3 = key + 1 < kvl ? ex2(fmaf(s[4 * j + 3], scale_log2, -offb)) : 0.f;
+          suma += p0 + p1;
+          sumb += p2 + p3;
+          p[j >> 1][2 * (j & 1)] = pack_half2(p0, p1);
+          p[j >> 1][2 * (j & 1) + 1] = pack_half2(p2, p3);
+        }
+#pragma unroll
+        for (int off = 1; off < 4; off <<= 1) {
+          suma += __shfl_xor_sync(0xffffffffu, suma, off);
+          sumb += __shfl_xor_sync(0xffffffffu, sumb, off);
+        }
+        const float inva = suma > 0.f ? 1.f / suma : 0.f;
+        const float invb = sumb > 0.f ? 1.f / sumb : 0.f;
+        float o[64];
+        mbar_wait(&kv_full[slot_v], ph_v);
+        wgmma_fence();
+#pragma unroll
+        for (int kk = 0; kk < NB; ++kk)
+          WgmmaRA<128, 1>::mma(o, p[kk], desc_v + ((kk * 16 * 128) >> 4), kk != 0);
+        wgmma_commit();
+        wgmma_wait<0>();
+        wgmma_fence_acc(o);
+        if (last && lane == 0) mbar_arrive(&kv_empty[slot_v]);
+        __half* oa = out + (static_cast<size_t>(smp) * S + (va ? ra : 0)) * ldo + h * ATC_DH + 2 * t;
+        __half* ob = out + (static_cast<size_t>(smp) * S + (vb ? rb : 0)) * ldo + h * ATC_DH + 2 * t;
+#pragma unroll
+        for (int j = 0; j < 16; ++j) {
+          const float x0 = o[4 * j] * inva, x1 = o[4 * j + 1] * inva, x2 = o[4 * j + 2] * invb, x3 = o[4 * j + 3] * invb;
+          const __half2 ha = __floats2half2_rn(x0, x1), hb = __floats2half2_rn(x2, x3);
+          if (va) *reinterpret_cast<__half2*>(oa + 8 * j) = ha;
+          if (vb) *reinterpret_cast<__half2*>(ob + 8 * j) = hb;
+          if (WIDE) {
+            const float2 fa = __half22float2(ha), fb = __half22float2(hb);
+            if (va) *reinterpret_cast<__half2*>(oa + d + 8 * j) = __floats2half2_rn(x0 - fa.x, x1 - fa.y);
+            if (vb) *reinterpret_cast<__half2*>(ob + d + 8 * j) = __floats2half2_rn(x2 - fb.x, x3 - fb.y);
+          }
+        }
       }
     }
   }
diff --git a/motion-diffusion-model_b200/csrc/engine.cu b/motion-diffusion-model_b200/csrc/engine.cu
--- a/motion-diffusion-model_b200/csrc/engine.cu
+++ b/motion-diffusion-model_b200/csrc/engine.cu
@@ -140,6 +140,7 @@
   CUtensorMap m_xin, m_h16, m_att, m_ffn, m_g16;
   CUtensorMap m_qkv_st, m_ffn_st;
   CUtensorMap m_qkv_kv;
+  CUtensorMap m_qkv_q;
   CUtensorMap m_res_c, m_res_u;
   CUtensorMap m_hres;
   float* pe_bias = nullptr;
@@ -231,10 +232,10 @@
 }
 template <int KEYS>
 static int set_attention_attr() {
-  CUDA_TRY(cudaFuncSetAttribute(attention_tc_kernel<KEYS, false>, cudaFuncAttributeMaxDynamicSharedMemorySize,
-                                AttnTcSmem::total(KEYS)));
-  CUDA_TRY(cudaFuncSetAttribute(attention_tc_kernel<KEYS, true>, cudaFuncAttributeMaxDynamicSharedMemorySize,
-                                AttnTcSmem::total(KEYS)));
+  CUDA_TRY(cudaFuncSetAttribute(attention_tc_persistent<KEYS, false>, cudaFuncAttributeMaxDynamicSharedMemorySize,
+                                AttnTcSmem<KEYS>::TOTAL));
+  CUDA_TRY(cudaFuncSetAttribute(attention_tc_persistent<KEYS, true>, cudaFuncAttributeMaxDynamicSharedMemorySize,
+                                AttnTcSmem<KEYS>::TOTAL));
   return B200MDM_OK;
 }
 static int init_kernel_attrs() {
@@ -346,23 +347,26 @@
 static int make_attention_kv_map(CUtensorMap* m, const void* qkv, int n_samples, int S, int ld) {
   return make_map_3d(m, qkv, n_samples, S, ld, ld, atc_keys(S));
 }
+static int make_attention_q_map(CUtensorMap* m, const void* qkv, int n_samples, int S, int ld) {
+  return make_map_3d(m, qkv, n_samples, S, ld, ld, ATC_QROWS);
+}
 template <int KEYS>
-static cudaError_t launch_attention_keys(const CUtensorMap& map_kv, const __half* qkv, __half* out, const int* kvlen,
-                                         dim3 grid, int S, int d, float scale_log2, cudaStream_t s, bool wide) {
-  return launch_k(wide ? attention_tc_kernel<KEYS, true> : attention_tc_kernel<KEYS, false>, grid, dim3(ATC_THREADS),
-                  AttnTcSmem::total(KEYS), s, map_kv, qkv, out, kvlen, S, d, scale_log2);
-}
-static int launch_attention_tc(const CUtensorMap& map_kv, const __half* qkv, __half* out, const int* kvlen, int n_samples,
-                               int S, int d, int H, cudaStream_t s, bool wide = false) {
+static cudaError_t launch_attention_keys(const CUtensorMap& map_kv, const CUtensorMap& map_q, __half* out,
+                                         const int* kvlen, int n_units, int H, int S, float scale_log2, cudaStream_t s,
+                                         int num_sms, bool wide) {
+  const int grid = n_units < num_sms ? n_units : num_sms;
+  return launch_k(wide ? attention_tc_persistent<KEYS, true> : attention_tc_persistent<KEYS, false>, dim3(grid),
+                  dim3(ATC_THREADS), AttnTcSmem<KEYS>::TOTAL, s, map_kv, map_q, out, kvlen, n_units, H, S, scale_log2);
+}
+static int launch_attention_tc(const CUtensorMap& map_kv, const CUtensorMap& map_q, __half* out, const int* kvlen,
+                               int n_samples, int S, int d, int H, cudaStream_t s, int num_sms, bool wide = false) {
   if (d != H * ATC_DH) return fail(B200MDM_ENOTIMPL, "attention: head_dim must be 128");
   if (S > ATC_MAX_KEYS) return fail(B200MDM_ENOTIMPL, "attention: at most %d tokens per sample", ATC_MAX_KEYS);
   const float scale_log2 = 1.4426950408889634f / sqrtf(static_cast<float>(ATC_DH));
-  const int tiles = (S + ATC_QROWS - 1) / ATC_QROWS;
-  const dim3 grid(H, n_samples, (tiles + ATC_TILES_PER_CTA - 1) / ATC_TILES_PER_CTA);
-  const int keys = atc_keys(S);
-  if (keys == 64) CUDA_TRY(launch_attention_keys<64>(map_kv, qkv, out, kvlen, grid, S, d, scale_log2, s, wide));
-  else if (keys == 208) CUDA_TRY(launch_attention_keys<208>(map_kv, qkv, out, kvlen, grid, S, d, scale_log2, s, wide));
-  else CUDA_TRY(launch_attention_keys<256>(map_kv, qkv, out, kvlen, grid, S, d, scale_log2, s, wide));
+  const int units = n_samples * H, keys = atc_keys(S);
+  if (keys == 64) CUDA_TRY(launch_attention_keys<64>(map_kv, map_q, out, kvlen, units, H, S, scale_log2, s, num_sms, wide));
+  else if (keys == 208) CUDA_TRY(launch_attention_keys<208>(map_kv, map_q, out, kvlen, units, H, S, scale_log2, s, num_sms, wide));
+  else CUDA_TRY(launch_attention_keys<256>(map_kv, map_q, out, kvlen, units, H, S, scale_log2, s, num_sms, wide));
   return B200MDM_OK;
 }
 #ifdef B200_TRACE
@@ -846,6 +850,7 @@
   TRY(make_map(&e->m_g16, e->g16, static_cast<size_t>(B) * T, 3 * d, 3 * d, GEMM_BLOCK_M));
   TRY(make_map_t(&e->m_qkv_st, e->qkv16, 2, M, 3 * d, 3 * d, 32));
   TRY(make_attention_kv_map(&e->m_qkv_kv, e->qkv16, Bp, S, 3 * d));
+  TRY(make_attention_q_map(&e->m_qkv_q, e->qkv16, Bp, S, 3 * d));
   TRY(make_map_t(&e->m_ffn_st, e->ffn16, 2, M, kw * e->ff, kw * e->ff, 32));
   TRY(make_map_res(&e->m_res_c, e->hres, MB, d));
   TRY(make_map_res(&e->m_res_u, e->hres + (halves == 2 ? MB * d * 2 : 0), MB, d));
@@ -1213,7 +1218,7 @@
       {
         TRY((launch_gemm_bias<false>(e->m_h16, w.m_wqkv, e->m_qkv_st, e->M, 3 * d, d, w.bqkv, s, e->num_sms)));
       }
-      TRY(launch_attention_tc(e->m_qkv_kv, e->qkv16, e->att16, e->kvlen, e->Bp, S, d, e->H, s, wide));
+      TRY(launch_attention_tc(e->m_qkv_kv, e->m_qkv_q, e->att16, e->kvlen, e->Bp, S, d, e->H, s, e->num_sms, wide));
     }
     if (!B200_SKIP(2)) TRY(launch_gemm_resid_ln(e->m_att, w.m_wo_256, e->m_hres, e->M, kw * d, w.bo, w.g1, w.be1, s, e->num_sms));
     if (e->dec_clip) {
@@ -1766,10 +1771,14 @@
   cudaStream_t s = static_cast<cudaStream_t>(stream);
   if (impl != 0 && impl != 1) return fail(B200MDM_EINVAL, "impl must be 0 (fp16 output) or 1 ([hi | lo] output)");
   if (S > ATC_MAX_KEYS) return fail(B200MDM_EINVAL, "attention handles at most %d tokens", ATC_MAX_KEYS);
-  CUtensorMap mkv;
+  int dev = 0, sms = 132;
+  CUDA_TRY(cudaGetDevice(&dev));
+  CUDA_TRY(cudaDeviceGetAttribute(&sms, cudaDevAttrMultiProcessorCount, dev));
+  CUtensorMap mkv, mq;
   TRY(make_attention_kv_map(&mkv, qkv16_dev, n_samples, S, 3 * d));
-  return launch_attention_tc(mkv, static_cast<const __half*>(qkv16_dev), static_cast<__half*>(out16_dev), kvlen_dev, n_samples,
-                             S, d, d / ATC_DH, s, impl == 1);
+  TRY(make_attention_q_map(&mq, qkv16_dev, n_samples, S, 3 * d));
+  return launch_attention_tc(mkv, mq, static_cast<__half*>(out16_dev), kvlen_dev, n_samples, S, d, d / ATC_DH, s, sms,
+                             impl == 1);
 }
 
 extern "C" int b200mdm_test_cross_attention(const void* q16_dev, const void* kv16_dev, const unsigned char* mask_dev,
@@ -1810,14 +1819,15 @@
   const int M = n_samples * S;
   __half* qkv = nullptr;
   CUDA_TRY(cudaMallocAsync(reinterpret_cast<void**>(&qkv), static_cast<size_t>(M) * 1536 * sizeof(__half), s));
-  CUtensorMap ma, mb, mc, mkv;
+  CUtensorMap ma, mb, mc, mkv, mq;
   int r = make_map(&ma, h16_dev, M, 512, ld, GEMM_BLOCK_M);
   if (r == B200MDM_OK) r = make_map(&mb, wqkv16_dev, 1536, 512, 512, 128);
   if (r == B200MDM_OK) r = make_map_t(&mc, qkv, 2, M, 1536, 1536, 32);
   if (r == B200MDM_OK) r = launch_gemm_bias<false>(ma, mb, mc, M, 1536, 512, bqkv_dev, s, sms);
   if (r == B200MDM_OK) r = make_attention_kv_map(&mkv, qkv, n_samples, S, 1536);
+  if (r == B200MDM_OK) r = make_attention_q_map(&mq, qkv, n_samples, S, 1536);
   if (r == B200MDM_OK)
-    r = launch_attention_tc(mkv, qkv, static_cast<__half*>(out16_dev), kvlen_dev, n_samples, S, 512, 4, s);
+    r = launch_attention_tc(mkv, mq, static_cast<__half*>(out16_dev), kvlen_dev, n_samples, S, 512, 4, s, sms);
   CUDA_TRY(cudaFreeAsync(qkv, s));
   return r;
 }
diff --git a/motion-diffusion-model_b200/csrc/wgmma_ops.inc b/motion-diffusion-model_b200/csrc/wgmma_ops.inc
--- a/motion-diffusion-model_b200/csrc/wgmma_ops.inc
+++ b/motion-diffusion-model_b200/csrc/wgmma_ops.inc
@@ -28,6 +28,16 @@
         : "l"(da), "l"(db), "r"(accumulate));
   }
 };
+template <> struct Wgmma<208> {
+  static constexpr int NREG = 104;
+  static __device__ __forceinline__ void mma(float (&d)[104], uint64_t da, uint64_t db, uint32_t accumulate) {
+    asm volatile(
+        "{\n\t.reg .pred p;\n\tsetp.ne.b32 p, %106, 0;\n\t"
+        "wgmma.mma_async.sync.aligned.m64n208k16.f32.f16.f16 {%0, %1, %2, %3, %4, %5, %6, %7, %8, %9, %10, %11, %12, %13, %14, %15, %16, %17, %18, %19, %20, %21, %22, %23, %24, %25, %26, %27, %28, %29, %30, %31, %32, %33, %34, %35, %36, %37, %38, %39, %40, %41, %42, %43, %44, %45, %46, %47, %48, %49, %50, %51, %52, %53, %54, %55, %56, %57, %58, %59, %60, %61, %62, %63, %64, %65, %66, %67, %68, %69, %70, %71, %72, %73, %74, %75, %76, %77, %78, %79, %80, %81, %82, %83, %84, %85, %86, %87, %88, %89, %90, %91, %92, %93, %94, %95, %96, %97, %98, %99, %100, %101, %102, %103}, %104, %105, p, 1, 1, 0, 0;\n\t}\n"
+        : "+f"(d[0]), "+f"(d[1]), "+f"(d[2]), "+f"(d[3]), "+f"(d[4]), "+f"(d[5]), "+f"(d[6]), "+f"(d[7]), "+f"(d[8]), "+f"(d[9]), "+f"(d[10]), "+f"(d[11]), "+f"(d[12]), "+f"(d[13]), "+f"(d[14]), "+f"(d[15]), "+f"(d[16]), "+f"(d[17]), "+f"(d[18]), "+f"(d[19]), "+f"(d[20]), "+f"(d[21]), "+f"(d[22]), "+f"(d[23]), "+f"(d[24]), "+f"(d[25]), "+f"(d[26]), "+f"(d[27]), "+f"(d[28]), "+f"(d[29]), "+f"(d[30]), "+f"(d[31]), "+f"(d[32]), "+f"(d[33]), "+f"(d[34]), "+f"(d[35]), "+f"(d[36]), "+f"(d[37]), "+f"(d[38]), "+f"(d[39]), "+f"(d[40]), "+f"(d[41]), "+f"(d[42]), "+f"(d[43]), "+f"(d[44]), "+f"(d[45]), "+f"(d[46]), "+f"(d[47]), "+f"(d[48]), "+f"(d[49]), "+f"(d[50]), "+f"(d[51]), "+f"(d[52]), "+f"(d[53]), "+f"(d[54]), "+f"(d[55]), "+f"(d[56]), "+f"(d[57]), "+f"(d[58]), "+f"(d[59]), "+f"(d[60]), "+f"(d[61]), "+f"(d[62]), "+f"(d[63]), "+f"(d[64]), "+f"(d[65]), "+f"(d[66]), "+f"(d[67]), "+f"(d[68]), "+f"(d[69]), "+f"(d[70]), "+f"(d[71]), "+f"(d[72]), "+f"(d[73]), "+f"(d[74]), "+f"(d[75]), "+f"(d[76]), "+f"(d[77]), "+f"(d[78]), "+f"(d[79]), "+f"(d[80]), "+f"(d[81]), "+f"(d[82]), "+f"(d[83]), "+f"(d[84]), "+f"(d[85]), "+f"(d[86]), "+f"(d[87]), "+f"(d[88]), "+f"(d[89]), "+f"(d[90]), "+f"(d[91]), "+f"(d[92]), "+f"(d[93]), "+f"(d[94]), "+f"(d[95]), "+f"(d[96]), "+f"(d[97]), "+f"(d[98]), "+f"(d[99]), "+f"(d[100]), "+f"(d[101]), "+f"(d[102]), "+f"(d[103])
+        : "l"(da), "l"(db), "r"(accumulate));
+  }
+};
 template <> struct Wgmma<256> {
   static constexpr int NREG = 128;
   static __device__ __forceinline__ void mma(float (&d)[128], uint64_t da, uint64_t db, uint32_t accumulate) {
@@ -36,36 +46,6 @@
         "wgmma.mma_async.sync.aligned.m64n256k16.f32.f16.f16 {%0, %1, %2, %3, %4, %5, %6, %7, %8, %9, %10, %11, %12, %13, %14, %15, %16, %17, %18, %19, %20, %21, %22, %23, %24, %25, %26, %27, %28, %29, %30, %31, %32, %33, %34, %35, %36, %37, %38, %39, %40, %41, %42, %43, %44, %45, %46, %47, %48, %49, %50, %51, %52, %53, %54, %55, %56, %57, %58, %59, %60, %61, %62, %63, %64, %65, %66, %67, %68, %69, %70, %71, %72, %73, %74, %75, %76, %77, %78, %79, %80, %81, %82, %83, %84, %85, %86, %87, %88, %89, %90, %91, %92, %93, %94, %95, %96, %97, %98, %99, %100, %101, %102, %103, %104, %105, %106, %107, %108, %109, %110, %111, %112, %113, %114, %115, %116, %117, %118, %119, %120, %121, %122, %123, %124, %125, %126, %127}, %128, %129, p, 1, 1, 0, 0;\n\t}\n"
         : "+f"(d[0]), "+f"(d[1]), "+f"(d[2]), "+f"(d[3]), "+f"(d[4]), "+f"(d[5]), "+f"(d[6]), "+f"(d[7]), "+f"(d[8]), "+f"(d[9]), "+f"(d[10]), "+f"(d[11]), "+f"(d[12]), "+f"(d[13]), "+f"(d[14]), "+f"(d[15]), "+f"(d[16]), "+f"(d[17]), "+f"(d[18]), "+f"(d[19]), "+f"(d[20]), "+f"(d[21]), "+f"(d[22]), "+f"(d[23]), "+f"(d[24]), "+f"(d[25]), "+f"(d[26]), "+f"(d[27]), "+f"(d[28]), "+f"(d[29]), "+f"(d[30]), "+f"(d[31]), "+f"(d[32]), "+f"(d[33]), "+f"(d[34]), "+f"(d[35]), "+f"(d[36]), "+f"(d[37]), "+f"(d[38]), "+f"(d[39]), "+f"(d[40]), "+f"(d[41]), "+f"(d[42]), "+f"(d[43]), "+f"(d[44]), "+f"(d[45]), "+f"(d[46]), "+f"(d[47]), "+f"(d[48]), "+f"(d[49]), "+f"(d[50]), "+f"(d[51]), "+f"(d[52]), "+f"(d[53]), "+f"(d[54]), "+f"(d[55]), "+f"(d[56]), "+f"(d[57]), "+f"(d[58]), "+f"(d[59]), "+f"(d[60]), "+f"(d[61]), "+f"(d[62]), "+f"(d[63]), "+f"(d[64]), "+f"(d[65]), "+f"(d[66]), "+f"(d[67]), "+f"(d[68]), "+f"(d[69]), "+f"(d[70]), "+f"(d[71]), "+f"(d[72]), "+f"(d[73]), "+f"(d[74]), "+f"(d[75]), "+f"(d[76]), "+f"(d[77]), "+f"(d[78]), "+f"(d[79]), "+f"(d[80]), "+f"(d[81]), "+f"(d[82]), "+f"(d[83]), "+f"(d[84]), "+f"(d[85]), "+f"(d[86]), "+f"(d[87]), "+f"(d[88]), "+f"(d[89]), "+f"(d[90]), "+f"(d[91]), "+f"(d[92]), "+f"(d[93]), "+f"(d[94]), "+f"(d[95]), "+f"(d[96]), "+f"(d[97]), "+f"(d[98]), "+f"(d[99]), "+f"(d[100]), "+f"(d[101]), "+f"(d[102]), "+f"(d[103]), "+f"(d[104]), "+f"(d[105]), "+f"(d[106]), "+f"(d[107]), "+f"(d[108]), "+f"(d[109]), "+f"(d[110]), "+f"(d[111]), "+f"(d[112]), "+f"(d[113]), "+f"(d[114]), "+f"(d[115]), "+f"(d[116]), "+f"(d[117]), "+f"(d[118]), "+f"(d[119]), "+f"(d[120]), "+f"(d[121]), "+f"(d[122]), "+f"(d[123]), "+f"(d[124]), "+f"(d[125]), "+f"(d[126]), "+f"(d[127])
         : "l"(da), "l"(db), "r"(accumulate));
-  }
-};
-template <> struct WgmmaRA<64, 0> {
-  static constexpr int NREG = 32;
-  static __device__ __forceinline__ void mma(float (&d)[32], const uint32_t (&a)[4], uint64_t db, uint32_t accumulate) {
-    asm volatile(
-        "{\n\t.reg .pred p;\n\tsetp.ne.b32 p, %37, 0;\n\t"
-        "wgmma.mma_async.sync.aligned.m64n64k16.f32.f16.f16 {%0, %1, %2, %3, %4, %5, %6, %7, %8, %9, %10, %11, %12, %13, %14, %15, %16, %17, %18, %19, %20, %21, %22, %23, %24, %25, %26, %27, %28, %29, %30, %31}, {%32, %33, %34, %35}, %36, p, 1, 1, 0;\n\t}\n"
-        : "+f"(d[0]), "+f"(d[1]), "+f"(d[2]), "+f"(d[3]), "+f"(d[4]), "+f"(d[5]), "+f"(d[6]), "+f"(d[7]), "+f"(d[8]), "+f"(d[9]), "+f"(d[10]), "+f"(d[11]), "+f"(d[12]), "+f"(d[13]), "+f"(d[14]), "+f"(d[15]), "+f"(d[16]), "+f"(d[17]), "+f"(d[18]), "+f"(d[19]), "+f"(d[20]), "+f"(d[21]), "+f"(d[22]), "+f"(d[23]), "+f"(d[24]), "+f"(d[25]), "+f"(d[26]), "+f"(d[27]), "+f"(d[28]), "+f"(d[29]), "+f"(d[30]), "+f"(d[31])
-        : "r"(a[0]), "r"(a[1]), "r"(a[2]), "r"(a[3]), "l"(db), "r"(accumulate));
-  }
-};
-template <> struct WgmmaRA<208, 0> {
-  static constexpr int NREG = 104;
-  static __device__ __forceinline__ void mma(float (&d)[104], const uint32_t (&a)[4], uint64_t db, uint32_t accumulate) {
-    asm volatile(
-        "{\n\t.reg .pred p;\n\tsetp.ne.b32 p, %109, 0;\n\t"
-        "wgmma.mma_async.sync.aligned.m64n208k16.f32.f16.f16 {%0, %1, %2, %3, %4, %5, %6, %7, %8, %9, %10, %11, %12, %13, %14, %15, %16, %17, %18, %19, %20, %21, %22, %23, %24, %25, %26, %27, %28, %29, %30, %31, %32, %33, %34, %35, %36, %37, %38, %39, %40, %41, %42, %43, %44, %45, %46, %47, %48, %49, %50, %51, %52, %53, %54, %55, %56, %57, %58, %59, %60, %61, %62, %63, %64, %65, %66, %67, %68, %69, %70, %71, %72, %73, %74, %75, %76, %77, %78, %79, %80, %81, %82, %83, %84, %85, %86, %87, %88, %89, %90, %91, %92, %93, %94, %95, %96, %97, %98, %99, %100, %101, %102, %103}, {%104, %105, %106, %107}, %108, p, 1, 1, 0;\n\t}\n"
-        : "+f"(d[0]), "+f"(d[1]), "+f"(d[2]), "+f"(d[3]), "+f"(d[4]), "+f"(d[5]), "+f"(d[6]), "+f"(d[7]), "+f"(d[8]), "+f"(d[9]), "+f"(d[10]), "+f"(d[11]), "+f"(d[12]), "+f"(d[13]), "+f"(d[14]), "+f"(d[15]), "+f"(d[16]), "+f"(d[17]), "+f"(d[18]), "+f"(d[19]), "+f"(d[20]), "+f"(d[21]), "+f"(d[22]), "+f"(d[23]), "+f"(d[24]), "+f"(d[25]), "+f"(d[26]), "+f"(d[27]), "+f"(d[28]), "+f"(d[29]), "+f"(d[30]), "+f"(d[31]), "+f"(d[32]), "+f"(d[33]), "+f"(d[34]), "+f"(d[35]), "+f"(d[36]), "+f"(d[37]), "+f"(d[38]), "+f"(d[39]), "+f"(d[40]), "+f"(d[41]), "+f"(d[42]), "+f"(d[43]), "+f"(d[44]), "+f"(d[45]), "+f"(d[46]), "+f"(d[47]), "+f"(d[48]), "+f"(d[49]), "+f"(d[50]), "+f"(d[51]), "+f"(d[52]), "+f"(d[53]), "+f"(d[54]), "+f"(d[55]), "+f"(d[56]), "+f"(d[57]), "+f"(d[58]), "+f"(d[59]), "+f"(d[60]), "+f"(d[61]), "+f"(d[62]), "+f"(d[63]), "+f"(d[64]), "+f"(d[65]), "+f"(d[66]), "+f"(d[67]), "+f"(d[68]), "+f"(d[69]), "+f"(d[70]), "+f"(d[71]), "+f"(d[72]), "+f"(d[73]), "+f"(d[74]), "+f"(d[75]), "+f"(d[76]), "+f"(d[77]), "+f"(d[78]), "+f"(d[79]), "+f"(d[80]), "+f"(d[81]), "+f"(d[82]), "+f"(d[83]), "+f"(d[84]), "+f"(d[85]), "+f"(d[86]), "+f"(d[87]), "+f"(d[88]), "+f"(d[89]), "+f"(d[90]), "+f"(d[91]), "+f"(d[92]), "+f"(d[93]), "+f"(d[94]), "+f"(d[95]), "+f"(d[96]), "+f"(d[97]), "+f"(d[98]), "+f"(d[99]), "+f"(d[100]), "+f"(d[101]), "+f"(d[102]), "+f"(d[103])
-        : "r"(a[0]), "r"(a[1]), "r"(a[2]), "r"(a[3]), "l"(db), "r"(accumulate));
-  }
-};
-template <> struct WgmmaRA<256, 0> {
-  static constexpr int NREG = 128;
-  static __device__ __forceinline__ void mma(float (&d)[128], const uint32_t (&a)[4], uint64_t db, uint32_t accumulate) {
-    asm volatile(
-        "{\n\t.reg .pred p;\n\tsetp.ne.b32 p, %133, 0;\n\t"
-        "wgmma.mma_async.sync.aligned.m64n256k16.f32.f16.f16 {%0, %1, %2, %3, %4, %5, %6, %7, %8, %9, %10, %11, %12, %13, %14, %15, %16, %17, %18, %19, %20, %21, %22, %23, %24, %25, %26, %27, %28, %29, %30, %31, %32, %33, %34, %35, %36, %37, %38, %39, %40, %41, %42, %43, %44, %45, %46, %47, %48, %49, %50, %51, %52, %53, %54, %55, %56, %57, %58, %59, %60, %61, %62, %63, %64, %65, %66, %67, %68, %69, %70, %71, %72, %73, %74, %75, %76, %77, %78, %79, %80, %81, %82, %83, %84, %85, %86, %87, %88, %89, %90, %91, %92, %93, %94, %95, %96, %97, %98, %99, %100, %101, %102, %103, %104, %105, %106, %107, %108, %109, %110, %111, %112, %113, %114, %115, %116, %117, %118, %119, %120, %121, %122, %123, %124, %125, %126, %127}, {%128, %129, %130, %131}, %132, p, 1, 1, 0;\n\t}\n"
-        : "+f"(d[0]), "+f"(d[1]), "+f"(d[2]), "+f"(d[3]), "+f"(d[4]), "+f"(d[5]), "+f"(d[6]), "+f"(d[7]), "+f"(d[8]), "+f"(d[9]), "+f"(d[10]), "+f"(d[11]), "+f"(d[12]), "+f"(d[13]), "+f"(d[14]), "+f"(d[15]), "+f"(d[16]), "+f"(d[17]), "+f"(d[18]), "+f"(d[19]), "+f"(d[20]), "+f"(d[21]), "+f"(d[22]), "+f"(d[23]), "+f"(d[24]), "+f"(d[25]), "+f"(d[26]), "+f"(d[27]), "+f"(d[28]), "+f"(d[29]), "+f"(d[30]), "+f"(d[31]), "+f"(d[32]), "+f"(d[33]), "+f"(d[34]), "+f"(d[35]), "+f"(d[36]), "+f"(d[37]), "+f"(d[38]), "+f"(d[39]), "+f"(d[40]), "+f"(d[41]), "+f"(d[42]), "+f"(d[43]), "+f"(d[44]), "+f"(d[45]), "+f"(d[46]), "+f"(d[47]), "+f"(d[48]), "+f"(d[49]), "+f"(d[50]), "+f"(d[51]), "+f"(d[52]), "+f"(d[53]), "+f"(d[54]), "+f"(d[55]), "+f"(d[56]), "+f"(d[57]), "+f"(d[58]), "+f"(d[59]), "+f"(d[60]), "+f"(d[61]), "+f"(d[62]), "+f"(d[63]), "+f"(d[64]), "+f"(d[65]), "+f"(d[66]), "+f"(d[67]), "+f"(d[68]), "+f"(d[69]), "+f"(d[70]), "+f"(d[71]), "+f"(d[72]), "+f"(d[73]), "+f"(d[74]), "+f"(d[75]), "+f"(d[76]), "+f"(d[77]), "+f"(d[78]), "+f"(d[79]), "+f"(d[80]), "+f"(d[81]), "+f"(d[82]), "+f"(d[83]), "+f"(d[84]), "+f"(d[85]), "+f"(d[86]), "+f"(d[87]), "+f"(d[88]), "+f"(d[89]), "+f"(d[90]), "+f"(d[91]), "+f"(d[92]), "+f"(d[93]), "+f"(d[94]), "+f"(d[95]), "+f"(d[96]), "+f"(d[97]), "+f"(d[98]), "+f"(d[99]), "+f"(d[100]), "+f"(d[101]), "+f"(d[102]), "+f"(d[103]), "+f"(d[104]), "+f"(d[105]), "+f"(d[106]), "+f"(d[107]), "+f"(d[108]), "+f"(d[109]), "+f"(d[110]), "+f"(d[111]), "+f"(d[112]), "+f"(d[113]), "+f"(d[114]), "+f"(d[115]), "+f"(d[116]), "+f"(d[117]), "+f"(d[118]), "+f"(d[119]), "+f"(d[120]), "+f"(d[121]), "+f"(d[122]), "+f"(d[123]), "+f"(d[124]), "+f"(d[125]), "+f"(d[126]), "+f"(d[127])
-        : "r"(a[0]), "r"(a[1]), "r"(a[2]), "r"(a[3]), "l"(db), "r"(accumulate));
   }
 };
 template <> struct WgmmaRA<128, 1> {
```
